# joejep/FOCNeRF

Measured on AMD Instinct MI355X. Metric: train_samples_per_sec, higher is better.
Workload: dtype f16

## Files before the change

focnerf_amd/_lib.py:

```python
import ctypes
import os

import torch

_HERE = os.path.dirname(os.path.abspath(__file__))
LIB_PATH = os.environ.get("FOCNERF_LIB_PATH") or os.path.join(_HERE, "libfocnerf_hip.so")

c_u8p = ctypes.c_void_p
c_vp = ctypes.c_void_p
u32 = ctypes.c_uint32
u64 = ctypes.c_uint64
f32 = ctypes.c_float
i32 = ctypes.c_int

FOC_F32 = 0
FOC_F16 = 1



class FocOccTrainNode(ctypes.Structure):
    _fields_ = [
        ("struct_bytes", u32),
        ("n_rays", u32), ("max_steps", u32), ("cascade", u32), ("grid_size", u32), ("cap", u32), ("pad_align", u32),
        ("bound", f32), ("dt_gamma", f32), ("min_near", f32),
# ... 59 lines not shown
    "foc_occ_train_backward_pad31": (i32, [ctypes.POINTER(FocOccTrainNode), f32, c_vp]),
    "foc_occ_train_forward_obj": (i32, [ctypes.POINTER(FocOccTrainNode), ctypes.POINTER(FocOccTrainObject), c_vp]),
    "foc_occ_train_backward_obj": (i32, [ctypes.POINTER(FocOccTrainNode), ctypes.POINTER(FocOccTrainObject), c_vp]),
    "foc_occ_tail_forward_sumsq": (i32, [c_vp, c_vp, u32, c_vp, c_vp, u32, u32, f32, f32, c_vp, f32, c_vp, c_vp, c_vp, c_vp, c_vp, c_vp, c_vp, c_vp]),
    "foc_occ_tail_backward_sumsq": (i32, [c_vp, c_vp, c_vp, c_vp, u32, c_vp, c_vp, c_vp, c_vp, c_vp, u32, u32, f32, f32, c_vp, f32, c_vp, c_vp, c_vp, c_vp]),
    "foc_occ_tail_forward": (i32, [c_vp, c_vp, u32, c_vp, c_vp, u32, u32, f32, f32, c_vp, f32, c_vp, c_vp, c_vp, c_vp, c_vp, c_vp, c_vp]),
    "foc_occ_tail_backward": (i32, [c_vp, c_vp, c_vp, c_vp, u32, c_vp, c_vp, c_vp, c_vp, c_vp, u32, u32, f32, f32, c_vp, f32, c_vp, c_vp, c_vp]),
    "foc_march_rays_train_scratch_bytes": (u64, [u32, u32]),
    "foc_composite_rays_train_forward": (i32, [c_vp, c_vp, c_vp, c_vp, u32, u32, f32, c_vp, c_vp, c_vp, c_vp]),
    "foc_composite_rays_train_backward": (i32, [c_vp, c_vp, c_vp, c_vp, c_vp, c_vp, c_vp, c_vp, u32, u32, f32,
                                                c_vp, c_vp, c_vp]),
    "foc_march_rays": (i32, [u32, u32, c_vp, c_vp, c_vp, c_vp, f32, f32, u32, u32, u32, c_vp, c_vp, c_vp,
                             c_vp, c_vp, c_vp, c_vp, c_vp]),
    "foc_composite_rays": (i32, [u32, u32, f32, c_vp, c_vp, c_vp, c_vp, c_vp, c_vp, c_vp, c_vp, c_vp]),
    "foc_compact_alive": (i32, [c_vp, u32, c_vp, c_vp, c_vp, c_vp]),
    "foc_march_rays_two_phase": (i32, [u32, u32, c_vp, c_vp, c_vp, c_vp, f32, f32, u32, u32, u32, c_vp, c_vp, c_vp, c_vp, c_vp, c_vp, c_vp, c_vp, i32, c_vp]),
    "foc_composite_compact": (i32, [u32, u32, f32, c_vp, c_vp, c_vp, c_vp, c_vp, c_vp, c_vp, c_vp, c_vp, c_vp, c_vp, c_vp, u32, u32, i32, c_vp]),
    "foc_march_rays_two_phase_fills": (i32, [u32, i32]),
    "foc_march_rays_two_phase_sample_major": (i32, [u32, u32, i32]),
    "foc_occ_render_step_scratch_bytes": (u64, [u32]),
    "foc_occ_render_step": (i32, [u32, u32, c_vp, c_vp, c_vp, c_vp, c_vp, c_vp, f32, f32, u32, u32, u32, c_vp, c_vp, c_vp, c_vp, c_vp, c_vp, c_vp, c_vp,
                                  c_vp, c_vp, c_vp, u32, f32, u32, c_vp, u32, c_vp, u32, u32, c_vp, f32, c_vp, c_vp, c_vp, c_vp, u32, c_vp, u32, u32, c_vp]),
    "foc_occ_render_step_pad31": (i32, [u32, u32, c_vp, c_vp, c_vp, c_vp, c_vp, c_vp, f32, f32, u32, u32, u32, c_vp, c_vp, c_vp, c_vp, c_vp, c_vp, c_vp, c_vp,
                                        c_vp, c_vp, c_vp, u32, f32, u32, c_vp, u32, c_vp, u32, u32, c_vp, f32, c_vp, c_vp, c_vp, c_vp, u32, c_vp, u32, u32, f32,
                                        c_vp]),
    "foc_occ_render_step_pad": (i32, [u32, u32, c_vp, c_vp, c_vp, c_vp, c_vp, c_vp, f32, f32, u32, u32, u32, c_vp, c_vp, c_vp, c_vp, c_vp, c_vp, c_vp, c_vp,
                                      c_vp, c_vp, c_vp, u32, f32, u32, c_vp, u32, c_vp, u32, u32, c_vp, f32, c_vp, c_vp, c_vp, c_vp, u32, c_vp, u32, u32, f32,
                                      c_vp]),
    "foc_grid_encode_forward": (i32, [c_vp, c_vp, c_vp, c_vp, u32, u32, u32, u32, f32, u32, c_vp, u32, i32, u32,
                                      i32, c_vp, c_vp]),
    "foc_grid_encode_forward_bl": (i32, [c_vp, c_vp, c_vp, c_vp, u32, u32, u32, u32, f32, u32, c_vp, u32, i32, u32,
                                         i32, c_vp, c_vp]),
    "foc_grid_encode_backward": (i32, [c_vp, c_vp, c_vp, c_vp, c_vp, u32, u32, u32, u32, f32, u32, c_vp, c_vp,
                                       u32, i32, u32, i32, i32, c_vp, c_vp]),
    "foc_grid_encode_backward_workspace_bytes": (u64, [u32, u32, u32, u32, i32]),
    "foc_grid_planes_to_rows": (i32, [c_vp, c_vp, u32, u32, u32, c_vp]),
    "foc_grid_rows_to_planes": (i32, [c_vp, c_vp, u32, u32, u32, c_vp]),
    "foc_grid_encode_backward_binned": (i32, [c_vp, c_vp, c_vp, c_vp, c_vp, u32, u32, u32, u32, f32, u32, c_vp, c_vp,
                                              u32, i32, u32, i32, i32, c_vp, c_vp, u64, c_vp]),
    "foc_grid_encode_forward_counted": (i32, [c_vp, c_vp, c_vp, c_vp, u32, u32, u32, u32, f32, u32, u32, i32, u32, i32, c_vp, c_vp, u64, c_vp]),
    "foc_grid_encode_backward_count": (i32, [c_vp, c_vp, u32, u32, u32, u32, f32, u32, u32, i32, u32, i32, c_vp, c_vp, u64, c_vp]),
    "foc_grid_encode_backward_binned_counted": (i32, [c_vp, c_vp, c_vp, c_vp, c_vp, u32, u32, u32, u32, f32, u32, c_vp, c_vp,
                                                      u32, i32, u32, i32, i32, c_vp, c_vp, u64, c_vp]),
    "foc_grad_total_variation": (i32, [c_vp, c_vp, c_vp, c_vp, f32, u32, u32, u32, u32, f32, u32, u32, i32, i32, c_vp]),
    "foc_freq_encode_forward": (i32, [c_vp, u32, u32, u32, u32, c_vp, c_vp]),
    "foc_freq_encode_backward": (i32, [c_vp, c_vp, u32, u32, u32, u32, c_vp, c_vp]),
    "foc_ffmlp_forward": (i32, [c_vp, c_vp, u32, u32, u32, u32, u32, u32, u32, c_vp, c_vp, c_vp]),
    "foc_ffmlp_inference": (i32, [c_vp, c_vp, u32, u32, u32, u32, u32, u32, u32, c_vp, c_vp, c_vp]),
    "foc_ffmlp_backward": (i32, [c_vp, c_vp, c_vp, c_vp, u32, u32, u32, u32, u32, u32, u32, i32,
                                 c_vp, c_vp, c_vp, c_vp, u64, c_vp]),
    "foc_ffmlp_backward_workspace_bytes": (u64, [u32, u32, u32]),
    "foc_ffmlp_forward_planar": (i32, [c_vp, c_vp, u32, u32, u32, u32, u32, u32, u32, c_vp, c_vp]),
    "foc_ffmlp_backward_planar": (i32, [c_vp, c_vp, c_vp, u32, u32, u32, u32, u32, u32, u32, i32, c_vp, c_vp, c_vp, u64, c_vp]),
    "foc_allocate_splitk": (i32, [u64]),
    "foc_free_splitk": (i32, []),
    "foc_combine_select": (i32, [c_vp, c_vp, c_vp, c_vp, u64, c_vp]),
    "foc_combine_pack_keys": (i32, [c_vp, u32, c_vp, u64, c_vp]),
    "foc_combine_unpack": (i32, [c_vp, u32, c_vp, c_vp, c_vp, u64, c_vp]),
    "foc_combine_select_composite": (i32, [c_vp, u32, c_vp, c_vp, u32, u32, c_vp, u32, c_vp, c_vp, c_vp, c_vp]),
    "foc_combine_select4": (i32, [c_vp, c_vp, u64, c_vp]),
    "foc_combine_select_composite_attr": (i32, [c_vp, u32, c_vp, c_vp, u32, c_vp, c_vp, u32, u32, c_vp, u32, c_vp, c_vp, c_vp, c_vp, c_vp, c_vp, c_vp, c_vp]),
    "foc_combine_select4_ids": (i32, [c_vp, u32, c_vp, c_vp, u64, c_vp]),
    "foc_mo_select": (i32, [c_vp, c_vp, c_vp, c_vp, u64, u32, u32, c_vp]),
    "foc_fixed_field_pack": (i32, [c_vp, c_vp, c_vp, c_vp, c_vp, c_vp, f32, u32, u32, f32, f32, c_vp, c_vp, c_vp, c_vp, u32, c_vp]),
    "foc_fixed_cull_scratch_bytes": (u64, [u32, u32]),
    "foc_fixed_cull": (i32, [c_vp, c_vp, c_vp, c_vp, c_vp, u32, u32, f32, c_vp, u32, u32, c_vp, c_vp, c_vp, c_vp, u64, c_vp]),
    "foc_fixed_cull_emit": (i32, [c_vp, c_vp, c_vp, c_vp, c_vp, u32, u32, f32, c_vp, c_vp, u32, c_vp, c_vp, c_vp]),
    "foc_fixed_field_pack_culled": (i32, [c_vp, c_vp, c_vp, c_vp, u32, c_vp, c_vp, u32, u32, f32, f32, c_vp, c_vp]),
    "foc_composite_fixed_steps":(i32, [c_vp, c_vp, c_vp, c_vp, u32, u32, f32, c_vp, c_vp, c_vp]),
    "foc_fixed_sample": (i32, [c_vp, c_vp, c_vp, c_vp, c_vp, c_vp, u32, u32, f32, c_vp, c_vp, c_vp, u32, c_vp]),
    "foc_fixed_tail_forward": (i32, [c_vp, c_vp, c_vp, c_vp, c_vp, c_vp, f32, u32, u32, f32, f32, c_vp, c_vp, c_vp, c_vp, c_vp, c_vp, u32, c_vp, c_vp]),
    "foc_fixed_tail_backward": (i32, [c_vp, c_vp, c_vp, c_vp, c_vp, c_vp, c_vp, c_vp, c_vp, c_vp, c_vp, f32, u32, u32, f32, f32, c_vp, c_vp, u32, c_vp, c_vp]),
    "foc_fixed_head_forward": (i32, [c_vp, c_vp, c_vp, c_vp, c_vp, u32, u32, f32, c_vp, c_vp, c_vp, c_vp, c_vp, c_vp, c_vp, u32, c_vp]),
    "foc_fixed_head_backward": (i32, [c_vp, c_vp, c_vp, c_vp, c_vp, c_vp, c_vp, c_vp, c_vp, c_vp, u32, u32, f32, c_vp, u32, c_vp]),
    "foc_color_head_forward": (i32, [c_vp, c_vp, u32, c_vp, u32, u32, u32, u32, c_vp, u32, c_vp, c_vp]),
    "foc_field_forward_train": (i32, [c_vp, c_vp, u32, c_vp, u32, c_vp, u32, u32, u32, u32, c_vp, c_vp, u32, c_vp, c_vp]),
    "foc_color_head_backward": (i32, [c_vp, c_vp, c_vp, u32, c_vp, c_vp, u32, u32, u32, u32, c_vp, c_vp, c_vp, u64, u32, c_vp, c_vp, c_vp]),
    "foc_color_head_forward_pad": (i32, [c_vp, c_vp, u32, c_vp, u32, u32, u32, u32, c_vp, u32, c_vp, f32, c_vp]),
    "foc_color_head_backward_pad": (i32, [c_vp, c_vp, c_vp, u32, c_vp, c_vp, u32, u32, u32, u32, c_vp, c_vp, c_vp, u64, u32, c_vp, c_vp, f32, c_vp]),
    "foc_field_forward_train_pad": (i32, [c_vp, c_vp, u32, c_vp, u32, c_vp, u32, u32, u32, u32, c_vp, c_vp, u32, c_vp, f32, c_vp]),
    "foc_color_head_forward_pad31": (i32, [c_vp, c_vp, u32, c_vp, u32, u32, u32, u32, c_vp, u32, c_vp, f32, c_vp]),
    "foc_color_head_backward_pad31": (i32, [c_vp, c_vp, c_vp, u32, c_vp, c_vp, u32, u32, u32, u32, c_vp, c_vp, c_vp, u64, u32, c_vp, c_vp, f32, c_vp]),
    "foc_field_forward_train_pad31": (i32, [c_vp, c_vp, u32, c_vp, u32, c_vp, u32, u32, u32, u32, c_vp, c_vp, u32, c_vp, f32, c_vp]),
    "foc_fixed_composite_forward": (i32, [c_vp, c_vp, c_vp, f32, u32, u32, f32, c_vp, c_vp]),
    "foc_fixed_composite_backward": (i32, [c_vp, c_vp, c_vp, c_vp, f32, u32, u32, f32, c_vp, c_vp, c_vp]),
    "foc_sample_head_forward": (i32, [c_vp, c_vp, u64, c_vp, c_vp, c_vp, u32, c_vp]),
    "foc_sample_head_backward": (i32, [c_vp, c_vp, c_vp, u64, c_vp, u32, c_vp]),
    "foc_sh_encode": (i32, [c_vp, u64, c_vp, c_vp]),
    "foc_rgb_head_forward": (i32, [c_vp, u64, c_vp, c_vp]),
    "foc_rgb_head_backward": (i32, [c_vp, c_vp, u64, c_vp, c_vp]),
    "foc_fixed_render_inference": (i32, [c_vp, c_vp, c_vp, c_vp, c_vp, c_vp, f32, u32, u32, f32, f32, c_vp, c_vp, c_vp, c_vp, u32, c_vp, c_vp]),
    "foc_nerf_field_inference": (i32, [c_vp, i32, c_vp, u32, u32, u32, c_vp, u32, c_vp, u32, u32, u32, u32, c_vp, c_vp, c_vp, c_vp]),
    "foc_nerf_field_inference_pad": (i32, [c_vp, i32, c_vp, u32, u32, u32, c_vp, u32, c_vp, u32, u32, u32, u32, c_vp, c_vp, c_vp, f32, c_vp]),
    "foc_nerf_field_inference_pad31": (i32, [c_vp, i32, c_vp, u32, u32, u32, c_vp, u32, c_vp, u32, u32, u32, u32, c_vp, c_vp, c_vp, f32, c_vp]),
    "foc_mark_untrained_grid": (i32, [c_vp, u32, f32, f32, f32, f32, f32, u32, u32, c_vp, c_vp, c_vp]),
    "foc_grid_cells_xyz": (i32, [u32, u32, f32, c_vp, c_vp, c_vp]),
    "foc_grid_update_sample_workspace_bytes": (u64, [u32, u32]),
    "foc_grid_update_sample": (i32, [c_vp, u32, u32, f32, u32, c_vp, c_vp, c_vp, c_vp, c_vp, c_vp, u64, c_vp]),
    "foc_grid_update_apply_workspace_bytes": (u64, [u32, u32]),
    "foc_grid_update_apply": (i32, [c_vp, u32, u32, c_vp, c_vp, u32, f32, f32, f32, c_vp, c_vp, c_vp, u64, c_vp]),
    "foc_background_forward": (i32, [c_vp, c_vp, c_vp, f32, u32, c_vp, c_vp, f32, u32, c_vp, c_vp, c_vp]),
    "foc_background_backward_workspace_bytes": (u64, [u32]),
    "foc_background_backward": (i32, [c_vp, c_vp, c_vp, c_vp, f32, u32, c_vp, c_vp, f32, u32, c_vp, c_vp, c_vp, c_vp, u64, c_vp]),
}


def _load():
    if not os.path.exists(LIB_PATH):
        raise ImportError(
            f"focnerf_amd: {LIB_PATH} is missing. Build it with `python -c 'import __graft_entry__ as g; g.build()'` "
            f"or `make -C focnerf_amd/csrc`. There is no CPU or PyTorch fallback for these ops.")
    try:
        lib = ctypes.CDLL(LIB_PATH)
    except OSError as e:
        raise ImportError(f"focnerf_amd: failed to load {LIB_PATH}: {e}") from e
    for name, (res, args) in SIGNATURES.items():
        fn = getattr(lib, name)
        fn.restype = res
        fn.argtypes = args
    return lib


class _Stream(ctypes.c_void_p):
    device_index = None


_multi_device = None


def _on_tensor_device(fn):
    def call(*args):
        global _multi_device
        if _multi_device is None:
            _multi_device = torch.cuda.device_count() > 1
        if _multi_device and args:
            idx = getattr(args[-1], "device_index", None)
            if idx is not None and idx != torch.cuda.current_device():
                with torch.cuda.device(idx):
                    return fn(*args)
        return fn(*args)
    call.__name__ = getattr(fn, "__name__", "foc_call")
    return call


class _Lib:

    def __init__(self, cdll):
        self._cdll = cdll
        for name, (_, args) in SIGNATURES.items():
            fn = getattr(cdll, name)
            setattr(self, name, _on_tensor_device(fn) if args and args[-1] is c_vp and not name.endswith("_bytes") else fn)


lib = _Lib(_load())


def check(rc, what=""):
    if rc != 0:
        msg = lib.foc_last_error().decode("utf-8", "replace")
        raise RuntimeError(f"focnerf_amd {what}: {msg} (code {rc})")


def ptr(t):
    if t is None:
        return None
    return ctypes.c_void_p(t.data_ptr())


_raw_stream = getattr(torch._C, "_cuda_getCurrentRawStream", None) if os.environ.get("FOC_RAW_STREAM", "1") != "0" else None


def raw_stream(index):
    if _raw_stream is not None:
        return _raw_stream(index)
    return torch.cuda.current_stream(index).cuda_stream


def stream_of(t=None):
    dev = t.device if t is not None else None
    index = dev.index if dev is not None and dev.index is not None else torch.cuda.current_device()
    s = _Stream(raw_stream(index))
    s.device_index = index
    return s


def require_cuda(*tensors):
    for t in tensors:
        if t is not None and not t.is_cuda:
            raise RuntimeError("focnerf_amd: expected a CUDA(HIP) tensor; these ops have no CPU implementation")


def dtype_code(t):
    if t.dtype == torch.float32:
        return FOC_F32
    if t.dtype == torch.float16:
        return FOC_F16
    raise RuntimeError(f"focnerf_amd: unsupported dtype {t.dtype} (float32 or float16 expected)")


def get_option(name):
    v = ctypes.c_int(0)
    check(lib.foc_get_option(name.encode(), ctypes.cast(ctypes.byref(v), ctypes.c_void_p)), "get_option")
    return v.value


def set_option(name, value):
    check(lib.foc_set_option(name.encode(), int(value)), "set_option")


class option:

    def __init__(self, name, value):
        self.name, self.value = name, int(value)

    def __enter__(self):
        self.old = get_option(self.name)
        set_option(self.name, self.value)
        return self

    def __exit__(self, *exc):
        set_option(self.name, self.old)
        return False
```

focnerf_amd/csrc/combine.hip:

```cpp
#include "common.h"
#include <string.h>

static thread_local char g_err[512] = "";

void foc_set_error(const char *fmt, ...) {
    va_list ap;
    va_start(ap, fmt);
    vsnprintf(g_err, sizeof(g_err), fmt, ap);
    va_end(ap);
}

__global__ void __launch_bounds__(256) k_combine_select(const float *__restrict__ dens, const float *__restrict__ rgb,
                                                        float *__restrict__ max_dens, float *__restrict__ best_rgb, uint64_t n) {
    for (uint64_t i = (uint64_t)blockIdx.x * 256 + threadIdx.x; i < n; i += (uint64_t)gridDim.x * 256) {
        const float d = dens[i], m = max_dens[i];
        if (d > m) { best_rgb[i * 3] = rgb[i * 3]; best_rgb[i * 3 + 1] = rgb[i * 3 + 1]; best_rgb[i * 3 + 2] = rgb[i * 3 + 2]; }
        max_dens[i] = (d != d || m != m) ? __builtin_nanf("") : (d > m ? d : m);
    }
}

__global__ void __launch_bounds__(256) k_combine_pack(const float *__restrict__ dens, uint32_t rank, uint64_t *__restrict__ keys, uint64_t n) {
    for (uint64_t i = (uint64_t)blockIdx.x * 256 + threadIdx.x; i < n; i += (uint64_t)gridDim.x * 256) {
        float d = dens[i];
        d = d > 0.0f ? d : 0.0f;
// ... 162 lines not shown
        if (lane < n_obj) {
            at->obj_weights[(uint64_t)n * n_obj + lane] = my_w;
            at->obj_depth[(uint64_t)n * n_obj + lane] = my_d;
        }
        if (lane == 0) at->instance[n] = inst;
    }
    if (lane == 0) {
        for (uint32_t q = 0; q < n_bg; q++) {
            const float rest = (1 - ws) * (q == 0 ? bg0 : bg1);
            const float o[4] = {r + rest, g + rest, b + rest, a + rest};
#pragma unroll
            for (int k = 0; k < 4; k++) image4[((uint64_t)q * N + n) * 4 + k] = fminf(1.0f, fmaxf(0.0f, o[k]));
        }
        depth[n] = d;
    }
}

__global__ void __launch_bounds__(256) k_combine_select_composite(CombineFields fields, uint32_t K, const float *__restrict__ nears,
                                                                  const float *__restrict__ fars, uint32_t N, uint32_t T, float bg0, float bg1,
                                                                  uint32_t n_bg, float *__restrict__ image4, float *__restrict__ depth,
                                                                  float4 *__restrict__ merged4) {
    combine_select_composite_body<0>(fields, nullptr, K, nears, fars, N, T, bg0, bg1, n_bg, image4, depth, merged4);
}

template <int NOBJ>
__global__ void __launch_bounds__(256) k_combine_select_composite_attr(CombineFields fields, CombineAttr at, uint32_t K,
                                                                       const float *__restrict__ nears, const float *__restrict__ fars, uint32_t N,
                                                                       uint32_t T, float bg0, float bg1, uint32_t n_bg, float *__restrict__ image4,
                                                                       float *__restrict__ depth, float4 *__restrict__ merged4) {
    combine_select_composite_body<NOBJ>(fields, &at, K, nears, fars, N, T, bg0, bg1, n_bg, image4, depth, merged4);
}

__global__ void __launch_bounds__(256) k_combine_select4(const float4 *__restrict__ f4, float4 *__restrict__ acc4, uint64_t n) {
    for (uint64_t i = (uint64_t)blockIdx.x * 256 + threadIdx.x; i < n; i += (uint64_t)gridDim.x * 256) {
        const float4 f = f4[i];
        float4 best = acc4[i];
        const float m = best.x;
        if (f.x > m) { best.y = f.y; best.z = f.z; best.w = f.w; }
        best.x = (f.x != f.x || m != m) ? __builtin_nanf("") : (f.x > m ? f.x : m);
        acc4[i] = best;
    }
}

__global__ void __launch_bounds__(256) k_combine_select4_ids(const float4 *__restrict__ f4, uint8_t id, float4 *__restrict__ acc4,
                                                             uint8_t *__restrict__ acc_ids, uint64_t n) {
    for (uint64_t i = (uint64_t)blockIdx.x * 256 + threadIdx.x; i < n; i += (uint64_t)gridDim.x * 256) {
        const float4 f = f4[i];
        float4 best = acc4[i];
        const float m = best.x;
        if (f.x > m) { best.y = f.y; best.z = f.z; best.w = f.w; acc_ids[i] = id; }
        best.x = (f.x != f.x || m != m) ? __builtin_nanf("") : (f.x > m ? f.x : m);
        acc4[i] = best;
    }
}

template <typename T>
__global__ void __launch_bounds__(256) k_mo_select(const T *__restrict__ sig_new, const T *__restrict__ feat_new, T *__restrict__ sig_best,
                                                   T *__restrict__ feat_best, uint64_t n, uint32_t width) {
    const uint64_t s0 = ((uint64_t)blockIdx.x * 4u + (threadIdx.x >> 6)) * 64u;
    if (s0 >= n) return;
    const uint32_t lane = threadIdx.x & 63u;
    bool take = false;
    if (s0 + lane < n) {
        const T a_raw = sig_new[s0 + lane];
        const float a = (float)a_raw, b = (float)sig_best[s0 + lane];
        take = (a != a) || (b == b && a >= b);
        if (take) sig_best[s0 + lane] = a_raw;
    }
    const uint64_t rows = __ballot(take);
    const uint32_t live = (uint32_t)(n - s0 < 64u ? n - s0 : 64u);
    const uint64_t base = s0 * width;
    for (uint32_t e = lane; e < live * width; e += 64u)
        if ((rows >> (e / width)) & 1ull) feat_best[base + e] = feat_new[base + e];
}

#include <stdlib.h>
#include <string.h>
#include <atomic>
#include <mutex>
struct FocOptionRow { const char *name; std::atomic<int> value; };
static FocOptionRow foc_option_table[FOC_OPT_COUNT] = {
    {"FOC_MLP_BWD_FUSED", 1}, {"FOC_FIELD_FWD_FUSED", 1}, {"FOC_GB_MERGE_MAX_RES", 480}, {"FOC_GB_FACTORED", 1}, {"FOC_GB_TAIL_SPLIT", 16}, {"FOC_GRID_FUSE_SMALL", 1},
    {"FOC_GRID_PAIRS", 1}, {"FOC_GRID_FAST", 1}, {"FOC_MARCH_SERIAL", -1}, {"FOC_MARCH_RAYS_ROW_MAX", 131072}, {"FOC_OCC_MARCH_FORM", -1},
    {"FOC_OCC_SAMPLE_MAJOR", 1}, {"FOC_OCC_FIELD_PIECE", 1 << 23}, {"FOC_DETERMINISTIC", 0},
};
static int foc_option_parse(int which, const char *text) {
    if (which == FOC_OPT_OCC_MARCH_FORM) {
        if (text[0] == 't') return 0;
        if (text[0] == 'r') return 1;
        if (text[0] == 'l') return 2;
        if (text[0] == 's') return 3;
    }
    return atoi(text);
}
static void foc_options_init() {
    static std::once_flag once;
    std::call_once(once, [] {
        for (int i = 0; i < FOC_OPT_COUNT; i++) {
            const char *e = getenv(foc_option_table[i].name);
            if (e && e[0]) foc_option_table[i].value.store(foc_option_parse(i, e), std::memory_order_relaxed);
        }
    });
}
int foc_opt(FocOpt which) { foc_options_init(); return foc_option_table[which].value.load(std::memory_order_relaxed); }

extern "C" {

int foc_set_option(const char *name, int value) {
    foc_options_init();
    for (int i = 0; i < FOC_OPT_COUNT; i++)
        if (name && strcmp(name, foc_option_table[i].name) == 0) { foc_option_table[i].value.store(value, std::memory_order_relaxed); return FOC_OK; }
    foc_set_error("set_option: unknown option '%s'", name ? name : "(null)");
    return FOC_E_INVALID;
}

int foc_get_option(const char *name, int *value) {
    foc_options_init();
    for (int i = 0; i < FOC_OPT_COUNT; i++)
        if (name && value && strcmp(name, foc_option_table[i].name) == 0) { *value = foc_option_table[i].value.load(std::memory_order_relaxed); return FOC_OK; }
    foc_set_error("get_option: unknown option '%s'", name ? name : "(null)");
    return FOC_E_INVALID;
}

int foc_guard_pick_device(int stream_is_null, int stream_device, int pointer_device, int current_device) {
    return foc_guard_pick(stream_is_null != 0, stream_device, pointer_device, current_device);
}


int foc_combine_select_composite(const float *const *fields4, uint32_t K, const float *nears, const float *fars, uint32_t N, uint32_t T,
                                 const float *bgs, uint32_t n_bg, float *image4, float *depth, float *merged4, void *stream) {
    FocDeviceGuard foc_guard_(stream, nears);
    FOC_REQUIRE(K >= 1 && K <= FOC_COMBINE_MAX_OBJECTS, FOC_E_INVALID, "combine_select_composite: 1 <= K <= %d objects per call (got %u)",
                FOC_COMBINE_MAX_OBJECTS, K);
    FOC_REQUIRE(n_bg >= 1 && n_bg <= 2 && bgs, FOC_E_INVALID, "combine_select_composite: one or two backgrounds");
    FOC_REQUIRE(T >= 2, FOC_E_INVALID, "combine_select_composite: T must be >= 2");
    if (N == 0) return FOC_OK;
    FOC_REQUIRE(fields4 && nears && fars && image4 && depth, FOC_E_INVALID, "combine_select_composite: null pointer");
    CombineFields f;
    for (uint32_t k = 0; k < FOC_COMBINE_MAX_OBJECTS; k++) {
        f.p[k] = reinterpret_cast<const float4 *>(k < K ? fields4[k] : fields4[0]);
        FOC_REQUIRE(f.p[k] && ((uintptr_t)f.p[k] & 15) == 0, FOC_E_INVALID, "combine_select_composite: field %u is null or not 16-byte aligned", k);
    }
    FOC_REQUIRE(((uintptr_t)merged4 & 15) == 0, FOC_E_INVALID, "combine_select_composite: merged4 must be 16-byte aligned");
    hipLaunchKernelGGL(k_combine_select_composite, dim3(foc_div_up(N, 4)), dim3(256), 0, (hipStream_t)stream, f, K, nears, fars, N, T, bgs[0],
                       n_bg > 1 ? bgs[1] : 0.0f, n_bg, image4, depth, reinterpret_cast<float4 *>(merged4));
    FOC_CHECK_LAUNCH("combine_select_composite");
    return FOC_OK;
}

int foc_combine_select4(const float *field4, float *acc4, uint64_t n, void *stream) {
    FocDeviceGuard foc_guard_(stream, field4);
    FOC_REQUIRE(n == 0 || (field4 && acc4), FOC_E_INVALID, "combine_select4: null pointer");
    FOC_REQUIRE((((uintptr_t)field4 | (uintptr_t)acc4) & 15) == 0, FOC_E_INVALID, "combine_select4: fields must be 16-byte aligned");
    if (n == 0) return FOC_OK;
    hipLaunchKernelGGL(k_combine_select4, dim3(foc_grid_1d(n, 256)), dim3(256), 0, (hipStream_t)stream, reinterpret_cast<const float4 *>(field4),
                       reinterpret_cast<float4 *>(acc4), n);
    FOC_CHECK_LAUNCH("combine_select4");
    return FOC_OK;
}

int foc_combine_select_composite_attr(const float *const *fields4, uint32_t K, const uint8_t *const *id_planes, const uint32_t *ids,
                                      uint32_t n_obj, const float *nears, const float *fars, uint32_t N, uint32_t T, const float *bgs,
                                      uint32_t n_bg, float *image4, float *depth, float *merged4, float *obj_weights, float *obj_depth,
                                      int32_t *instance, uint8_t *winner, void *stream) {
    FocDeviceGuard foc_guard_(stream, nears);
    FOC_REQUIRE(K >= 1 && K <= FOC_COMBINE_MAX_OBJECTS, FOC_E_INVALID, "combine_select_composite_attr: 1 <= K <= %d fields per call (got %u)",
                FOC_COMBINE_MAX_OBJECTS, K);
// ... 114 lines not shown
```

focnerf_amd/csrc/common.h:

```cpp
#pragma once
#include <hip/hip_runtime.h>
#include <hip/hip_fp16.h>
#include <stdint.h>
#include <stdio.h>
#include <stdarg.h>
#include "../../include/focnerf.h"

#define FOC_WAVE 64

void foc_set_error(const char *fmt, ...);

enum FocOpt {
    FOC_OPT_MLP_BWD_FUSED,
    FOC_OPT_FIELD_FWD_FUSED,
    FOC_OPT_GB_MERGE_MAX_RES,
    FOC_OPT_GB_FACTORED,
    FOC_OPT_GB_TAIL_SPLIT,
    FOC_OPT_GRID_FUSE_SMALL,
    FOC_OPT_GRID_PAIRS,
    FOC_OPT_GRID_FAST,
    FOC_OPT_MARCH_SERIAL,
    FOC_OPT_MARCH_RAYS_ROW_MAX,
    FOC_OPT_OCC_MARCH_FORM,
    FOC_OPT_OCC_SAMPLE_MAJOR,
    FOC_OPT_OCC_FIELD_PIECE,
    FOC_OPT_DETERMINISTIC,
    FOC_OPT_COUNT
};
int foc_opt(FocOpt which);

#define FOC_REQUIRE(cond, code, ...)                    \
    do {                                                \
        if (!(cond)) {                                  \
            foc_set_error(__VA_ARGS__);                 \
            return (code);                              \
        }                                               \
    } while (0)

#define FOC_CHECK_LAUNCH(name)                                                     \
    do {                                                                           \
        hipError_t e_ = hipGetLastError();                                         \
        if (e_ != hipSuccess) {                                                    \
            foc_set_error("%s: launch failed: %s", name, hipGetErrorString(e_));   \
            return FOC_E_LAUNCH;                                                   \
        }                                                                          \
    } while (0)

static inline int foc_guard_pick(bool stream_is_null, int stream_device, int pointer_device, int current_device) {
    if (!stream_is_null && stream_device >= 0) return stream_device;
    if (pointer_device >= 0) return pointer_device;
    return current_device;
}
struct FocDeviceGuard {
    int prev = -1;
    explicit FocDeviceGuard(void *stream, const void *first_pointer = nullptr) {
        static int n_devices = -1;
        if (n_devices < 0 && hipGetDeviceCount(&n_devices) != hipSuccess) { (void)hipGetLastError(); n_devices = 0; }
        if (n_devices == 1) return;
        int cur = 0;
        if (hipGetDevice(&cur) != hipSuccess) return;
        int sdev = -1, pdev = -1;
        if (stream != nullptr) {
            if (hipStreamGetDevice(static_cast<hipStream_t>(stream), &sdev) != hipSuccess) { (void)hipGetLastError(); sdev = -1; }
        } else if (first_pointer != nullptr) {
            hipPointerAttribute_t attr;
            if (hipPointerGetAttributes(&attr, first_pointer) == hipSuccess && attr.type == hipMemoryTypeDevice) pdev = attr.device;
            else (void)hipGetLastError();
        }
        const int want = foc_guard_pick(stream == nullptr, sdev, pdev, cur);
        if (want != cur && hipSetDevice(want) == hipSuccess) prev = cur;
    }
    ~FocDeviceGuard() { if (prev >= 0) (void)hipSetDevice(prev); }
    FocDeviceGuard(const FocDeviceGuard &) = delete;
    FocDeviceGuard &operator=(const FocDeviceGuard &) = delete;
};

static inline uint32_t foc_div_up(uint64_t a, uint64_t b) { return (uint32_t)((a + b - 1) / b); }

static inline uint32_t foc_grid_1d(uint64_t n, uint32_t block, uint32_t max_blocks = 256 * 8) {
    uint64_t g = (n + block - 1) / block;
    if (g < 1) g = 1;
    if (g > max_blocks) g = max_blocks;
    return (uint32_t)g;
}

__device__ __forceinline__ _Float16 foc_f2h(float v) { asm volatile("" : "+v"(v)); return (_Float16)v; }

__global__ static void __launch_bounds__(256) k_foc_zero(uint32_t *__restrict__ p, uint64_t n_words) {
    for (uint64_t i = (uint64_t)blockIdx.x * 256 + threadIdx.x; i < n_words; i += (uint64_t)gridDim.x * 256) p[i] = 0u;
}
static inline hipError_t foc_zero_async(void *p, size_t bytes, hipStream_t st) {
    const uint64_t n = bytes / 4;
    if (n == 0) return hipSuccess;
    uint64_t blocks = (n + 255) / 256;
    if (blocks > 4096) blocks = 4096;
    hipLaunchKernelGGL(k_foc_zero, dim3((uint32_t)blocks), dim3(256), 0, st, reinterpret_cast<uint32_t *>(p), n);
    return hipGetLastError();
}

__device__ __forceinline__ void foc_lds_barrier() { asm volatile("s_waitcnt lgkmcnt(0)\n\ts_barrier" ::: "memory"); }

__device__ __forceinline__ float wave_sum(float v) {
#pragma unroll
    for (int o = 32; o > 0; o >>= 1) v += __shfl_xor(v, o, 64);
    return v;
}
__device__ __forceinline__ int wave_sum_i(int v) {
#pragma unroll
    for (int o = 32; o > 0; o >>= 1) v += __shfl_xor(v, o, 64);
    return v;
}
__device__ __forceinline__ float wave_incl_prod(float v, int lane) {
#pragma unroll
    for (int o = 1; o < 64; o <<= 1) {
        float u = __shfl_up(v, o, 64);
        if (lane >= o) v *= u;
    }
    return v;
}
__device__ __forceinline__ float wave_incl_sum(float v, int lane) {
#pragma unroll
    for (int o = 1; o < 64; o <<= 1) {
        float u = __shfl_up(v, o, 64);
        if (lane >= o) v += u;
    }
    return v;
}
__device__ __forceinline__ int wave_incl_sum_i(int v, int lane) {
#pragma unroll
    for (int o = 1; o < 64; o <<= 1) {
        int u = __shfl_up(v, o, 64);
        if (lane >= o) v += u;
    }
    return v;
}
```

focnerf_amd/csrc/field_fwd.hip:

```cpp
#include "mlp_common.h"

typedef uint32_t ff_u2 __attribute__((ext_vector_type(2)));

__device__ __forceinline__ uint32_t ff_pack(float a, float b) {
    typedef _Float16 h2 __attribute__((ext_vector_type(2)));
    const h2 p = {(_Float16)a, (_Float16)b};
    return __builtin_bit_cast(uint32_t, p);
}

#ifndef FF_MIN_WAVES
#define FF_MIN_WAVES 2
#endif
template <int NLS, int NLC, bool RELU>
__global__ void __launch_bounds__(MLP_BLOCK, FF_MIN_WAVES) k_field_fwd_train(const _Float16 *__restrict__ planes, const _Float16 *__restrict__ w_sigma,
                                                               const _Float16 *__restrict__ w_color, _Float16 *__restrict__ h_out,
                                                               _Float16 *__restrict__ c_out, uint32_t B, MlpHead hd) {
    constexpr int HIDDEN = 64, MT = 2, KC = 4, KS0 = 2;
    constexpr int FS = MT * KS0 + (NLS - 1) * MT * KC + KC;
    constexpr int FC = MT * KS0 + (NLC - 1) * MT * KC + KC;
    extern __shared__ __attribute__((aligned(16))) _Float16 lds[];
    _Float16 *ldsS = lds, *ldsC = lds + FS * 512;
    const float *obj_bias = reinterpret_cast<const float *>(ldsC + FC * 512);
    stage_weights_fwd<HIDDEN>(w_sigma, ldsS, 32, NLS);
    stage_weights_fwd<HIDDEN>(w_color, ldsC, 32, NLC, true, head_ld0(hd));
    if (head_bias(hd)) stage_head_bias(w_color, hd, const_cast<float *>(obj_bias), HIDDEN);
    __syncthreads();

    const uint32_t lane = threadIdx.x & 63, wave = threadIdx.x >> 6;
    const int c = lane & 31, h = lane >> 5;
    const uint32_t n_tiles = (B + 31) / 32;
    const uint32_t tstride = gridDim.x * MLP_WAVES;
    uint32_t tile = blockIdx.x * MLP_WAVES + wave;
    h8 x_nxt[KS0], sh_nxt;
    auto fetch = [&](uint32_t t) {
#ifdef FF_TIMING_NO_LOAD
        const uint64_t r = (uint64_t)c + 0 * t;
#else
        const uint64_t r = min((uint64_t)min(t, n_tiles - 1u) * 32 + c, (uint64_t)B - 1);
#endif
#pragma unroll
        for (int kc = 0; kc < KS0; kc++) x_nxt[kc] = ld_planar8(planes, B, r, kc, h);
        sh_nxt = ld_head8(planes, hd, r, 0, h);
    };
    fetch(tile);
    for (; tile < n_tiles; tile += tstride) {
#ifndef FF_TIMING_HOIST
        asm volatile("" ::: "memory");
#endif
        const uint64_t row_raw = (uint64_t)tile * 32 + c;
        h8 x_cur[KS0];
#pragma unroll
        for (int kc = 0; kc < KS0; kc++) x_cur[kc] = x_nxt[kc];
        const h8 sh = sh_nxt;
        fetch(tile + tstride);
        f16v acc[MT];
#pragma unroll
        for (int mt = 0; mt < MT; mt++)
#pragma unroll
            for (int e = 0; e < 16; e++) acc[mt][e] = 0.0f;
#pragma unroll
        for (int kc = 0; kc < KS0; kc++)
#pragma unroll
            for (int mt = 0; mt < MT; mt++) acc[mt] = mfma16(ld_frag(ldsS, mt * KS0 + kc, lane), x_cur[kc], acc[mt]);
        f16v o;
        for (uint32_t l = 1; l <= (uint32_t)NLS; l++) {
            h8 bf[KC];
#pragma unroll
            for (int kc = 0; kc < KC; kc++) bf[kc] = acc_to_frag<RELU>(acc[kc >> 1], kc & 1);
            if (l < (uint32_t)NLS) {
                const uint32_t fbase = MT * KS0 + (l - 1) * MT * KC;
#pragma unroll
                for (int mt = 0; mt < MT; mt++)
#pragma unroll
                    for (int e = 0; e < 16; e++) acc[mt][e] = 0.0f;
#pragma unroll
                for (int kc = 0; kc < KC; kc++)
#pragma unroll
                    for (int mt = 0; mt < MT; mt++) acc[mt] = mfma16(ld_frag(ldsS, fbase + mt * KC + kc, lane), bf[kc], acc[mt]);
            } else {
#pragma unroll
                for (int e = 0; e < 16; e++) o[e] = 0.0f;
#pragma unroll
                for (int kc = 0; kc < KC; kc++) o = mfma16(ld_frag(ldsS, FS - KC + kc, lane), bf[kc], o);
            }
        }
        uint32_t P0 = ff_pack(o[0], o[1]), P1 = ff_pack(o[2], o[3]), P2 = ff_pack(o[4], o[5]), P3 = ff_pack(o[6], o[7]);
#ifdef FF_TIMING_NO_STORE
        if (row_raw == 0xFFFFFFFFFFull) {
#else
        if (row_raw < B) {
#endif
            *reinterpret_cast<ff_u2 *>(h_out + row_raw * 16 + 4 * h) = ff_u2{P0, P1};
            *reinterpret_cast<ff_u2 *>(h_out + row_raw * 16 + 8 + 4 * h) = ff_u2{P2, P3};
        }
        const uint32_t nxt = h == 0 ? P2 : 0u;
        const ff_u2 s02 = __builtin_amdgcn_permlane32_swap(P0, P2, false, false);
        const ff_u2 s13 = __builtin_amdgcn_permlane32_swap(P1, P3, false, false);
        const h8 hk = head_shift(u32x4{s02.x, s13.x, s02.y, s13.y}, nxt);
#pragma unroll
        for (int mt = 0; mt < MT; mt++) {
            if (head_bias(hd)) acc[mt] = ld_obj_bias(obj_bias, mt, h);
            else {
#pragma unroll
                for (int e = 0; e < 16; e++) acc[mt][e] = 0.0f;
            }
        }
#pragma unroll
        for (int kc = 0; kc < KS0; kc++)
#pragma unroll
            for (int mt = 0; mt < MT; mt++) acc[mt] = mfma16(ld_frag(ldsC, mt * KS0 + kc, lane), kc == 0 ? sh : hk, acc[mt]);
        for (uint32_t l = 1; l <= (uint32_t)NLC; l++) {
            h8 bf[KC];
#pragma unroll
            for (int kc = 0; kc < KC; kc++) bf[kc] = acc_to_frag<RELU>(acc[kc >> 1], kc & 1);
            if (l < (uint32_t)NLC) {
                const uint32_t fbase = MT * KS0 + (l - 1) * MT * KC;
#pragma unroll
                for (int mt = 0; mt < MT; mt++)
#pragma unroll
                    for (int e = 0; e < 16; e++) acc[mt][e] = 0.0f;
#pragma unroll
                for (int kc = 0; kc < KC; kc++)
#pragma unroll
                    for (int mt = 0; mt < MT; mt++) acc[mt] = mfma16(ld_frag(ldsC, fbase + mt * KC + kc, lane), bf[kc], acc[mt]);
            } else {
#pragma unroll
                for (int e = 0; e < 16; e++) o[e] = 0.0f;
#pragma unroll
                for (int kc = 0; kc < KC; kc++) o = mfma16(ld_frag(ldsC, FC - KC + kc, lane), bf[kc], o);
                if (hd.out_width == 4u) {
#ifdef FF_TIMING_NO_STORE
                    if (h == 0 && row_raw == 0xFFFFFFFFFFull) *reinterpret_cast<ff_u2 *>(c_out + row_raw * 4) = ff_u2{ff_pack(o[0], o[1]), ff_pack(o[2], o[3])};
#else
                    if (h == 0 && row_raw < B) *reinterpret_cast<ff_u2 *>(c_out + row_raw * 4) = ff_u2{ff_pack(o[0], o[1]), ff_pack(o[2], o[3])};
#endif
                } else store_tile<false>(c_out, 16, row_raw, B, 0, 16, o, h);
            }
        }
    }
}

static uint32_t ff_num_cus() {
    int dev = 0, n = 0;
    if (hipGetDevice(&dev) != hipSuccess || hipDeviceGetAttribute(&n, hipDeviceAttributeMultiprocessorCount, dev) != hipSuccess || n <= 0) n = 256;
    return (uint32_t)n;
}

template <int NLS, int NLC, bool RELU>
static int ff_launch(const void *planes, const void *w_sigma, const void *w_color, void *h, void *c, uint32_t B, const MlpHead &hd, hipStream_t st) {
    auto kern = k_field_fwd_train<NLS, NLC, RELU>;
    const size_t lds = (size_t)((4 + (NLS - 1) * 8 + 4) + (4 + (NLC - 1) * 8 + 4)) * 1024 + 256;
    if (lds > 64 * 1024) (void)hipFuncSetAttribute(reinterpret_cast<const void *>(kern), hipFuncAttributeMaxDynamicSharedMemorySize, (int)lds);
    static int resident = 0;
    if (!resident) {
        int n = 0;
        if (hipOccupancyMaxActiveBlocksPerMultiprocessor(&n, kern, MLP_BLOCK, lds) != hipSuccess || n < 1) n = 2;
        resident = n > 8 ? 8 : n;
    }
    uint32_t grid = foc_div_up(foc_div_up(B, 32), MLP_WAVES);
    const uint32_t cap = ff_num_cus() * (uint32_t)resident;
    if (grid > cap) grid = cap;
    hipLaunchKernelGGL(kern, dim3(grid), dim3(MLP_BLOCK), lds, st, (const _Float16 *)planes, (const _Float16 *)w_sigma, (const _Float16 *)w_color,
                       (_Float16 *)h, (_Float16 *)c, B, hd);
    FOC_CHECK_LAUNCH("field_forward_train");
    return FOC_OK;
}

template <int NLS, int NLC>
static int ff_launch_act(const void *planes, const void *w_sigma, const void *w_color, void *h, void *c, uint32_t B, int relu, const MlpHead &hd, hipStream_t st) {
    return relu ? ff_launch<NLS, NLC, true>(planes, w_sigma, w_color, h, c, B, hd, st) : ff_launch<NLS, NLC, false>(planes, w_sigma, w_color, h, c, B, hd, st);
}

static int field_forward_train(const void *planes, const void *sigma_weights, uint32_t sigma_layers, const void *ray_sh, uint32_t samples_per_ray,
                               const void *color_weights, uint32_t color_layers, uint32_t hidden_dim, uint32_t activation, uint32_t B, void *h, void *c,
                               uint32_t out_width, const void *obj_feat, float input_pad, bool pad31, void *stream) {
    FocDeviceGuard foc_guard_(stream, planes);
    if (B == 0) return FOC_OK;
    FOC_REQUIRE(planes && sigma_weights && ray_sh && color_weights && h && c, FOC_E_INVALID, "field_forward_train: null pointer");
    FOC_REQUIRE(hidden_dim == 64 && samples_per_ray >= 1, FOC_E_INVALID, "field_forward_train: hidden_dim must be 64 (got %u), samples_per_ray >= 1", hidden_dim);
    FOC_REQUIRE(activation == FOC_ACT_RELU || activation == FOC_ACT_NONE, FOC_E_INVALID, "field_forward_train: hidden activation must be relu(0) or none(6)");
    FOC_REQUIRE(out_width == 16 || out_width == 4, FOC_E_INVALID, "field_forward_train: out_width must be 16 or 4 (got %u)", out_width);
    const int prc = head_pad_check("field_forward_train", pad31, obj_feat, input_pad);
    if (prc) return prc;
    const MlpHead hd{(const _Float16 *)ray_sh, nullptr, samples_per_ray, out_width, (const _Float16 *)obj_feat, input_pad};
    const int relu = activation == FOC_ACT_RELU;
    hipStream_t st = (hipStream_t)stream;
    switch (sigma_layers * 10 + color_layers) {
        case 12: return ff_launch_act<1, 2>(planes, sigma_weights, color_weights, h, c, B, relu, hd, st);
        case 13: return ff_launch_act<1, 3>(planes, sigma_weights, color_weights, h, c, B, relu, hd, st);
        case 22: return ff_launch_act<2, 2>(planes, sigma_weights, color_weights, h, c, B, relu, hd, st);
        case 23: return ff_launch_act<2, 3>(planes, sigma_weights, color_weights, h, c, B, relu, hd, st);
        case 33: return ff_launch_act<3, 3>(planes, sigma_weights, color_weights, h, c, B, relu, hd, st);
        default: foc_set_error("field_forward_train: layer counts (%u, %u) are not built (1/2, 1/3, 2/2, 2/3, 3/3)", sigma_layers, color_layers); return FOC_E_INVALID;
    }
}

extern "C" {

int foc_field_forward_train(const void *planes, const void *sigma_weights, uint32_t sigma_layers, const void *ray_sh, uint32_t samples_per_ray,
                            const void *color_weights, uint32_t color_layers, uint32_t hidden_dim, uint32_t activation, uint32_t B, void *h, void *c,
                            uint32_t out_width, const void *obj_feat, void *stream) {
    return field_forward_train(planes, sigma_weights, sigma_layers, ray_sh, samples_per_ray, color_weights, color_layers, hidden_dim, activation, B, h, c,
                               out_width, obj_feat, 0.0f, false, stream);
}

int foc_field_forward_train_pad(const void *planes, const void *sigma_weights, uint32_t sigma_layers, const void *ray_sh, uint32_t samples_per_ray,
                                const void *color_weights, uint32_t color_layers, uint32_t hidden_dim, uint32_t activation, uint32_t B, void *h, void *c,
                                uint32_t out_width, const void *obj_feat, float input_pad, void *stream) {
    return field_forward_train(planes, sigma_weights, sigma_layers, ray_sh, samples_per_ray, color_weights, color_layers, hidden_dim, activation, B, h, c,
                               out_width, obj_feat, input_pad, false, stream);
}

int foc_field_forward_train_pad31(const void *planes, const void *sigma_weights, uint32_t sigma_layers, const void *ray_sh, uint32_t samples_per_ray,
                                  const void *color_weights, uint32_t color_layers, uint32_t hidden_dim, uint32_t activation, uint32_t B, void *h, void *c,
                                  uint32_t out_width, const void *obj_feat, float input_pad, void *stream) {
    return field_forward_train(planes, sigma_weights, sigma_layers, ray_sh, samples_per_ray, color_weights, color_layers, hidden_dim, activation, B, h, c,
                               out_width, obj_feat, input_pad, true, stream);
}

}
```

focnerf_amd/csrc/fixedstep.hip:

```cpp
#include "common.h"
#include "fs_common.h"
#include <float.h>

typedef _Float16 h8 __attribute__((ext_vector_type(8)));

template <bool NOISE>
__device__ __forceinline__ float fs_zu(const FsGeom &g, uint32_t i, uint32_t T, float u) {
    const float lin = (i < T / 2) ? (g.step * (float)i) : fmaf(-g.step, (float)(T - 1 - i), 1.0f);
    float z = g.near + g.span * lin;
    if (NOISE) z = z + (u - 0.5f) * g.sample_dist;
    return z;
}

__device__ __forceinline__ void fs_sh16(float x, float y, float z, float (&o)[16]) {
    const float xy = x * y, xz = x * z, yz = y * z, x2 = x * x, y2 = y * y, z2 = z * z;
    o[0] = 0.28209479177387814f;
    o[1] = -0.48860251190291987f * y;
    o[2] = 0.48860251190291987f * z;
    o[3] = -0.48860251190291987f * x;
    o[4] = 1.0925484305920792f * xy;
    o[5] = -1.0925484305920792f * yz;
    o[6] = 0.94617469575755997f * z2 - 0.31539156525251999f;
    o[7] = -1.0925484305920792f * xz;
    o[8] = 0.54627421529603959f * x2 - 0.54627421529603959f * y2;
    o[9] = 0.59004358992664352f * y * (-3.0f * x2 + y2);
    o[10] = 2.8906114426405538f * xy * z;
    o[11] = 0.45704579946446572f * y * (1.0f - 5.0f * z2);
    o[12] = 0.3731763325901154f * z * (5.0f * z2 - 3.0f);
    o[13] = 0.45704579946446572f * x * (1.0f - 5.0f * z2);
    o[14] = 1.4453057213202769f * z * (x2 - y2);
    o[15] = 0.59004358992664352f * x * (-x2 + 3.0f * y2);
}

__global__ void __launch_bounds__(256) k_fs_sample(const float *__restrict__ rays_o, const float *__restrict__ rays_d, const float *__restrict__ nears,
                                                   const float *__restrict__ fars, const float *__restrict__ aabb, const float *__restrict__ noise,
                                                   uint32_t N, uint32_t T, float bound, float *__restrict__ xyzs, float *__restrict__ enc_in,
                                                   _Float16 *__restrict__ ray_sh, uint32_t ray_block) {
    const uint64_t total = ray_block ? (uint64_t)((N + FS_RAY_BLOCK - 1) / FS_RAY_BLOCK) * FS_RAY_BLOCK * T : (uint64_t)N * T;
    const FsBox box = fs_box(aabb);
    const float two_b = 2 * bound;
    for (uint64_t s = (uint64_t)blockIdx.x * 256 + threadIdx.x; s < total; s += (uint64_t)gridDim.x * 256) {
        uint32_t n, i;
        bool own = true;
        if (ray_block) {
            const uint32_t blk = (uint32_t)(s / ((uint64_t)FS_RAY_BLOCK * T)), in = (uint32_t)(s - (uint64_t)blk * FS_RAY_BLOCK * T);
            i = in / FS_RAY_BLOCK;
            n = blk * FS_RAY_BLOCK + in % FS_RAY_BLOCK;
            own = n < N;
            n = own ? n : N - 1;
        } else {
            n = (uint32_t)(s / T); i = (uint32_t)(s - (uint64_t)n * T);
        }
        const FsGeom g = fs_geom(nears, fars, n, T);
        const float z = fs_z(g, i, T, noise, (uint64_t)n * T + i);
        float x, y, w;
        fs_point(rays_o[n * 3], rays_o[n * 3 + 1], rays_o[n * 3 + 2], rays_d[n * 3], rays_d[n * 3 + 1], rays_d[n * 3 + 2], z, box, x, y, w);
        if (xyzs) { xyzs[s * 3] = x; xyzs[s * 3 + 1] = y; xyzs[s * 3 + 2] = w; }
        if (enc_in) { enc_in[s * 3] = fs_norm(x, bound, two_b); enc_in[s * 3 + 1] = fs_norm(y, bound, two_b); enc_in[s * 3 + 2] = fs_norm(w, bound, two_b); }
        if (ray_sh && i == 0 && own) {
            float sh[16];
            fs_sh16(rays_d[n * 3], rays_d[n * 3 + 1], rays_d[n * 3 + 2], sh);
            h8 lo, hi;
#pragma unroll
            for (int k = 0; k < 8; k++) { lo[k] = foc_f2h(sh[k]); hi[k] = foc_f2h(sh[8 + k]); }
            h8 *dst = reinterpret_cast<h8 *>(ray_sh + (uint64_t)n * 16);
            dst[0] = lo; dst[1] = hi;
        }
    }
}

__global__ void __launch_bounds__(256) k_fs_head_fwd(const _Float16 *__restrict__ h, const float *__restrict__ rays_d, const float *__restrict__ nears,
                                                     const float *__restrict__ fars, const float *__restrict__ noise, uint32_t N, uint32_t T,
                                                     float density_scale, float *__restrict__ sigma_out, float *__restrict__ trans_out,
                                                     float *__restrict__ weights_out, float *__restrict__ weights_sum, float *__restrict__ depth,
                                                     _Float16 *__restrict__ cin, const _Float16 *__restrict__ obj, uint32_t cin_ld) {
    const uint32_t lane = threadIdx.x & 63;
    const uint32_t n = blockIdx.x * 4 + (threadIdx.x >> 6);
    if (n >= N) return;
    const FsGeom g = fs_geom(nears, fars, n, T);
    h8 shlo, shhi;
    h8 ob1 = {0, 0, 0, 0, 0, 0, 0, 0}, ob2 = {0, 0, 0, 0, 0, 0, 0, 0};
    _Float16 ob0 = (_Float16)0;
    if (cin) {
        float sh[16];
        fs_sh16(rays_d[n * 3], rays_d[n * 3 + 1], rays_d[n * 3 + 2], sh);
#pragma unroll
        for (int k = 0; k < 8; k++) { shlo[k] = foc_f2h(sh[k]); shhi[k] = foc_f2h(sh[8 + k]); }
        if (obj) {
            ob0 = obj[0];
#pragma unroll
            for (int k = 0; k < 8; k++) ob1[k] = obj[1 + k];
#pragma unroll
            for (int k = 0; k < 7; k++) ob2[k] = obj[9 + k];
        }
    }
    float Tc = 1.0f, ws = 0, dp = 0;
    for (uint32_t base = 0; base < T; base += 64) {
        const uint32_t i = base + lane;
        const bool valid = i < T;
        const uint64_t s = (uint64_t)n * T + (valid ? i : T - 1);
        h8 r0, r1;
        if (cin) { r0 = *reinterpret_cast<const h8 *>(h + s * 16); r1 = *reinterpret_cast<const h8 *>(h + s * 16 + 8); }
        else r0[0] = h[s * 16];
        const float sigma = expf((float)r0[0]);
        const float z = fs_z(g, valid ? i : T - 1, T, noise, s);
        float delta = g.sample_dist;
        if (i + 1 < T) delta = fs_z(g, i + 1, T, noise, s + 1) - z;
        const float alpha = valid ? 1 - expf((-delta * density_scale) * sigma) : 0.0f;
        const float om = valid ? (1 - alpha + 1e-15f) : 1.0f;
        const float P = wave_incl_prod(om, (int)lane);
        float Pex = __shfl_up(P, 1, 64);
        if (lane == 0) Pex = 1.0f;
        const float Tb = Tc * Pex;
        const float w = alpha * Tb;
        if (valid) {
            sigma_out[s] = sigma; trans_out[s] = Tb; weights_out[s] = w;
            float oz = (z - g.near) / g.span;
            oz = oz < 0.0f ? 0.0f : (oz > 1.0f ? 1.0f : oz);
            ws += w; dp += w * oz;
            if (cin) {
                h8 c2, c3;
#pragma unroll
                for (int k = 0; k < 7; k++) { c2[k] = r0[k + 1]; c3[k] = r1[k + 1]; }
                c2[7] = r1[0]; c3[7] = ob0;
                h8 *dst = reinterpret_cast<h8 *>(cin + s * cin_ld);
                dst[0] = shlo; dst[1] = shhi; dst[2] = c2; dst[3] = c3;
                if (cin_ld == 48) { dst[4] = ob1; dst[5] = ob2; }
            }
        }
        Tc *= __shfl(P, 63, 64);
    }
    ws = wave_sum(ws); dp = wave_sum(dp);
    if (lane == 0) { weights_sum[n] = ws; depth[n] = dp; }
}

__device__ __forceinline__ float wave_suffix_incl_sum(float v, int lane) {
#pragma unroll
    for (int o = 1; o < 64; o <<= 1) {
        const float u = __shfl_down(v, o, 64);
        if (lane + o < 64) v += u;
    }
    return v;
}

// ... 23 lines not shown
        float oz = (z - g.near) / g.span;
        oz = oz < 0.0f ? 0.0f : (oz > 1.0f ? 1.0f : oz);
        float gi = (grad_w ? grad_w[s] : 0.0f) + gws;
        if (gdp != 0.0f) gi += gdp * oz;
        const float gw_i = valid ? gi * (alpha * Tb) : 0.0f;
        const float incl = wave_suffix_incl_sum(gw_i, (int)lane);
        const float S_i = S_carry + (incl - gw_i);
        const float dalpha = gi * Tb - S_i / om;
        const float dsigma = dalpha * (delta * density_scale) * ex;
        const _Float16 h0 = h[s * 16];
        const float dh0 = dsigma * expf(fminf(fmaxf((float)h0, -15.0f), 15.0f));
        if (valid) {
            h8 o0, o1;
            if (grad_cin) {
                const h8 c2 = *reinterpret_cast<const h8 *>(grad_cin + s * cin_ld + 16), c3 = *reinterpret_cast<const h8 *>(grad_cin + s * cin_ld + 24);
#pragma unroll
                for (int k = 0; k < 7; k++) { o0[k + 1] = c2[k]; o1[k + 1] = c3[k]; }
                o1[0] = c2[7];
            } else {
#pragma unroll
                for (int k = 0; k < 8; k++) { o0[k] = (_Float16)0; o1[k] = (_Float16)0; }
            }
            o0[0] = foc_f2h(dh0);
            h8 *dst = reinterpret_cast<h8 *>(grad_h + s * 16);
            dst[0] = o0; dst[1] = o1;
        }
        S_carry += __shfl(incl, 0, 64);
    }
}

__device__ __forceinline__ float fs_sigmoid_h(float x) {
    return (float)(_Float16)(1.0f / (1.0f + expf(-x)));
}

__global__ void __launch_bounds__(256) k_fs_composite_fwd(const _Float16 *__restrict__ c, const float *__restrict__ weights, const float *__restrict__ bg_ray,
                                                          float bg_scalar, uint32_t N, uint32_t T, float thresh, float *__restrict__ image) {
    const uint32_t lane = threadIdx.x & 63;
    const uint32_t n = blockIdx.x * 4 + (threadIdx.x >> 6);
    if (n >= N) return;
    float r = 0, g = 0, b = 0, ws = 0;
    for (uint32_t i = lane; i < T; i += 64) {
        const uint64_t s = (uint64_t)n * T + i;
        const float w = weights[s];
        ws += w;
        if (w > thresh) {
            const uint2 raw = *reinterpret_cast<const uint2 *>(c + s * 16);
            const _Float16 *cc = reinterpret_cast<const _Float16 *>(&raw);
            r += w * fs_sigmoid_h((float)cc[0]); g += w * fs_sigmoid_h((float)cc[1]); b += w * fs_sigmoid_h((float)cc[2]);
        }
    }
    r = wave_sum(r); g = wave_sum(g); b = wave_sum(b); ws = wave_sum(ws);
    if (lane == 0) {
        const float b0 = bg_ray ? bg_ray[n * 3] : bg_scalar, b1 = bg_ray ? bg_ray[n * 3 + 1] : bg_scalar, b2 = bg_ray ? bg_ray[n * 3 + 2] : bg_scalar;
        image[n * 3] = r + (1 - ws) * b0; image[n * 3 + 1] = g + (1 - ws) * b1; image[n * 3 + 2] = b + (1 - ws) * b2;
    }
}

__global__ void __launch_bounds__(256) k_fs_composite_bwd(const float *__restrict__ grad_image, const _Float16 *__restrict__ c, const float *__restrict__ weights,
                                                          const float *__restrict__ bg_ray, float bg_scalar, uint32_t N, uint32_t T, float thresh,
                                                          _Float16 *__restrict__ grad_c, float *__restrict__ grad_w) {
    const uint64_t total = (uint64_t)N * T;
    for (uint64_t s = (uint64_t)blockIdx.x * 256 + threadIdx.x; s < total; s += (uint64_t)gridDim.x * 256) {
        const uint32_t n = (uint32_t)(s / T);
        const float g0 = grad_image[n * 3], g1 = grad_image[n * 3 + 1], g2 = grad_image[n * 3 + 2];
        const float b0 = bg_ray ? bg_ray[n * 3] : bg_scalar, b1 = bg_ray ? bg_ray[n * 3 + 1] : bg_scalar, b2 = bg_ray ? bg_ray[n * 3 + 2] : bg_scalar;
        const float w = weights[s];
        float gw = -(g0 * b0 + g1 * b1 + g2 * b2);
        h8 o0, o1;
#pragma unroll
        for (int k = 0; k < 8; k++) { o0[k] = (_Float16)0; o1[k] = (_Float16)0; }
        if (w > thresh) {
            const uint2 raw = *reinterpret_cast<const uint2 *>(c + s * 16);
            const _Float16 *cc = reinterpret_cast<const _Float16 *>(&raw);
            const float y0 = fs_sigmoid_h((float)cc[0]), y1 = fs_sigmoid_h((float)cc[1]), y2 = fs_sigmoid_h((float)cc[2]);
            gw += g0 * y0 + g1 * y1 + g2 * y2;
            o0[0] = foc_f2h(g0 * w * y0 * (1 - y0)); o0[1] = foc_f2h(g1 * w * y1 * (1 - y1)); o0[2] = foc_f2h(g2 * w * y2 * (1 - y2));
        }
        grad_w[s] = gw;
        h8 *dst = reinterpret_cast<h8 *>(grad_c + s * 16);
        dst[0] = o0; dst[1] = o1;
    }
}

template <bool NOISE>
__global__ void __launch_bounds__(256) k_fs_tail_fwd(const _Float16 *__restrict__ h, const _Float16 *__restrict__ c, const float *__restrict__ nears,
                                                     const float *__restrict__ fars, const float *__restrict__ noise, const float *__restrict__ bg_ray,
                                                     float bg_scalar, uint32_t N, uint32_t T, float density_scale, float thresh,
                                                     float *__restrict__ sigma_out, float *__restrict__ trans_out, float *__restrict__ weights_out,
                                                     float *__restrict__ weights_sum, float *__restrict__ depth, float *__restrict__ image, uint32_t c_ld,
                                                     float *__restrict__ ray_sumsq) {
    const uint32_t lane = threadIdx.x & 63;
    const uint32_t n = blockIdx.x * 4 + (threadIdx.x >> 6);
    if (n >= N) return;
    const FsGeom g = fs_geom(nears, fars, n, T);
    float Tc = 1.0f, ws = 0, dp = 0, r = 0, gg = 0, b = 0, sq = 0;
    for (uint32_t base = 0; base < T; base += 64) {
        const uint32_t i = base + lane;
        const bool valid = i < T;
        const uint32_t ic = valid ? i : T - 1;
        const uint64_t s = (uint64_t)n * T + ic;
        const _Float16 h0 = h[s * 16];
        const uint2 raw = *reinterpret_cast<const uint2 *>(c + s * c_ld);
        float u0 = 0.0f, u1 = 0.0f;
        if (NOISE) { u0 = noise[s]; u1 = noise[(uint64_t)n * T + min(ic + 1u, T - 1u)]; }
        const float sigma = expf((float)h0);
        const float z = fs_zu<NOISE>(g, ic, T, u0);
        float delta = g.sample_dist;
        if (i + 1 < T) delta = fs_zu<NOISE>(g, i + 1, T, u1) - z;
        const float alpha = valid ? 1 - expf((-delta * density_scale) * sigma) : 0.0f;
        const float om = valid ? (1 - alpha + 1e-15f) : 1.0f;
        const float P = wave_incl_prod(om, (int)lane);
        float Pex = __shfl_up(P, 1, 64);
        if (lane == 0) Pex = 1.0f;
        const float Tb = Tc * Pex;
        const float w = alpha * Tb;
        if (valid) {
            sigma_out[s] = sigma; trans_out[s] = Tb; weights_out[s] = w;
            float oz = (z - g.near) / g.span;
            oz = oz < 0.0f ? 0.0f : (oz > 1.0f ? 1.0f : oz);
            ws += w; dp += w * oz; sq = fmaf(sigma, sigma, sq);
            if (w > thresh) {
                const _Float16 *cc = reinterpret_cast<const _Float16 *>(&raw);
                r += w * fs_sigmoid_h((float)cc[0]); gg += w * fs_sigmoid_h((float)cc[1]); b += w * fs_sigmoid_h((float)cc[2]);
            }
        }
        Tc *= __shfl(P, 63, 64);
    }
    ws = wave_sum(ws); dp = wave_sum(dp); r = wave_sum(r); gg = wave_sum(gg); b = wave_sum(b);
    if (ray_sumsq) {
        sq = wave_sum(sq);
        if (lane == 0) ray_sumsq[n] = sq;
    }
    if (lane == 0) {
        const float b0 = bg_ray ? bg_ray[n * 3] : bg_scalar, b1 = bg_ray ? bg_ray[n * 3 + 1] : bg_scalar, b2 = bg_ray ? bg_ray[n * 3 + 2] : bg_scalar;
        image[n * 3] = r + (1 - ws) * b0; image[n * 3 + 1] = gg + (1 - ws) * b1; image[n * 3 + 2] = b + (1 - ws) * b2;
        weights_sum[n] = ws; depth[n] = dp;
    }
}

__device__ __forceinline__ float fs_opaque(float v) { asm volatile("" : "+v"(v)); return v; }

template <bool NOISE>
__global__ void __launch_bounds__(256) k_fs_tail_bwd(const float *__restrict__ grad_image, const float *__restrict__ grad_ws, const float *__restrict__ grad_depth,
                                                     const _Float16 *__restrict__ c, const float *__restrict__ sigma_in, const float *__restrict__ trans_in,
                                                     const float *__restrict__ weights, const float *__restrict__ nears, const float *__restrict__ fars,
                                                     const float *__restrict__ noise, const float *__restrict__ bg_ray, float bg_scalar, uint32_t N, uint32_t T,
                                                     float density_scale, float thresh, _Float16 *__restrict__ grad_c, _Float16 *__restrict__ grad_h0, uint32_t c_ld,
                                                     const float *__restrict__ grad_sumsq) {
    const uint32_t lane = threadIdx.x & 63;
    const uint32_t n = blockIdx.x * 4 + (threadIdx.x >> 6);
    if (n >= N) return;
    const FsGeom g = fs_geom(nears, fars, n, T);
    const float gws = grad_ws ? grad_ws[n] : 0.0f, gdp = grad_depth ? grad_depth[n] : 0.0f;
    const float gsq2 = grad_sumsq ? 2.0f * grad_sumsq[n] : 0.0f;
    const float g0 = grad_image[n * 3], g1 = grad_image[n * 3 + 1], g2 = grad_image[n * 3 + 2];
    const float b0 = bg_ray ? bg_ray[n * 3] : bg_scalar, b1 = bg_ray ? bg_ray[n * 3 + 1] : bg_scalar, b2 = bg_ray ? bg_ray[n * 3 + 2] : bg_scalar;
    const float e_lo = expf(fs_opaque(-15.0f)), e_hi = expf(fs_opaque(15.0f));
    float S_carry = 0.0f;
    const uint32_t n_chunks = (T + 63) / 64;
    for (uint32_t cidx = n_chunks; cidx-- > 0;) {
        const uint32_t i = cidx * 64 + lane;
        const bool valid = i < T;
        const uint32_t ic = valid ? i : T - 1;
        const uint64_t s = (uint64_t)n * T + ic;
        const float sigma = sigma_in[s], Tb = trans_in[s], w = weights[s];
        const uint2 raw = *reinterpret_cast<const uint2 *>(c + s * c_ld);
        float u0 = 0.0f, u1 = 0.0f;
        if (NOISE) { u0 = noise[s]; u1 = noise[(uint64_t)n * T + min(ic + 1u, T - 1u)]; }
        float gw = -(g0 * b0 + g1 * b1 + g2 * b2);
        h8 o0, o1;
#pragma unroll
        for (int k = 0; k < 8; k++) { o0[k] = (_Float16)0; o1[k] = (_Float16)0; }
        if (w > thresh) {
            const _Float16 *cc = reinterpret_cast<const _Float16 *>(&raw);
            const float y0 = fs_sigmoid_h((float)cc[0]), y1 = fs_sigmoid_h((float)cc[1]), y2 = fs_sigmoid_h((float)cc[2]);
            gw += g0 * y0 + g1 * y1 + g2 * y2;
            o0[0] = foc_f2h(g0 * w * y0 * (1 - y0)); o0[1] = foc_f2h(g1 * w * y1 * (1 - y1)); o0[2] = foc_f2h(g2 * w * y2 * (1 - y2));
        }
        if (valid) {
            if (c_ld == 4u) *reinterpret_cast<uint2 *>(grad_c + s * 4) = *reinterpret_cast<const uint2 *>(&o0);
            else { h8 *dst = reinterpret_cast<h8 *>(grad_c + s * 16); dst[0] = o0; dst[1] = o1; }
        }
        const float z = fs_zu<NOISE>(g, ic, T, u0);
        float delta = g.sample_dist;
        if (i + 1 < T) delta = fs_zu<NOISE>(g, i + 1, T, u1) - z;
        const float ex = expf((-delta * density_scale) * sigma);
        const float alpha = 1 - ex;
        const float om = 1 - alpha + 1e-15f;
        float oz = (z - g.near) / g.span;
        oz = oz < 0.0f ? 0.0f : (oz > 1.0f ? 1.0f : oz);
        float gi = gw + gws;
        if (gdp != 0.0f) gi += gdp * oz;
        const float gw_i = valid ? gi * (alpha * Tb) : 0.0f;
        const float incl = wave_suffix_incl_sum(gw_i, (int)lane);
        const float S_i = S_carry + (incl - gw_i);
        const float dalpha = gi * Tb - S_i / om;
        float dsigma = dalpha * (delta * density_scale) * ex;
        if (gsq2 != 0.0f) dsigma = fmaf(gsq2, sigma, dsigma);
        const float dh0 = dsigma * fminf(fmaxf(sigma, e_lo), e_hi);
        if (valid) grad_h0[s] = foc_f2h(dh0);
        S_carry += __shfl(incl, 0, 64);
    }
}


template <bool PACK>
__device__ __forceinline__ void fs_infer_finish(FsRayAcc &a, uint32_t n, uint32_t lane, const float *__restrict__ bg_ray, float bg_scalar,
                                                float *__restrict__ image, float *__restrict__ depth, float *__restrict__ weights_sum) {
    const float ws = wave_sum(a.ws), dp = wave_sum(a.dp), r = wave_sum(a.r), gg = wave_sum(a.g), b = wave_sum(a.b);
    if (lane == 0 && (!PACK || image)) {
        const float b0 = bg_ray ? bg_ray[n * 3] : bg_scalar, b1 = bg_ray ? bg_ray[n * 3 + 1] : bg_scalar, b2 = bg_ray ? bg_ray[n * 3 + 2] : bg_scalar;
        image[n * 3] = r + (1 - ws) * b0; image[n * 3 + 1] = gg + (1 - ws) * b1; image[n * 3 + 2] = b + (1 - ws) * b2;
        depth[n] = dp;
        weights_sum[n] = ws;
    }
}

template <bool PACK>
__global__ void __launch_bounds__(256) k_fs_render_infer(const float *__restrict__ sigma_in, const float *__restrict__ rgb_in, const float *__restrict__ nears,
                                                         const float *__restrict__ fars, const float *__restrict__ noise, const float *__restrict__ bg_ray,
                                                         float bg_scalar, uint32_t N, uint32_t T, float density_scale, float thresh,
                                                         float *__restrict__ image, float *__restrict__ depth, float *__restrict__ weights_sum,
                                                         float *__restrict__ rgb_masked, float4 *__restrict__ field4) {
    const uint32_t lane = threadIdx.x & 63;
    const uint32_t n = blockIdx.x * 4 + (threadIdx.x >> 6);
    if (n >= N) return;
    const FsGeom g = fs_geom(nears, fars, n, T);
    FsRayAcc a = {1.0f, 0, 0, 0, 0, 0};
    for (uint32_t base = 0; base < T; base += 64) {
        const uint32_t i = base + lane;
        const bool valid = i < T;
        const uint64_t s = (uint64_t)n * T + (valid ? i : T - 1);
        const float sigma = sigma_in[s];
        float c0 = 0, c1 = 0, c2 = 0;
        if (valid) { c0 = rgb_in[s * 3]; c1 = rgb_in[s * 3 + 1]; c2 = rgb_in[s * 3 + 2]; }
        fs_infer_tile<PACK>(a, g, n, i, lane, T, sigma, c0, c1, c2, noise, density_scale, thresh, rgb_masked, field4, nullptr);
    }
    fs_infer_finish<PACK>(a, n, lane, bg_ray, bg_scalar, image, depth, weights_sum);
}

#define FS_BLK_RAYS 16u
template <bool PACK>
__global__ void __launch_bounds__(1024) k_fs_render_infer_blk(const float *__restrict__ sigma_in, const float *__restrict__ rgb_in, const float *__restrict__ nears,
                                                              const float *__restrict__ fars, const float *__restrict__ noise, const float *__restrict__ bg_ray,
                                                              float bg_scalar, uint32_t N, uint32_t T, float density_scale, float thresh,
                                                              float *__restrict__ image, float *__restrict__ depth, float *__restrict__ weights_sum,
                                                              float *__restrict__ rgb_masked, float4 *__restrict__ field4, float *__restrict__ sigma_rm) {
    __shared__ float tile_s[64][FS_BLK_RAYS + 1];
    __shared__ float tile_c[64][FS_BLK_RAYS * 3 + 1];
    const uint32_t tid = threadIdx.x, lane = tid & 63;
    const uint32_t wv = __builtin_amdgcn_readfirstlane(tid >> 6);
    const uint32_t n0 = blockIdx.x * FS_BLK_RAYS;
    const uint64_t row0 = fs_block_row(n0, 0, T);
    const bool is_s = tid < 256;
    const uint32_t li = is_s ? tid : tid - 256;
    const uint32_t l_step = is_s ? li >> 2 : li / 12, l_part = is_s ? (li & 3) : li % 12;
    const float *src = is_s ? sigma_in + row0 + l_part * 4 : rgb_in + row0 * 3 + l_part * 4;
    const uint32_t src_ld = is_s ? FS_RAY_BLOCK : FS_RAY_BLOCK * 3;
    float *dst = is_s ? &tile_s[l_step][l_part * 4] : &tile_c[l_step][l_part * 4];
    float4 nx = make_float4(0, 0, 0, 0);
    if (l_step < T) nx = *reinterpret_cast<const float4 *>(src + (uint64_t)l_step * src_ld);
    const uint32_t n = n0 + wv;
    const bool own = n < N;
    const FsGeom g = fs_geom(nears, fars, own ? n : N - 1, T);
    FsRayAcc a = {1.0f, 0, 0, 0, 0, 0};
    for (uint32_t base = 0; base < T; base += 64) {
        dst[0] = nx.x; dst[1] = nx.y; dst[2] = nx.z; dst[3] = nx.w;
        __syncthreads();
        if (base + 64 + l_step < T) nx = *reinterpret_cast<const float4 *>(src + (uint64_t)(base + 64 + l_step) * src_ld);
        if (own)
            fs_infer_tile<PACK>(a, g, n, base + lane, lane, T, tile_s[lane][wv], tile_c[lane][wv * 3], tile_c[lane][wv * 3 + 1], tile_c[lane][wv * 3 + 2],
                                noise, density_scale, thresh, rgb_masked, field4, sigma_rm);
        __syncthreads();
    }
    if (own) fs_infer_finish<PACK>(a, n, lane, bg_ray, bg_scalar, image, depth, weights_sum);
}

struct VtState { uint32_t count, first_enc, bad, pad; };

__device__ __forceinline__ bool vt_turn(const float *__restrict__ d, uint32_t i) {
    const float ax = d[(i + 1) * 3] - d[i * 3], ay = d[(i + 1) * 3 + 1] - d[i * 3 + 1], az = d[(i + 1) * 3 + 2] - d[i * 3 + 2];
    const float bx = d[(i + 2) * 3] - d[(i + 1) * 3], by = d[(i + 2) * 3 + 1] - d[(i + 1) * 3 + 1], bz = d[(i + 2) * 3 + 2] - d[(i + 1) * 3 + 2];
    return (bx * ax + by * ay) + bz * az < 0.0f;
}

__global__ void __launch_bounds__(256) k_vt_find(const float *__restrict__ d, uint32_t N, VtState *__restrict__ st) {
    for (uint32_t i = blockIdx.x * 256 + threadIdx.x; i + 2 < N; i += gridDim.x * 256)
        if (vt_turn(d, i)) { atomicAdd(&st->count, 1u); atomicMax(&st->first_enc, N - i); }
}

__global__ void __launch_bounds__(256) k_vt_check(const float *__restrict__ d, uint32_t N, VtState *__restrict__ st) {
    const uint32_t fe = st->first_enc;
    if (fe == 0u) return;
    const uint32_t W = N - fe + 2u;
    for (uint32_t i = blockIdx.x * 256 + threadIdx.x; i + 2 < N; i += gridDim.x * 256) {
        const bool expect = (i + 2u) % W == 0u || (i + 1u) % W == 0u;
        if (vt_turn(d, i) != expect) st->bad = 1u;
    }
}

__global__ void __launch_bounds__(256) k_vt_perm(uint32_t N, uint32_t th, uint32_t tw, const VtState *__restrict__ st, int64_t *__restrict__ perm) {
    const uint32_t fe = st->first_enc, W = fe ? N - fe + 2u : 0u;
    const uint32_t H = W ? N / W : 0u;
    const bool grid = W >= 16u && N % W == 0u && H >= 8u && st->count == 2u * (H - 1u) && st->bad == 0u;
    for (uint32_t p = blockIdx.x * 256 + threadIdx.x; p < N; p += gridDim.x * 256) {
        uint32_t src = p;
        if (grid) {
            const uint64_t wt = (uint64_t)W * th;
            const uint32_t ty = (uint32_t)(p / wt), rem = (uint32_t)(p - ty * wt);
            const uint32_t rows_here = min(th, H - ty * th);
            const uint32_t tx = min(rem / (rows_here * tw), (W - 1u) / tw), r2 = rem - tx * rows_here * tw;
            const uint32_t cols_here = min(tw, W - tx * tw);
            src = (ty * th + r2 / cols_here) * W + tx * tw + r2 % cols_here;
        }
        perm[p] = (int64_t)src;
    }
}

extern "C" {

int foc_fixed_sample(const float *rays_o, const float *rays_d, const float *nears, const float *fars, const float *aabb, const float *noise,
                     uint32_t N, uint32_t T, float bound, float *xyzs, float *enc_in, void *ray_sh, uint32_t ray_block, void *stream) {
    FocDeviceGuard foc_guard_(stream, rays_o);
    if (N == 0) return FOC_OK;
    FOC_REQUIRE(rays_o && rays_d && nears && fars && aabb && (xyzs || enc_in), FOC_E_INVALID, "fixed_sample: null pointer");
    FOC_REQUIRE(T >= 2, FOC_E_INVALID, "fixed_sample: T must be >= 2");
    FOC_REQUIRE(ray_block == 0 || ray_block == FS_RAY_BLOCK, FOC_E_INVALID, "fixed_sample: ray_block must be 0 (ray-major) or %u (got %u)", FS_RAY_BLOCK, ray_block);
    const uint64_t rows = ray_block ? (uint64_t)foc_div_up(N, FS_RAY_BLOCK) * FS_RAY_BLOCK * T : (uint64_t)N * T;
    hipLaunchKernelGGL(k_fs_sample, dim3(foc_grid_1d(rows, 256, 256 * 16)), dim3(256), 0, (hipStream_t)stream, rays_o, rays_d, nears, fars, aabb,
                       noise, N, T, bound, xyzs, enc_in, (_Float16 *)ray_sh, ray_block);
    FOC_CHECK_LAUNCH("fixed_sample");
    return FOC_OK;
}

int foc_fixed_head_forward(const void *h, const float *rays_d, const float *nears, const float *fars, const float *noise, uint32_t N, uint32_t T,
                           float density_scale, float *sigma, float *trans, float *weights, float *weights_sum, float *depth, void *cin,
                           const void *obj_feat, uint32_t cin_width, void *stream) {
    FocDeviceGuard foc_guard_(stream, h);
    if (N == 0) return FOC_OK;
    FOC_REQUIRE(h && rays_d && nears && fars && sigma && trans && weights && weights_sum && depth, FOC_E_INVALID, "fixed_head_forward: null pointer");
    FOC_REQUIRE(T >= 2, FOC_E_INVALID, "fixed_head_forward: T must be >= 2");
    FOC_REQUIRE(cin_width == 32 || cin_width == 48, FOC_E_INVALID, "fixed_head_forward: cin_width must be 32 or 48 (got %u)", cin_width);
    FOC_REQUIRE(!obj_feat || cin_width == 48, FOC_E_INVALID, "fixed_head_forward: an object feature needs the 48-wide colour input");
    hipLaunchKernelGGL(k_fs_head_fwd, dim3(foc_div_up(N, 4)), dim3(256), 0, (hipStream_t)stream, (const _Float16 *)h, rays_d, nears, fars, noise, N, T,
                       density_scale, sigma, trans, weights, weights_sum, depth, (_Float16 *)cin, (const _Float16 *)obj_feat, cin_width);
    FOC_CHECK_LAUNCH("fixed_head_forward");
    return FOC_OK;
}

int foc_fixed_head_backward(const void *h, const float *sigma, const float *trans, const float *nears, const float *fars, const float *noise,
                            const float *grad_w, const float *grad_ws, const float *grad_depth, const void *grad_cin, uint32_t N, uint32_t T,
                            float density_scale, void *grad_h, uint32_t cin_width, void *stream) {
    FocDeviceGuard foc_guard_(stream, h);
    if (N == 0) return FOC_OK;
    FOC_REQUIRE(h && sigma && trans && nears && fars && grad_h, FOC_E_INVALID, "fixed_head_backward: null pointer");
    FOC_REQUIRE(T >= 2, FOC_E_INVALID, "fixed_head_backward: T must be >= 2");
    FOC_REQUIRE(cin_width == 32 || cin_width == 48, FOC_E_INVALID, "fixed_head_backward: cin_width must be 32 or 48 (got %u)", cin_width);
    hipLaunchKernelGGL(k_fs_head_bwd, dim3(foc_div_up(N, 4)), dim3(256), 0, (hipStream_t)stream, (const _Float16 *)h, sigma, trans, nears, fars, noise,
                       grad_w, grad_ws, grad_depth, (const _Float16 *)grad_cin, N, T, density_scale, (_Float16 *)grad_h, cin_width);
    FOC_CHECK_LAUNCH("fixed_head_backward");
    return FOC_OK;
}

int foc_fixed_composite_forward(const void *c, const float *weights, const float *bg_ray, float bg_scalar, uint32_t N, uint32_t T, float thresh,
                                float *image, void *stream) {
    FocDeviceGuard foc_guard_(stream, c);
    if (N == 0) return FOC_OK;
    FOC_REQUIRE(c && weights && image, FOC_E_INVALID, "fixed_composite_forward: null pointer");
    hipLaunchKernelGGL(k_fs_composite_fwd, dim3(foc_div_up(N, 4)), dim3(256), 0, (hipStream_t)stream, (const _Float16 *)c, weights, bg_ray, bg_scalar, N, T,
                       thresh, image);
    FOC_CHECK_LAUNCH("fixed_composite_forward");
    return FOC_OK;
}

int foc_fixed_composite_backward(const float *grad_image, const void *c, const float *weights, const float *bg_ray, float bg_scalar, uint32_t N,
                                 uint32_t T, float thresh, void *grad_c, float *grad_w, void *stream) {
    FocDeviceGuard foc_guard_(stream, grad_image);
    if (N == 0) return FOC_OK;
    FOC_REQUIRE(grad_image && c && weights && grad_c && grad_w, FOC_E_INVALID, "fixed_composite_backward: null pointer");
    hipLaunchKernelGGL(k_fs_composite_bwd, dim3(foc_grid_1d((uint64_t)N * T, 256, 256 * 16)), dim3(256), 0, (hipStream_t)stream, grad_image,
                       (const _Float16 *)c, weights, bg_ray, bg_scalar, N, T, thresh, (_Float16 *)grad_c, grad_w);
    FOC_CHECK_LAUNCH("fixed_composite_backward");
    return FOC_OK;
}

int foc_fixed_tail_forward(const void *h, const void *c, const float *nears, const float *fars, const float *noise, const float *bg_ray, float bg_scalar,
                           uint32_t N, uint32_t T, float density_scale, float thresh, float *sigma, float *trans, float *weights, float *weights_sum,
                           float *depth, float *image, uint32_t c_width, float *ray_sumsq, void *stream) {
    FocDeviceGuard foc_guard_(stream, h);
    if (N == 0) return FOC_OK;
    FOC_REQUIRE(c_width == 16 || c_width == 4, FOC_E_INVALID, "fixed_tail_forward: c_width must be 16 or 4 (got %u)", c_width);
    FOC_REQUIRE(h && c && nears && fars && sigma && trans && weights && weights_sum && depth && image, FOC_E_INVALID, "fixed_tail_forward: null pointer");
    FOC_REQUIRE(T >= 2, FOC_E_INVALID, "fixed_tail_forward: T must be >= 2");
    auto kern = noise ? k_fs_tail_fwd<true> : k_fs_tail_fwd<false>;
    hipLaunchKernelGGL(kern, dim3(foc_div_up(N, 4)), dim3(256), 0, (hipStream_t)stream, (const _Float16 *)h, (const _Float16 *)c, nears, fars, noise,
                       bg_ray, bg_scalar, N, T, density_scale, thresh, sigma, trans, weights, weights_sum, depth, image, c_width, ray_sumsq);
    FOC_CHECK_LAUNCH("fixed_tail_forward");
    return FOC_OK;
}

int foc_fixed_tail_backward(const float *grad_image, const float *grad_ws, const float *grad_depth, const void *c, const float *sigma, const float *trans,
                            const float *weights, const float *nears, const float *fars, const float *noise, const float *bg_ray, float bg_scalar,
                            uint32_t N, uint32_t T, float density_scale, float thresh, void *grad_c, void *grad_h0, uint32_t c_width, const float *grad_sumsq,
                            void *stream) {
    FocDeviceGuard foc_guard_(stream, grad_image);
    if (N == 0) return FOC_OK;
    FOC_REQUIRE(c_width == 16 || c_width == 4, FOC_E_INVALID, "fixed_tail_backward: c_width must be 16 or 4 (got %u)", c_width);
    FOC_REQUIRE(grad_image && c && sigma && trans && weights && nears && fars && grad_c && grad_h0, FOC_E_INVALID, "fixed_tail_backward: null pointer");
    FOC_REQUIRE(T >= 2, FOC_E_INVALID, "fixed_tail_backward: T must be >= 2");
    auto kern = noise ? k_fs_tail_bwd<true> : k_fs_tail_bwd<false>;
    hipLaunchKernelGGL(kern, dim3(foc_div_up(N, 4)), dim3(256), 0, (hipStream_t)stream, grad_image, grad_ws, grad_depth, (const _Float16 *)c, sigma,
                       trans, weights, nears, fars, noise, bg_ray, bg_scalar, N, T, density_scale, thresh, (_Float16 *)grad_c, (_Float16 *)grad_h0, c_width,
                       grad_sumsq);
    FOC_CHECK_LAUNCH("fixed_tail_backward");
    return FOC_OK;
}

int foc_fixed_render_inference(const float *sigma, const float *rgb, const float *nears, const float *fars, const float *noise, const float *bg_ray,
                               float bg_scalar, uint32_t N, uint32_t T, float density_scale, float thresh, float *image, float *depth, float *weights_sum,
                               float *rgb_masked, uint32_t ray_block, float *sigma_raymajor, void *stream) {
    FocDeviceGuard foc_guard_(stream, sigma);
    if (N == 0) return FOC_OK;
    FOC_REQUIRE(sigma && rgb && nears && fars && image && depth && weights_sum, FOC_E_INVALID, "fixed_render_inference: null pointer");
    FOC_REQUIRE(T >= 2, FOC_E_INVALID, "fixed_render_inference: T must be >= 2");
    FOC_REQUIRE(ray_block == 0 || ray_block == FS_RAY_BLOCK, FOC_E_INVALID, "fixed_render_inference: ray_block must be 0 or %u (got %u)", FS_RAY_BLOCK, ray_block);
    FOC_REQUIRE(ray_block || !sigma_raymajor, FOC_E_INVALID, "fixed_render_inference: sigma_raymajor is the un-blocked copy of a blocked sigma (ray_block == 0: sigma already is ray-major)");
    if (ray_block) {
        FOC_REQUIRE((((uintptr_t)sigma | (uintptr_t)rgb) & 15) == 0, FOC_E_INVALID, "fixed_render_inference: blocked sigma / rgb must be 16-byte aligned");
        hipLaunchKernelGGL(k_fs_render_infer_blk<false>, dim3(foc_div_up(N, FS_BLK_RAYS)), dim3(1024), 0, (hipStream_t)stream, sigma, rgb, nears, fars, noise, bg_ray, bg_scalar,
                           N, T, density_scale, thresh, image, depth, weights_sum, rgb_masked, (float4 *)nullptr, sigma_raymajor);
        FOC_CHECK_LAUNCH("fixed_render_inference");
        return FOC_OK;
    }
    hipLaunchKernelGGL(k_fs_render_infer<false>, dim3(foc_div_up(N, 4)), dim3(256), 0, (hipStream_t)stream, sigma, rgb, nears, fars, noise, bg_ray, bg_scalar, N, T,
                       density_scale, thresh, image, depth, weights_sum, rgb_masked, (float4 *)nullptr);
    FOC_CHECK_LAUNCH("fixed_render_inference");
    return FOC_OK;
}

int foc_fixed_field_pack(const float *sigma, const float *rgb, const float *nears, const float *fars, const float *noise, const float *bg_ray,
                         float bg_scalar, uint32_t N, uint32_t T, float density_scale, float thresh, float *image, float *depth, float *weights_sum,
                         float *field4, uint32_t ray_block, void *stream) {
    FocDeviceGuard foc_guard_(stream, sigma);
    if (N == 0) return FOC_OK;
    FOC_REQUIRE(sigma && rgb && nears && fars && field4, FOC_E_INVALID, "fixed_field_pack: null pointer");
    FOC_REQUIRE((image && depth && weights_sum) || (!image && !depth && !weights_sum), FOC_E_INVALID,
                "fixed_field_pack: image, depth and weights_sum go together (all or none)");
    FOC_REQUIRE(((uintptr_t)field4 & 15) == 0, FOC_E_INVALID, "fixed_field_pack: field4 must be 16-byte aligned");
    FOC_REQUIRE(T >= 2, FOC_E_INVALID, "fixed_field_pack: T must be >= 2");
    FOC_REQUIRE(ray_block == 0 || ray_block == FS_RAY_BLOCK, FOC_E_INVALID, "fixed_field_pack: ray_block must be 0 or %u (got %u)", FS_RAY_BLOCK, ray_block);
    if (ray_block) {
        FOC_REQUIRE((((uintptr_t)sigma | (uintptr_t)rgb) & 15) == 0, FOC_E_INVALID, "fixed_field_pack: blocked sigma / rgb must be 16-byte aligned");
        hipLaunchKernelGGL(k_fs_render_infer_blk<true>, dim3(foc_div_up(N, FS_BLK_RAYS)), dim3(1024), 0, (hipStream_t)stream, sigma, rgb, nears, fars, noise, bg_ray, bg_scalar,
                           N, T, density_scale, thresh, image, depth, weights_sum, (float *)nullptr, (float4 *)field4, (float *)nullptr);
        FOC_CHECK_LAUNCH("fixed_field_pack");
        return FOC_OK;
    }
    hipLaunchKernelGGL(k_fs_render_infer<true>, dim3(foc_div_up(N, 4)), dim3(256), 0, (hipStream_t)stream, sigma, rgb, nears, fars, noise, bg_ray, bg_scalar, N, T,
                       density_scale, thresh, image, depth, weights_sum, (float *)nullptr, (float4 *)field4);
    FOC_CHECK_LAUNCH("fixed_field_pack");
    return FOC_OK;
}

int foc_view_tile_order(const float *rays_d, uint32_t N, uint32_t tile_h, uint32_t tile_w, int64_t *perm, void *state16, void *stream) {
    FocDeviceGuard foc_guard_(stream, rays_d);
    if (N == 0) return FOC_OK;
    FOC_REQUIRE(rays_d && perm && state16, FOC_E_INVALID, "view_tile_order: null pointer");
    FOC_REQUIRE(tile_h >= 1 && tile_w >= 1 && tile_h * tile_w <= 4096, FOC_E_INVALID, "view_tile_order: tile %u x %u", tile_h, tile_w);
    FOC_REQUIRE(N < (1u << 31), FOC_E_INVALID, "view_tile_order: N too large");
    hipStream_t st = (hipStream_t)stream;
    VtState *state = reinterpret_cast<VtState *>(state16);
    if (foc_zero_async(state, sizeof(VtState), st) != hipSuccess) { foc_set_error("view_tile_order: zero fill failed"); return FOC_E_LAUNCH; }
    if (N >= 3) {
        hipLaunchKernelGGL(k_vt_find, dim3(foc_grid_1d(N, 256)), dim3(256), 0, st, rays_d, N, state);
        hipLaunchKernelGGL(k_vt_check, dim3(foc_grid_1d(N, 256)), dim3(256), 0, st, rays_d, N, state);
    }
    hipLaunchKernelGGL(k_vt_perm, dim3(foc_grid_1d(N, 256)), dim3(256), 0, st, N, tile_h, tile_w, state, perm);
    FOC_CHECK_LAUNCH("view_tile_order");
    return FOC_OK;
}

}
```

focnerf_amd/csrc/fs_common.h:

```cpp
#pragma once
#include "common.h"

struct FsGeom { float near, far, span, sample_dist, step; };

#define FS_RAY_BLOCK 64u
__host__ __device__ __forceinline__ uint64_t fs_block_row(uint32_t n, uint32_t i, uint32_t T) {
    return (uint64_t)(n / FS_RAY_BLOCK) * FS_RAY_BLOCK * T + (uint64_t)i * FS_RAY_BLOCK + n % FS_RAY_BLOCK;
}

__device__ __forceinline__ FsGeom fs_geom(const float *__restrict__ nears, const float *__restrict__ fars, uint32_t n, uint32_t T) {
    FsGeom g;
    g.near = nears[n]; g.far = fars[n];
    g.span = g.far - g.near;
    g.sample_dist = g.span / (float)T;
    g.step = 1.0f / (float)(T - 1);
    return g;
}
__device__ __forceinline__ float fs_z(const FsGeom &g, uint32_t i, uint32_t T, const float *__restrict__ noise, uint64_t s) {
    const float lin = (i < T / 2) ? (g.step * (float)i) : fmaf(-g.step, (float)(T - 1 - i), 1.0f);
    float z = g.near + g.span * lin;
    if (noise) z = z + (noise[s] - 0.5f) * g.sample_dist;
    return z;
}

struct FsBox { float a0, a1, a2, a3, a4, a5; };
__device__ __forceinline__ FsBox fs_box(const float *__restrict__ aabb) { return FsBox{aabb[0], aabb[1], aabb[2], aabb[3], aabb[4], aabb[5]}; }
__device__ __forceinline__ void fs_point(float ox, float oy, float oz, float dx, float dy, float dz, float z, const FsBox &b, float &x, float &y, float &w) {
    x = ox + dx * z; y = oy + dy * z; w = oz + dz * z;
    x = fminf(fmaxf(x, b.a0), b.a3); y = fminf(fmaxf(y, b.a1), b.a4); w = fminf(fmaxf(w, b.a2), b.a5);
}
__device__ __forceinline__ float fs_norm(float x, float bound, float two_b) { return (x + bound) / two_b; }

struct FsRayAcc { float Tc, ws, dp, r, g, b; };

template <bool PACK>
__device__ __forceinline__ void fs_infer_tile(FsRayAcc &a, const FsGeom &g, uint32_t n, uint32_t i, uint32_t lane, uint32_t T, float sigma, float c0, float c1,
                                              float c2, const float *__restrict__ noise, float density_scale, float thresh, float *__restrict__ rgb_masked,
                                              float4 *__restrict__ field4, float *__restrict__ sigma_rm) {
    const bool valid = i < T;
    const uint64_t s = (uint64_t)n * T + (valid ? i : T - 1);
    const float z = fs_z(g, valid ? i : T - 1, T, noise, s);
    float delta = g.sample_dist;
    if (i + 1 < T) delta = fs_z(g, i + 1, T, noise, s + 1) - z;
    const float alpha = valid ? 1 - expf((-delta * density_scale) * sigma) : 0.0f;
    const float om = valid ? (1 - alpha + 1e-15f) : 1.0f;
    const float P = wave_incl_prod(om, (int)lane);
    float Pex = __shfl_up(P, 1, 64);
    if (lane == 0) Pex = 1.0f;
    const float w = alpha * (a.Tc * Pex);
    if (valid) {
        float oz = (z - g.near) / g.span;
        oz = oz < 0.0f ? 0.0f : (oz > 1.0f ? 1.0f : oz);
        a.ws += w; a.dp += w * oz;
        const bool on = w > thresh;
        if (on) { a.r += w * c0; a.g += w * c1; a.b += w * c2; }
        if (rgb_masked) { rgb_masked[s * 3] = on ? c0 : 0.0f; rgb_masked[s * 3 + 1] = on ? c1 : 0.0f; rgb_masked[s * 3 + 2] = on ? c2 : 0.0f; }
        if (PACK) field4[s] = make_float4(sigma, on ? c0 : 0.0f, on ? c1 : 0.0f, on ? c2 : 0.0f);
        if (sigma_rm) sigma_rm[s] = sigma;
    }
    a.Tc *= __shfl(P, 63, 64);
}
```

focnerf_amd/csrc/raymarching.hip:

```cpp
#include "common.h"
#include "occ_cell.h"
#include <float.h>

#define RM_SQRT3 1.7320508075688772f
#define RM_RPI   0.3183098861837907f

__device__ __forceinline__ float rm_sign(float x) { return copysignf(1.0f, x); }

__device__ __forceinline__ uint32_t rm_morton3D_invert(uint32_t x) {
    x = x & 0x49249249u;
    x = (x | (x >> 2)) & 0xc30c30c3u;
    x = (x | (x >> 4)) & 0x0f00f00fu;
    x = (x | (x >> 8)) & 0xff0000ffu;
    x = (x | (x >> 16)) & 0x0000ffffu;
    return x;
}

__device__ __forceinline__ void rm_near_far(float ox, float oy, float oz, float dx, float dy, float dz, float a0, float a1, float a2, float a3, float a4, float a5,
                                            float min_near, float &near_out, float &far_out) {
    const float rdx = 1 / dx, rdy = 1 / dy, rdz = 1 / dz;
    float near = (a0 - ox) * rdx, far = (a3 - ox) * rdx, t;
    if (near > far) { t = near; near = far; far = t; }
    float near_y = (a1 - oy) * rdy, far_y = (a4 - oy) * rdy;
    if (near_y > far_y) { t = near_y; near_y = far_y; far_y = t; }
    bool miss = (near > far_y || near_y > far);
    if (!miss) {
        if (near_y > near) near = near_y;
        if (far_y < far) far = far_y;
        float near_z = (a2 - oz) * rdz, far_z = (a5 - oz) * rdz;
        if (near_z > far_z) { t = near_z; near_z = far_z; far_z = t; }
        miss = (near > far_z || near_z > far);
        if (!miss) {
            if (near_z > near) near = near_z;
            if (far_z < far) far = far_z;
            if (near < min_near) near = min_near;
        }
    }
    near_out = miss ? FLT_MAX : near;
    far_out = miss ? FLT_MAX : far;
}

__global__ void __launch_bounds__(256) k_near_far_from_aabb(const float *__restrict__ rays_o, const float *__restrict__ rays_d,
                                     const float *__restrict__ aabb, uint32_t N, float min_near,
                                     float *__restrict__ nears, float *__restrict__ fars) {
    const float a0 = aabb[0], a1 = aabb[1], a2 = aabb[2], a3 = aabb[3], a4 = aabb[4], a5 = aabb[5];
    for (uint32_t n = blockIdx.x * blockDim.x + threadIdx.x; n < N; n += gridDim.x * blockDim.x) {
        float near, far;
        rm_near_far(rays_o[n * 3], rays_o[n * 3 + 1], rays_o[n * 3 + 2], rays_d[n * 3], rays_d[n * 3 + 1], rays_d[n * 3 + 2], a0, a1, a2, a3, a4, a5, min_near, near, far);
        nears[n] = near;
        fars[n] = far;
    }
}

__global__ void __launch_bounds__(256) k_sph_from_ray(const float *__restrict__ rays_o, const float *__restrict__ rays_d, float radius,
                               uint32_t N, float *__restrict__ coords) {
    for (uint32_t n = blockIdx.x * blockDim.x + threadIdx.x; n < N; n += gridDim.x * blockDim.x) {
        const float ox = rays_o[n * 3], oy = rays_o[n * 3 + 1], oz = rays_o[n * 3 + 2];
        const float dx = rays_d[n * 3], dy = rays_d[n * 3 + 1], dz = rays_d[n * 3 + 2];
        const float A = fmaf(dz, dz, fmaf(dy, dy, dx * dx));
        const float B = fmaf(oz, dz, fmaf(oy, dy, ox * dx));
        const float C = fmaf(-radius, radius, fmaf(oz, oz, fmaf(oy, oy, ox * ox)));
        const float t = (-B + sqrtf(fmaf(B, B, -(A * C)))) / A;
        const float x = fmaf(t, dx, ox), y = fmaf(t, dy, oy), z = fmaf(t, dz, oz);
        const float theta = atan2f(sqrtf(fmaf(z, z, x * x)), y);
        const float phi = atan2f(z, x);
        coords[n * 2] = fmaf(2 * theta, RM_RPI, -1.0f);
        coords[n * 2 + 1] = phi * RM_RPI;
    }
}

__global__ void __launch_bounds__(256) k_morton3D(const int32_t *__restrict__ coords, uint32_t N, int32_t *__restrict__ indices) {
    for (uint32_t n = blockIdx.x * blockDim.x + threadIdx.x; n < N; n += gridDim.x * blockDim.x)
        indices[n] = (int32_t)rm_morton3D((uint32_t)coords[n * 3], (uint32_t)coords[n * 3 + 1], (uint32_t)coords[n * 3 + 2]);
}
__global__ void __launch_bounds__(256) k_morton3D_invert(const int32_t *__restrict__ indices, uint32_t N, int32_t *__restrict__ coords) {
    for (uint32_t n = blockIdx.x * blockDim.x + threadIdx.x; n < N; n += gridDim.x * blockDim.x) {
        const int32_t ind = indices[n];
        coords[n * 3] = (int32_t)rm_morton3D_invert((uint32_t)(ind >> 0));
        coords[n * 3 + 1] = (int32_t)rm_morton3D_invert((uint32_t)(ind >> 1));
        coords[n * 3 + 2] = (int32_t)rm_morton3D_invert((uint32_t)(ind >> 2));
    }
}

__global__ void __launch_bounds__(256) k_packbits_x4(const float4 *__restrict__ grid4, uint32_t N4, float thresh,
                              uint32_t *__restrict__ bitfield4) {
    for (uint32_t n = blockIdx.x * blockDim.x + threadIdx.x; n < N4; n += gridDim.x * blockDim.x) {
        uint32_t bits = 0;
#pragma unroll
        for (int q = 0; q < 8; q++) {
            const float4 v = grid4[(uint64_t)n * 8 + q];
            bits |= (v.x > thresh ? 1u : 0u) << (q * 4 + 0);
            bits |= (v.y > thresh ? 1u : 0u) << (q * 4 + 1);
            bits |= (v.z > thresh ? 1u : 0u) << (q * 4 + 2);
            bits |= (v.w > thresh ? 1u : 0u) << (q * 4 + 3);
        }
        bitfield4[n] = bits;
    }
}
__global__ void __launch_bounds__(256) k_packbits_tail(const float *__restrict__ grid, uint32_t n0, uint32_t N, float thresh,
                                uint8_t *__restrict__ bitfield) {
    for (uint32_t n = n0 + blockIdx.x * blockDim.x + threadIdx.x; n < N; n += gridDim.x * blockDim.x) {
        uint32_t bits = 0;
#pragma unroll
        for (int i = 0; i < 8; i++) bits |= (grid[(uint64_t)n * 8 + i] > thresh ? 1u : 0u) << i;
        bitfield[n] = (uint8_t)bits;
    }
}

struct RmCell { float x, y, z, dt, mip_bound; int nx, ny, nz; };

struct RmParams {
    float bound, dt_gamma, dt_min, dt_max, rH, H3, Hf, Cf, Hm1;
    uint32_t H;
    float norm_inv;
    int rederive;
    int gamma_pow2;
};
__device__ __forceinline__ float rm_out(const RmParams &p, float x) { return p.norm_inv != 0.0f ? (x + p.bound) * p.norm_inv : x; }

__device__ __forceinline__ bool rm_cell(const uint8_t *__restrict__ grid, const RmParams &p, float ox, float oy, float oz,
                                        float dx, float dy, float dz, float t, RmCell &c) {
    c.x = rm_clamp(fmaf(t, dx, ox), -p.bound, p.bound);
// ... 1193 lines not shown
```

focnerf_amd/field.py:

```python
import os
from dataclasses import dataclass
from typing import Optional

import torch
from torch.autograd import Function
from torch.amp import custom_bwd, custom_fwd

from .backend import _gridencoder, _ffmlp
from .ffmlp import FFMLP, PackedMLP, single_pass_backward
from .gridencoder import GridEncoder, GridSpec


def fused_mlp(model, name):
    get = getattr(model, "fused_mlp", None)
    return get(name) if get is not None else getattr(model, name, None)


@dataclass(frozen=True)
class MlpShape:
    input_dim: int
    hidden_dim: int
    num_layers: int
    activation: int
    output_activation: int
# ... 105 lines not shown
            _half_scope = {}
        return self

    def __exit__(self, *exc):
        global _half_scope
        _half_scope = self._outer
        return False


def _half_of(param):
    if param.dtype == torch.half:
        return param.contiguous()
    if _half_scope is None:
        return param.detach().to(torch.half).contiguous()
    hit = _half_scope.get(id(param))
    if hit is not None and hit[0] is param and hit[1].device == param.device:
        if hit[2] is not None and _raw_stream_of(param.device) != hit[3]:
            torch.cuda.current_stream(param.device).wait_event(hit[2])
        return hit[1]
    h = param.detach().to(torch.half).contiguous()
    ev = st = None
    if h.is_cuda:
        st = _raw_stream_of(h.device)
        ev = torch.cuda.Event()
        ev.record(torch.cuda.current_stream(h.device))
    _half_scope[id(param)] = (param, h, ev, st)
    return h


def scope_cached(key, owner, make):
    if _half_scope is None:
        return make()
    hit = _half_scope.get(key)
    if hit is not None and hit[0] is owner:
        if hit[2] is not None and _raw_stream_of(hit[1].device) != hit[3]:
            torch.cuda.current_stream(hit[1].device).wait_event(hit[2])
        return hit[1]
    v = make()
    ev = st = None
    if v.is_cuda:
        st = _raw_stream_of(v.device)
        ev = torch.cuda.Event()
        ev.record(torch.cuda.current_stream(v.device))
    _half_scope[key] = (owner, v, ev, st)
    return v


def _check_colour_branch(colour, B):
    cweights, shape, ray_sh, T, c_width, obj_feat = colour[:6]
    T = int(T)
    if not (ray_sh.dtype == torch.half and ray_sh.dim() == 2 and ray_sh.shape[1] == 16 and ray_sh.is_contiguous() and T > 0
            and B == ray_sh.shape[0] * T):
        raise RuntimeError(f"hashgrid_mlp colour branch: ray_sh must be a contiguous half [B / T, 16] tensor with B = {B}, T = {T}; got "
                           f"{tuple(ray_sh.shape)} {ray_sh.dtype}{'' if ray_sh.is_contiguous() else ' (strided)'}")
    if c_width not in (4, 16):
        raise RuntimeError(f"hashgrid_mlp colour branch: c_width must be 4 or 16, got {c_width}")
    if shape.input_dim not in (32, 48) or (obj_feat is not None) != (shape.input_dim == 48) or (obj_feat is not None and obj_feat.numel() != 16):
        raise RuntimeError(f"hashgrid_mlp colour branch: a {shape.input_dim}-wide colour input takes "
                           f"{'a 16-element object feature' if shape.input_dim == 48 else 'no object feature'}, got "
                           f"{'none' if obj_feat is None else f'{obj_feat.numel()} elements'}")
    if cweights.numel() != 64 * (shape.input_dim + 64 * (shape.num_layers - 1) + 16):
        raise RuntimeError(f"hashgrid_mlp colour branch: the colour weights hold {cweights.numel()} elements, a {shape.input_dim}-wide "
                           f"{shape.num_layers}-layer network has {64 * (shape.input_dim + 64 * (shape.num_layers - 1) + 16)}")


class _hashgrid_mlp(Function):
    @staticmethod
    @custom_fwd(device_type="cuda")
    def forward(ctx, x, embeddings, weights, offsets, grid, sigma, training, colour=None):
        x = x.contiguous().float()
        B = x.shape[0]
        if colour is not None:
            _check_colour_branch(colour, B)
        S, H, (gridtype, align_corners, interp) = grid.log2_scale, grid.base_resolution, grid.tail()
        L = offsets.shape[0] - 1
        emb = _half_of(embeddings)
        w = _half_of(weights)
        enc = torch.empty(L, B, 2, device=x.device, dtype=torch.half)
        ticket = _gridencoder.grid_encode_forward_counted(x, emb, offsets, enc, B, 3, 2, L, S, H, gridtype, align_corners, interp,
                                                          standalone=_gridencoder.precount_standalone()) if training else None
        if ticket is None:
            _gridencoder.grid_encode_forward(x, emb, offsets, enc, B, 3, 2, L, S, H, None, gridtype, align_corners, interp)
        h = torch.empty(B, 16, device=x.device, dtype=torch.half)
        c = None
        if colour is not None:
            from ._lib import ptr, stream_of, check
            cweights, cshape, ray_sh, T, c_width, obj_feat = colour[:6]
            pad = float(colour[6]) if len(colour) > 6 else 0.0
            wc = _half_of(cweights)
            obj16 = obj_feat.detach().reshape(-1).half().contiguous() if obj_feat is not None else None
            c = torch.empty(B, c_width, device=x.device, dtype=torch.half)
            args = (ptr(enc), ptr(w), sigma.num_layers, ptr(ray_sh), int(T), ptr(wc), int(cshape.num_layers), 64, int(sigma.activation), B, ptr(h),
                    ptr(c), int(c_width), ptr(obj16))
            fn, extra = pad_twin("foc_field_forward_train", pad, obj16 is not None)
            check(fn(*args, *extra, stream_of(enc)), "field_forward_train")
        else:
            _ffmlp.ffmlp_forward_planar(enc, w, B, sigma.input_dim, 16, sigma.hidden_dim, sigma.num_layers, sigma.activation, sigma.output_activation, h)
        if training:
            ctx.save_for_backward(x, emb, w, offsets, enc)
            ctx.cfg = (grid, sigma, B, L)
            ctx.ticket = ticket
        if c is None:
            return h
        ctx.mark_non_differentiable(c)
        ctx.set_materialize_grads(False)
        return h, c

    @staticmethod
    @custom_bwd(device_type="cuda")
    def backward(ctx, grad_h, _grad_c=None):
        x, emb, w, offsets, enc = ctx.saved_tensors
        grid, sigma, B, L = ctx.cfg
        if grad_h is None:
            return (None,) * 8
        grad_h = grad_h.contiguous().half()
        g_enc = torch.empty_like(enc)
        g_w = torch.empty_like(w)
        _ffmlp.ffmlp_backward_planar(grad_h, enc, w, B, sigma.input_dim, 16, sigma.hidden_dim, sigma.num_layers, sigma.activation,
                                     sigma.output_activation, True, g_enc, g_w)
        g_emb = torch.zeros_like(emb)
        _gridencoder.grid_encode_backward(g_enc, x, emb, offsets, g_emb, B, 3, 2, L, grid.log2_scale, grid.base_resolution, None, None, *grid.tail(),
                                          grad_bl=False, precount=ctx.ticket)
        return None, g_emb, g_w, None, None, None, None, None


@torch.no_grad()
def field_infer(model, xn, dirs, dir_div=1, dir_block=0, obj_feat=None):
    from ._lib import ptr, stream_of, check
    enc, sn, cn = model.encoder, fused_mlp(model, "sigma_net"), fused_mlp(model, "color_net")
    grid = enc.spec()
    xn = xn.contiguous().float()
    dirs = dirs.contiguous().float()
    M = xn.shape[0]
    L = enc.offsets.shape[0] - 1
    emb, ws, wc = _half_of(enc.embeddings), _half_of(sn.weights), _half_of(cn.weights)
    planes = torch.empty(L, M, 2, device=xn.device, dtype=torch.half)
    _gridencoder.grid_encode_forward(xn, emb, enc.offsets, planes, M, 3, 2, L, grid.log2_scale, grid.base_resolution, None, *grid.tail())
    sigma = torch.empty(M, dtype=torch.float32, device=xn.device)
    rgb = torch.empty(M, 3, dtype=torch.float32, device=xn.device)
    obj16 = None
    if getattr(model, "uses_object_feature", False):
        if obj_feat is None:
            raise RuntimeError("field_infer: an object-conditioned network needs its encoded object feature")
        obj16 = obj_feat.detach().reshape(-1).half().contiguous()
        assert obj16.numel() == 16
    args = (ptr(planes), 1, ptr(dirs), int(dir_div), int(dir_block), dirs.shape[0], ptr(ws), sn.num_layers, ptr(wc), cn.num_layers, 64, sn.activation, M,
            ptr(sigma), ptr(rgb), ptr(obj16))
    fn, extra = pad_twin("foc_nerf_field_inference", float(getattr(model, "colour_input_pad", 0.0)), obj16 is not None)
    check(fn(*args, *extra, stream_of(xn)), "nerf_field_inference")
    return sigma, rgb


def hashgrid_mlp(encoder, mlp, x, bound=1, colour=None):
    prefix = list(x.shape[:-1])
    xn = (x if bound is None else (x + bound) / (2 * bound)).view(-1, 3)
    h = _hashgrid_mlp.apply(xn, encoder.embeddings, mlp.weights, encoder.offsets, encoder.spec(), MlpShape.of(mlp), mlp.training and torch.is_grad_enabled(),
                            colour)
    if colour is not None:
        h, c = h
        return h.view(prefix + [16]), c
    return h.view(prefix + [16])
```

focnerf_amd/fixedstep.py:

```python
import torch
from torch.autograd import Function

from . import raymarching
from ._lib import lib, ptr, stream_of, check
from .gridencoder import grid_encode


RAY_BLOCK = 64


def ray_block_default():
    import os
    return RAY_BLOCK if os.environ.get("FOC_RAY_BLOCK", str(RAY_BLOCK)) != "0" else 0


def blocked_rows(N, T, ray_block):
    return N * T if not ray_block else -(-N // ray_block) * ray_block * T


def fixed_sample(rays_o, rays_d, nears, fars, aabb, noise, T, bound, want_xyzs=False, want_ray_sh=False, ray_block=0):
    N = rays_o.shape[0]
    dev = rays_o.device
    rows = blocked_rows(N, T, ray_block)
    enc_in = torch.empty(rows, 3, dtype=torch.float32, device=dev)
    xyzs = torch.empty(rows, 3, dtype=torch.float32, device=dev) if want_xyzs else None
    ray_sh = torch.empty(N, 16, dtype=torch.float16, device=dev) if want_ray_sh else None
    check(lib.foc_fixed_sample(ptr(rays_o), ptr(rays_d), ptr(nears), ptr(fars), ptr(aabb), ptr(noise), N, T, float(bound), ptr(xyzs), ptr(enc_in),
                               ptr(ray_sh), int(ray_block), stream_of(rays_o)), "fixed_sample")
    if want_ray_sh:
        return enc_in, xyzs, ray_sh
    return enc_in, xyzs


def ray_sh_rows(rays_d):
    rays_d = rays_d.contiguous().float()
    N, dev = rays_d.shape[0], rays_d.device
    zeros, ones = torch.zeros(N, device=dev), torch.ones(N, device=dev)
    aabb = torch.tensor([-1., -1., -1., 1., 1., 1.], device=dev)
    return fixed_sample(torch.zeros_like(rays_d), rays_d, zeros, ones, aabb, None, 2, 1.0, want_ray_sh=True)[2]


class _density_head(Function):

    @staticmethod
    def forward(ctx, h, rays_d, nears, fars, noise, N, T, density_scale, obj_feat=None):
        h = h.contiguous()
        assert h.dtype == torch.float16 and h.shape == (N * T, 16)
        dev = h.device
        M = N * T
        sigma = torch.empty(M, dtype=torch.float32, device=dev)
        trans = torch.empty(M, dtype=torch.float32, device=dev)
        weights = torch.empty(M, dtype=torch.float32, device=dev)
        ws = torch.empty(N, dtype=torch.float32, device=dev)
        depth = torch.empty(N, dtype=torch.float32, device=dev)
        width = 32 if obj_feat is None else 48
        if obj_feat is not None:
            obj_feat = obj_feat.detach().reshape(-1).half().contiguous()
            assert obj_feat.numel() == 16
        cin = torch.empty(M, width, dtype=torch.float16, device=dev)
        check(lib.foc_fixed_head_forward(ptr(h), ptr(rays_d), ptr(nears), ptr(fars), ptr(noise), N, T, float(density_scale), ptr(sigma), ptr(trans),
                                         ptr(weights), ptr(ws), ptr(depth), ptr(cin), ptr(obj_feat), width, stream_of(h)), "fixed_head_forward")
        ctx.save_for_backward(h, sigma, trans, nears, fars, noise if noise is not None else torch.empty(0, device=dev))
        ctx.has_noise = noise is not None
        ctx.dims = (N, T, float(density_scale))
        ctx.width = width
        ctx.mark_non_differentiable(sigma)
        ctx.set_materialize_grads(False)
        return weights, ws, depth, sigma, cin

    @staticmethod
    def backward(ctx, g_weights, g_ws, g_depth, g_sigma, g_cin):
        h, sigma, trans, nears, fars, noise = ctx.saved_tensors
        N, T, ds = ctx.dims
        noise = noise if ctx.has_noise else None
        g_weights = g_weights.contiguous().float() if g_weights is not None else None
        g_ws = g_ws.contiguous().float() if g_ws is not None else None
        g_depth = g_depth.contiguous().float() if g_depth is not None else None
        g_cin = g_cin.contiguous().half() if g_cin is not None else None
        grad_h = torch.empty_like(h)
        check(lib.foc_fixed_head_backward(ptr(h), ptr(sigma), ptr(trans), ptr(nears), ptr(fars), ptr(noise), ptr(g_weights), ptr(g_ws), ptr(g_depth),
                                          ptr(g_cin), N, T, ds, ptr(grad_h), ctx.width, stream_of(h)), "fixed_head_backward")
        g_obj = None
        if ctx.width == 48 and ctx.needs_input_grad[8] and g_cin is not None:
            g_obj = g_cin[:, 31:47].float().sum(0)
        return grad_h, None, None, None, None, None, None, None, g_obj


class _fixed_composite(Function):

    @staticmethod
    def forward(ctx, c, weights, bg_ray, bg_scalar, N, T, thresh, weights_sum=None):
        c = c.contiguous()
        weights = weights.contiguous()
        assert c.dtype == torch.float16 and c.shape == (N * T, 16) and weights.dtype == torch.float32
        image = torch.empty(N, 3, dtype=torch.float32, device=c.device)
        check(lib.foc_fixed_composite_forward(ptr(c), ptr(weights), ptr(bg_ray), float(bg_scalar), N, T, float(thresh), ptr(image), stream_of(c)),
              "fixed_composite_forward")
        ctx.bg_grad = bg_ray is not None and ctx.needs_input_grad[2]
        if ctx.bg_grad and weights_sum is None:
            raise RuntimeError("_fixed_composite: a background that needs a gradient needs weights_sum")
        empty = torch.empty(0, device=c.device)
        ctx.save_for_backward(c, weights, bg_ray if bg_ray is not None else empty, weights_sum.detach() if ctx.bg_grad else empty)
        ctx.has_bg = bg_ray is not None
        ctx.dims = (N, T, float(thresh), float(bg_scalar))
        return image

    @staticmethod
    def backward(ctx, g_image):
        c, weights, bg_ray, weights_sum = ctx.saved_tensors
        N, T, thresh, bg_scalar = ctx.dims
        bg_ray = bg_ray if ctx.has_bg else None
        g_image = g_image.contiguous().float()
        grad_c = torch.empty_like(c)
        grad_w = torch.empty_like(weights)
        check(lib.foc_fixed_composite_backward(ptr(g_image), ptr(c), ptr(weights), ptr(bg_ray), bg_scalar, N, T, thresh, ptr(grad_c), ptr(grad_w),
                                               stream_of(c)), "fixed_composite_backward")
        g_bg = g_image * (1 - weights_sum).unsqueeze(-1) if ctx.bg_grad else None
        return grad_c, grad_w, g_bg, None, None, None, None, None


_C_WIDTH = 4


class _render_tail(Function):

    @staticmethod
    def forward(ctx, h, cweights, ray_sh, nears, fars, noise, bg_ray, bg_scalar, N, T, density_scale, thresh, num_layers, activation, obj_feat=None,
                want_sumsq=False, c_pre=None, w16_pre=None, input_pad=0.0):
        from .field import _half_of, pad_twin
        h = h.contiguous()
        assert h.dtype == torch.float16 and h.shape == (N * T, 16)
        assert ray_sh.dtype == torch.float16 and ray_sh.shape == (N, 16) and ray_sh.is_contiguous()
        dev, M = h.device, N * T
        st = stream_of(h)
        w16 = w16_pre if w16_pre is not None else _half_of(cweights)
        obj16 = None
        if obj_feat is not None:
            obj16 = obj_feat.detach().reshape(-1).half().contiguous()
            assert obj16.numel() == 16 and w16.numel() == 64 * (48 + 64 * (int(num_layers) - 1) + 16)
        if c_pre is not None:
            assert c_pre.dtype == torch.float16 and c_pre.shape == (M, _C_WIDTH) and c_pre.is_contiguous()
            c = c_pre
        else:
            c = torch.empty(M, _C_WIDTH, dtype=torch.float16, device=dev)
            args = (ptr(h), ptr(ray_sh), T, ptr(w16), M, 64, int(num_layers), int(activation), ptr(c), _C_WIDTH, ptr(obj16))
            fn, extra = pad_twin("foc_color_head_forward", input_pad, obj16 is not None)
            check(fn(*args, *extra, st), "color_head_forward")
        sigma = torch.empty(M, dtype=torch.float32, device=dev)
        trans = torch.empty(M, dtype=torch.float32, device=dev)
        weights = torch.empty(M, dtype=torch.float32, device=dev)
        ws = torch.empty(N, dtype=torch.float32, device=dev)
        depth = torch.empty(N, dtype=torch.float32, device=dev)
        image = torch.empty(N, 3, dtype=torch.float32, device=dev)
        sumsq = torch.empty(N, dtype=torch.float32, device=dev) if want_sumsq else None
        check(lib.foc_fixed_tail_forward(ptr(h), ptr(c), ptr(nears), ptr(fars), ptr(noise), ptr(bg_ray), float(bg_scalar), N, T, float(density_scale),
                                         float(thresh), ptr(sigma), ptr(trans), ptr(weights), ptr(ws), ptr(depth), ptr(image), _C_WIDTH, ptr(sumsq), st),
              "fixed_tail_forward")
        empty = torch.empty(0, device=dev)
        ctx.bg_grad = bg_ray is not None and ctx.needs_input_grad[6]
        ctx.save_for_backward(h, w16, sigma, trans, weights, c, ray_sh, nears, fars, noise if noise is not None else empty,
                              bg_ray if bg_ray is not None else empty, obj16 if obj16 is not None else empty, ws if ctx.bg_grad else empty)
        ctx.flags = (noise is not None, bg_ray is not None, obj16 is not None, obj_feat.dtype if obj_feat is not None else None,
                     tuple(obj_feat.shape) if obj_feat is not None else None)
        ctx.dims = (N, T, float(density_scale), float(thresh), float(bg_scalar), int(num_layers), int(activation), float(input_pad))
        ctx.mark_non_differentiable(sigma, weights, c)
        ctx.set_materialize_grads(False)
        if want_sumsq:
            return image, ws, depth, sigma, weights, c, sumsq
        return image, ws, depth, sigma, weights, c

    @staticmethod
    def backward(ctx, g_image, g_ws, g_depth, _g_sigma, _g_weights, _g_c, g_sumsq=None):
        from .backend import _scratch
        from .field import pad_twin
        h, w16, sigma, trans, weights, c, ray_sh, nears, fars, noise, bg_ray, obj16, ws = ctx.saved_tensors
        has_noise, has_bg, has_obj, obj_dtype, obj_shape = ctx.flags
        obj16 = obj16 if has_obj else None
        N, T, ds, thresh, bg_scalar, num_layers, activation, input_pad = ctx.dims
        noise = noise if has_noise else None
        bg_ray = bg_ray if has_bg else None
        dev, M = h.device, N * T
        st = stream_of(h)
        g_image = g_image.contiguous().float() if g_image is not None else torch.zeros(N, 3, dtype=torch.float32, device=dev)
        g_ws = g_ws.contiguous().float() if g_ws is not None else None
        g_depth = g_depth.contiguous().float() if g_depth is not None else None
        g_sumsq = g_sumsq.contiguous().float() if g_sumsq is not None else None
        grad_c = torch.empty_like(c)
        grad_h0 = torch.empty(M, dtype=torch.float16, device=dev)
        check(lib.foc_fixed_tail_backward(ptr(g_image), ptr(g_ws), ptr(g_depth), ptr(c), ptr(sigma), ptr(trans), ptr(weights), ptr(nears), ptr(fars),
                                          ptr(noise), ptr(bg_ray), bg_scalar, N, T, ds, thresh, ptr(grad_c), ptr(grad_h0), _C_WIDTH, ptr(g_sumsq), st),
              "fixed_tail_backward")
        grad_h = torch.empty_like(h)
        g_w = torch.empty_like(w16)
        wsb = _scratch.get("ffmlp_ws", lib.foc_ffmlp_backward_workspace_bytes(48 if has_obj else 32, 64, num_layers), dev)
        g_obj32 = torch.empty(16, dtype=torch.float32, device=dev) if has_obj and ctx.needs_input_grad[14] else None
        args = (ptr(grad_c), ptr(h), ptr(ray_sh), T, ptr(grad_h0), ptr(w16), M, 64, num_layers, activation, ptr(grad_h), ptr(g_w), ptr(wsb),
                wsb.numel(), _C_WIDTH, ptr(obj16), ptr(g_obj32))
        fn, extra = pad_twin("foc_color_head_backward", input_pad, has_obj)
        check(fn(*args, *extra, st), "color_head_backward")
        g_obj = g_obj32.to(obj_dtype).view(obj_shape) if g_obj32 is not None else None
        g_bg = g_image * (1 - ws).unsqueeze(-1) if ctx.bg_grad else None
        return (grad_h, g_w, None, None, None, None, g_bg) + (None,) * 7 + (g_obj, None, None, None, None)


class _masked_norm(Function):

    @staticmethod
    def forward(ctx, sumsq, outside):
        crit = torch.sqrt((sumsq * outside).sum())
        ctx.save_for_backward(crit, outside)
        return crit

    @staticmethod
    def backward(ctx, g):
        crit, outside = ctx.saved_tensors
        coef = torch.where(crit > 0, g / (2 * crit), torch.zeros_like(crit))
        return outside * coef, None


def _background(bg_color, N, dev):
    if bg_color is None:
        return None, 1.0
    if torch.is_tensor(bg_color):
        if bg_color.numel() > 1:
            return bg_color.to(dev, torch.float32).expand(N, 3).contiguous(), 0.0
        return None, float(bg_color)
    return None, float(bg_color)


def render_fixed_steps(model, rays_o, rays_d, yolo_details=None, num_steps=512, bg_color=None, perturb=False, weight_thresh=1e-10,
                       return_fields=None, _out=None, **kwargs):
    import time
    if return_fields is None:
        return_fields = not model.training
    t_start = time.time()
    prefix = rays_o.shape[:-1]
    rays_o = rays_o.contiguous().view(-1, 3).float()
    rays_d = rays_d.contiguous().view(-1, 3).float()
    N, T = rays_o.shape[0], int(num_steps)
    dev = rays_o.device
    aabb = model.aabb_train if model.training else model.aabb_infer
    nears, fars = raymarching.near_far_from_aabb(rays_o, rays_d, aabb, model.min_near)
    noise = torch.rand(N * T, dtype=torch.float32, device=dev) if perturb else None
    from .field import field_plan, field_infer
    plan = field_plan(model)
    if getattr(model, "bg_radius", 0) > 0:
        bg_color = model._background_colour(rays_o, rays_d, bg_color)
    want_tail = plan.tail and model.training and torch.is_grad_enabled()
    fused_infer = not torch.is_grad_enabled() and plan.infer
    rb = ray_block_default() if fused_infer else 0
    enc_in, _, ray_sh = fixed_sample(rays_o, rays_d, nears, fars, aabb, noise, T, model.bound, want_ray_sh=True) if want_tail else \
        fixed_sample(rays_o, rays_d, nears, fars, aabb, noise, T, model.bound, ray_block=rb) + (None,)

    if fused_infer:
        obj_feat = model.encode_object_feature(yolo_details, dev) if plan.uses_object_feature else None
        sigma, rgb = field_infer(model, enc_in, rays_d, dir_div=T, dir_block=rb, obj_feat=obj_feat)
        bg_ray, bg_scalar = _background(bg_color, N, dev)
        direct = (_out is not None and _out[0].dtype == torch.float32 and _out[1].dtype == torch.float32 and _out[0].is_contiguous()
                  and _out[1].is_contiguous() and _out[0].numel() == N and _out[1].numel() == 3 * N and _out[0].device == dev)
        depth, image = (_out[0].view(N), _out[1].view(N, 3)) if direct else (torch.empty(N, dtype=torch.float32, device=dev),
                                                                              torch.empty(N, 3, dtype=torch.float32, device=dev))
        weights_sum = torch.empty(N, dtype=torch.float32, device=dev)
        rgb_masked = densities = None
        if return_fields:
            if direct and len(_out) == 4 and all(t.dtype == torch.float32 and t.is_contiguous() and t.device == dev for t in _out[2:]) \
                    and _out[2].numel() == N * T and _out[3].numel() == 3 * N * T and rb:
                densities, rgb_masked = _out[2].view(N * T), _out[3].view(N * T, 3)
            else:
                rgb_masked = torch.empty(N * T, 3, dtype=torch.float32, device=dev)
                densities = torch.empty(N * T, dtype=torch.float32, device=dev) if rb else None
        check(lib.foc_fixed_render_inference(ptr(sigma), ptr(rgb), ptr(nears), ptr(fars), ptr(noise), ptr(bg_ray), float(bg_scalar), N, T,
                                             float(model.density_scale), float(weight_thresh), ptr(image), ptr(depth), ptr(weights_sum), ptr(rgb_masked),
                                             rb, ptr(densities), stream_of(sigma)), "fixed_render_inference")
        t_mid = time.time()
        results = {'depth': depth.view(*prefix), 'image': image.view(*prefix, 3), 'weights_sum': weights_sum, 'criterion_outside_mask': None,
                   'timing': [t_mid - t_start, time.time() - t_mid]}
        if return_fields:
            results['densities'] = (densities if rb else sigma).view(N, T, 1)
            results['rgbs'] = rgb_masked.view(N, T, 3)
        return results

    enc = model.encoder
    from .field import hashgrid_mlp, fused_mlp
    c_pre = obj_feat = None
    cweights = fused_mlp(model, "color_net").weights if want_tail else None
    with torch.autocast("cuda", dtype=torch.float16):
        if plan.uses_object_feature:
            obj_feat = model.encode_object_feature(yolo_details, dev)
        if plan.field:
            colour = wc16 = None
            if want_tail and plan.train_forward:
                from .field import _half_of
                wc16 = _half_of(cweights)
                colour = (wc16, plan.colour, ray_sh, T, _C_WIDTH, obj_feat, plan.colour_input_pad)
            h = hashgrid_mlp(enc, fused_mlp(model, "sigma_net"), enc_in, None, colour)
            if colour is not None:
                h, c_pre = h
        else:
            feats = grid_encode(enc_in, enc.embeddings, enc.offsets, enc.per_level_scale, enc.base_resolution, False, enc.gridtype_id,
                                enc.align_corners, enc.interp_id)
            h = fused_mlp(model, "sigma_net")(feats)
        if h.shape[1] != 16:
            raise RuntimeError("render_fixed_steps expects a 16-wide sigma head (1 + geo_feat_dim = 16)")
        fused_tail = want_tail
        want_crit = model.training and yolo_details is not None and yolo_details[0] is not None
        criterion_outside_mask = None
        if fused_tail:
            cn = fused_mlp(model, "color_net")
            bg_ray, bg_scalar = _background(bg_color, N, dev)
            outs = _render_tail.apply(h, cweights, ray_sh, nears, fars, noise, bg_ray, bg_scalar, N, T, model.density_scale, weight_thresh,
                                      cn.num_layers, cn.activation, obj_feat, want_crit and yolo_details[0].numel() == N, c_pre,
                                      wc16 if c_pre is not None else None, plan.colour_input_pad)
            image, weights_sum, depth, sigma, weights, c = outs[:6]
            if len(outs) == 7:
                criterion_outside_mask = _masked_norm.apply(outs[6], (~yolo_details[0].reshape(N)).to(torch.float32))
        else:
            weights, weights_sum, depth, sigma, cin = _density_head.apply(h, rays_d, nears, fars, noise, N, T, model.density_scale, obj_feat)
            if plan.colour_input_pad != 0:
                cin = torch.cat([cin[:, :-1], cin.new_full((cin.shape[0], 1), plan.colour_input_pad)], dim=1)
        if want_crit and criterion_outside_mask is None:
            from .activation import trunc_exp
            criterion_outside_mask = torch.norm(trunc_exp(h[:, 0]).view(N, T)[~yolo_details[0].squeeze(0)] - 0)
        if not fused_tail:
            c = fused_mlp(model, "color_net").forward_padded(cin)
    t_mid = time.time()

    if not fused_tail:
        bg_ray, bg_scalar = _background(bg_color, N, dev)
        image = _fixed_composite.apply(c, weights, bg_ray, bg_scalar, N, T, weight_thresh, weights_sum)

    results = {'depth': depth.view(*prefix), 'image': image.view(*prefix, 3), 'weights_sum': weights_sum,
               'criterion_outside_mask': criterion_outside_mask, 'timing': [t_mid - t_start, time.time() - t_mid]}
    if return_fields:
        from .head import rgb_head
        c16 = c.detach()
        if c16.shape[1] != 16:
            c16 = torch.nn.functional.pad(c16, (0, 16 - c16.shape[1]))
        rgb = rgb_head(c16) * (weights > weight_thresh).unsqueeze(-1)
        results['densities'] = sigma.view(N, T, 1)
        results['rgbs'] = rgb.view(N, T, 3)
    return results


@torch.no_grad()
def render_field4(model, rays_o, rays_d, num_steps=512, weight_thresh=1e-10, yolo_details=None, out=None, occupancy=None):
    from .field import field_plan, field_infer
    rays_o = rays_o.contiguous().view(-1, 3).float()
    rays_d = rays_d.contiguous().view(-1, 3).float()
    N, T = rays_o.shape[0], int(num_steps)
    dev = rays_o.device
    if out is None:
        out = torch.empty(N, T, 4, dtype=torch.float32, device=dev)
    assert out.shape == (N, T, 4) and out.dtype == torch.float32 and out.is_contiguous()
    plan = field_plan(model)
    if occupancy is not None:
        from .fixedcull import render_field4_culled
        return render_field4_culled(model, plan, rays_o, rays_d, T, weight_thresh, yolo_details, out, occupancy)
    if plan.infer and model.bg_radius <= 0:
        aabb = model.aabb_train if model.training else model.aabb_infer
        nears, fars = raymarching.near_far_from_aabb(rays_o, rays_d, aabb, model.min_near)
        rb = ray_block_default()
        enc_in, _ = fixed_sample(rays_o, rays_d, nears, fars, aabb, None, T, model.bound, ray_block=rb)
        obj_feat = model.encode_object_feature(yolo_details, dev) if plan.uses_object_feature else None
        sigma, rgb = field_infer(model, enc_in, rays_d, dir_div=T, dir_block=rb, obj_feat=obj_feat)
        check(lib.foc_fixed_field_pack(ptr(sigma), ptr(rgb), ptr(nears), ptr(fars), None, None, 1.0, N, T, float(model.density_scale),
                                       float(weight_thresh), None, None, None, ptr(out), rb, stream_of(sigma)), "fixed_field_pack")
        return out
    from .combine import pack_field4
    with torch.autocast("cuda", dtype=torch.float16):
        res = model.run(rays_o[None], rays_d[None], yolo_details, num_steps=T, upsample_steps=0, perturb=False, weight_thresh=weight_thresh,
                        return_fields=True)
    out.copy_(pack_field4(res['densities'], res['rgbs']))
    return out
```

include/focnerf.h:

```cpp
#ifndef FOCNERF_H
#define FOCNERF_H

#include <stdint.h>

#ifdef __cplusplus
extern "C" {
#endif

#define FOC_OK            0
#define FOC_E_INVALID     1
#define FOC_E_DTYPE       2
#define FOC_E_LAUNCH      3

#define FOC_F32 0
#define FOC_F16 1

#define FOC_ABI_VERSION 2
int         foc_abi_version(void);
const char *foc_last_error(void);
int foc_set_option(const char *name, int value);
int foc_get_option(const char *name, int *value);
int foc_guard_pick_device(int stream_is_null, int stream_device, int pointer_device, int current_device);
const char *foc_arch(void);

// ... 139 lines not shown
                             const int32_t *offsets, float weight,
                             uint32_t B, uint32_t D, uint32_t C, uint32_t L, float S, uint32_t H,
                             uint32_t gridtype, int align_corners, int dtype, void *stream);


int foc_freq_encode_forward(const float *inputs, uint32_t B, uint32_t D, uint32_t deg, uint32_t C,
                            float *outputs, void *stream);
int foc_freq_encode_backward(const float *grad, const float *outputs, uint32_t B, uint32_t D,
                             uint32_t deg, uint32_t C, float *grad_inputs, void *stream);


int foc_ffmlp_forward(const void *inputs, const void *weights, uint32_t B, uint32_t input_dim,
                      uint32_t output_dim, uint32_t hidden_dim, uint32_t num_layers,
                      uint32_t activation, uint32_t output_activation,
                      void *forward_buffer, void *outputs, void *stream);

int foc_ffmlp_inference(const void *inputs, const void *weights, uint32_t B, uint32_t input_dim,
                        uint32_t output_dim, uint32_t hidden_dim, uint32_t num_layers,
                        uint32_t activation, uint32_t output_activation,
                        void *inference_buffer, void *outputs, void *stream);

int foc_ffmlp_backward(const void *grad, const void *inputs, const void *weights,
                       const void *forward_buffer, uint32_t B, uint32_t input_dim,
                       uint32_t output_dim, uint32_t hidden_dim, uint32_t num_layers,
                       uint32_t activation, uint32_t output_activation, int calc_grad_inputs,
                       void *backward_buffer, void *grad_inputs, void *grad_weights,
                       void *workspace, uint64_t workspace_bytes, void *stream);
uint64_t foc_ffmlp_backward_workspace_bytes(uint32_t input_dim, uint32_t hidden_dim, uint32_t num_layers);

int foc_ffmlp_forward_planar(const void *inputs_planar, const void *weights, uint32_t B, uint32_t input_dim,
                             uint32_t output_dim, uint32_t hidden_dim, uint32_t num_layers,
                             uint32_t activation, uint32_t output_activation, void *outputs, void *stream);
int foc_ffmlp_backward_planar(const void *grad, const void *inputs_planar, const void *weights, uint32_t B,
                              uint32_t input_dim, uint32_t output_dim, uint32_t hidden_dim, uint32_t num_layers,
                              uint32_t activation, uint32_t output_activation, int calc_grad_inputs,
                              void *grad_inputs_planar, void *grad_weights, void *workspace, uint64_t workspace_bytes, void *stream);

int foc_nerf_field_inference(const void *enc, int enc_planar, const float *dirs, uint32_t dir_div,
                             uint32_t dir_block, uint32_t n_dirs, const void *sigma_weights, uint32_t sigma_layers, const void *color_weights,
                             uint32_t color_layers, uint32_t hidden_dim, uint32_t activation, uint32_t B,
                             float *sigma, float *rgb, const void *obj_feat, void *stream);
int foc_nerf_field_inference_pad(const void *enc, int enc_planar, const float *dirs, uint32_t dir_div,
                                 uint32_t dir_block, uint32_t n_dirs, const void *sigma_weights, uint32_t sigma_layers, const void *color_weights,
                                 uint32_t color_layers, uint32_t hidden_dim, uint32_t activation, uint32_t B,
                                 float *sigma, float *rgb, const void *obj_feat, float input_pad, void *stream);
int foc_nerf_field_inference_pad31(const void *enc, int enc_planar, const float *dirs, uint32_t dir_div,
                                   uint32_t dir_block, uint32_t n_dirs, const void *sigma_weights, uint32_t sigma_layers, const void *color_weights,
                                   uint32_t color_layers, uint32_t hidden_dim, uint32_t activation, uint32_t B,
                                   float *sigma, float *rgb, const void *obj_feat, float input_pad, void *stream);

int foc_color_head_forward(const void *h, const void *ray_sh, uint32_t samples_per_ray, const void *weights,
                           uint32_t B, uint32_t hidden_dim, uint32_t num_layers, uint32_t activation,
                           void *outputs, uint32_t out_width, const void *obj_feat, void *stream);
int foc_color_head_backward(const void *grad, const void *h, const void *ray_sh, uint32_t samples_per_ray,
                            const void *grad_h0, const void *weights, uint32_t B, uint32_t hidden_dim,
                            uint32_t num_layers, uint32_t activation, void *grad_h, void *grad_weights,
                            void *workspace, uint64_t workspace_bytes, uint32_t out_width, const void *obj_feat, float *grad_obj, void *stream);
int foc_color_head_forward_pad(const void *h, const void *ray_sh, uint32_t samples_per_ray, const void *weights,
                               uint32_t B, uint32_t hidden_dim, uint32_t num_layers, uint32_t activation,
                               void *outputs, uint32_t out_width, const void *obj_feat, float input_pad, void *stream);
int foc_color_head_backward_pad(const void *grad, const void *h, const void *ray_sh, uint32_t samples_per_ray,
                                const void *grad_h0, const void *weights, uint32_t B, uint32_t hidden_dim,
                                uint32_t num_layers, uint32_t activation, void *grad_h, void *grad_weights,
                                void *workspace, uint64_t workspace_bytes, uint32_t out_width, const void *obj_feat, float *grad_obj,
                                float input_pad, void *stream);
int foc_color_head_forward_pad31(const void *h, const void *ray_sh, uint32_t samples_per_ray, const void *weights,
                                 uint32_t B, uint32_t hidden_dim, uint32_t num_layers, uint32_t activation,
                                 void *outputs, uint32_t out_width, const void *obj_feat, float input_pad, void *stream);
int foc_color_head_backward_pad31(const void *grad, const void *h, const void *ray_sh, uint32_t samples_per_ray,
                                  const void *grad_h0, const void *weights, uint32_t B, uint32_t hidden_dim,
                                  uint32_t num_layers, uint32_t activation, void *grad_h, void *grad_weights,
                                  void *workspace, uint64_t workspace_bytes, uint32_t out_width, const void *obj_feat, float *grad_obj,
                                  float input_pad, void *stream);

int foc_field_forward_train(const void *planes, const void *sigma_weights, uint32_t sigma_layers, const void *ray_sh, uint32_t samples_per_ray,
                            const void *color_weights, uint32_t color_layers, uint32_t hidden_dim, uint32_t activation, uint32_t B,
                            void *h, void *c, uint32_t out_width, const void *obj_feat, void *stream);
int foc_field_forward_train_pad(const void *planes, const void *sigma_weights, uint32_t sigma_layers, const void *ray_sh, uint32_t samples_per_ray,
                                const void *color_weights, uint32_t color_layers, uint32_t hidden_dim, uint32_t activation, uint32_t B,
                                void *h, void *c, uint32_t out_width, const void *obj_feat, float input_pad, void *stream);
int foc_field_forward_train_pad31(const void *planes, const void *sigma_weights, uint32_t sigma_layers, const void *ray_sh, uint32_t samples_per_ray,
                                  const void *color_weights, uint32_t color_layers, uint32_t hidden_dim, uint32_t activation, uint32_t B,
                                  void *h, void *c, uint32_t out_width, const void *obj_feat, float input_pad, void *stream);

int foc_allocate_splitk(uint64_t size);
int foc_free_splitk(void);


int foc_combine_select(const float *dens, const float *rgb, float *max_dens, float *best_rgb,
                       uint64_t n, void *stream);

int foc_combine_pack_keys(const float *dens, uint32_t rank, uint64_t *keys, uint64_t n, void *stream);
int foc_combine_unpack(const uint64_t *keys, uint32_t rank, const float *rgb,
                       float *max_dens, float *masked_rgb, uint64_t n, void *stream);

int foc_composite_fixed_steps(const float *sigmas, const float *rgbs, const float *nears,
                              const float *fars, uint32_t N, uint32_t T, float bg,
                              float *image4, float *depth, void *stream);

#define FOC_COMBINE_MAX_OBJECTS 16

int foc_combine_select_composite(const float *const *fields4, uint32_t K, const float *nears, const float *fars,
                                 uint32_t N, uint32_t T, const float *bgs, uint32_t n_bg, float *image4, float *depth,
                                 float *merged4, void *stream);

int foc_combine_select4(const float *field4, float *acc4, uint64_t n, void *stream);

int foc_combine_select_composite_attr(const float *const *fields4, uint32_t K, const uint8_t *const *id_planes,
                                      const uint32_t *ids, uint32_t n_obj, const float *nears, const float *fars,
                                      uint32_t N, uint32_t T, const float *bgs, uint32_t n_bg, float *image4, float *depth,
                                      float *merged4, float *obj_weights, float *obj_depth, int32_t *instance,
                                      uint8_t *winner, void *stream);

int foc_combine_select4_ids(const float *field4, uint32_t id, float *acc4, uint8_t *acc_ids, uint64_t n, void *stream);

int foc_mo_select(const void *sigma_new, const void *feat_new, void *sigma_best, void *feat_best, uint64_t n,
                  uint32_t feat_width, uint32_t elem_bytes, void *stream);


int foc_fixed_sample(const float *rays_o, const float *rays_d, const float *nears, const float *fars,
                     const float *aabb, const float *noise, uint32_t N, uint32_t T, float bound,
                     float *xyzs, float *enc_in, void *ray_sh, uint32_t ray_block, void *stream);

int foc_fixed_head_forward(const void *h, const float *rays_d, const float *nears, const float *fars,
                           const float *noise, uint32_t N, uint32_t T, float density_scale,
                           float *sigma, float *trans, float *weights, float *weights_sum, float *depth,
                           void *cin, const void *obj_feat, uint32_t cin_width, void *stream);
int foc_fixed_head_backward(const void *h, const float *sigma, const float *trans, const float *nears,
                            const float *fars, const float *noise, const float *grad_w, const float *grad_ws,
                            const float *grad_depth, const void *grad_cin, uint32_t N, uint32_t T,
                            float density_scale, void *grad_h, uint32_t cin_width, void *stream);

int foc_fixed_tail_forward(const void *h, const void *c, const float *nears, const float *fars, const float *noise,
                           const float *bg_ray, float bg_scalar, uint32_t N, uint32_t T, float density_scale, float thresh,
                           float *sigma, float *trans, float *weights, float *weights_sum, float *depth, float *image,
                           uint32_t c_width, float *ray_sumsq, void *stream);
int foc_fixed_tail_backward(const float *grad_image, const float *grad_ws, const float *grad_depth, const void *c,
                            const float *sigma, const float *trans, const float *weights, const float *nears,
                            const float *fars, const float *noise, const float *bg_ray, float bg_scalar, uint32_t N,
                            uint32_t T, float density_scale, float thresh, void *grad_c, void *grad_h0, uint32_t c_width,
                            const float *grad_sumsq, void *stream);

int foc_occ_tail_forward(const void *h, const void *c, uint32_t c_width, const float *deltas, const int32_t *rays,
                         uint32_t M, uint32_t N, float T_thresh, float density_scale, const float *bg_ray, float bg_scalar,
                         const float *nears, const float *fars, float *weights_sum, float *image_raw, float *image,
                         float *depth, void *stream);
int foc_occ_tail_backward(const float *grad_image, const float *grad_ws, const void *h, const void *c, uint32_t c_width,
                          const float *deltas, const int32_t *rays, const int32_t *counter, const float *weights_sum,
                          const float *image_raw, uint32_t M, uint32_t N, float T_thresh, float density_scale,
                          const float *bg_ray, float bg_scalar, void *grad_c, void *grad_h0, void *stream);
int foc_occ_tail_forward_sumsq(const void *h, const void *c, uint32_t c_width, const float *deltas, const int32_t *rays,
                               uint32_t M, uint32_t N, float T_thresh, float density_scale, const float *bg_ray, float bg_scalar,
                               const float *nears, const float *fars, float *weights_sum, float *image_raw, float *image,
                               float *depth, float *ray_sumsq, void *stream);
int foc_occ_tail_backward_sumsq(const float *grad_image, const float *grad_ws, const void *h, const void *c, uint32_t c_width,
                                const float *deltas, const int32_t *rays, const int32_t *counter, const float *weights_sum,
                                const float *image_raw, uint32_t M, uint32_t N, float T_thresh, float density_scale,
                                const float *bg_ray, float bg_scalar, void *grad_c, void *grad_h0, const float *grad_sumsq, void *stream);

typedef struct FocOccTrainNode {
    uint32_t struct_bytes;
    uint32_t n_rays, max_steps, cascade, grid_size, cap, pad_align;
    float bound, dt_gamma, min_near;
    const float *rays_o, *rays_d, *aabb, *jitter;
    const uint8_t *bitfield;
    float *nears, *fars, *enc_in, *deltas;
    void *sh_rows;
    int32_t *rays, *counter, *march_scratch;
    uint32_t levels, base_resolution, gridtype, interp;
    int32_t align_corners, table_dtype;
    float per_level_scale_log2;
    const void *embeddings;
    const int32_t *offsets, *offsets_host;
    void *planes, *grid_workspace;
    uint64_t grid_workspace_bytes;
    uint32_t sigma_input_dim, sigma_hidden, sigma_layers, sigma_activation, sigma_output_activation;
    uint32_t color_hidden, color_layers, color_activation, c_width;
    const void *w_sigma, *w_color;
    void *h, *c;
    float T_thresh, density_scale, bg_scalar;
    const float *bg_ray;
    float *weights_sum, *image_raw, *image, *depth;
    int32_t precounted;
    const float *grad_image, *grad_ws;
    void *grad_c, *grad_h0, *grad_h, *grad_planes, *grad_w_color, *grad_w_sigma, *grad_embeddings, *mlp_workspace;
    uint64_t mlp_workspace_bytes;
} FocOccTrainNode;
int foc_occ_train_forward(const FocOccTrainNode *node, void *stream);
int foc_occ_train_backward(const FocOccTrainNode *node, void *stream);
int foc_occ_train_forward_pad31(const FocOccTrainNode *node, float input_pad, void *stream);
int foc_occ_train_backward_pad31(const FocOccTrainNode *node, float input_pad, void *stream);
typedef struct FocOccTrainObject {
    uint32_t struct_bytes;
    float input_pad;
    const void *obj_feat;
    float *ray_sumsq;
    const float *grad_sumsq;
    float *grad_obj;
} FocOccTrainObject;
int foc_occ_train_forward_obj(const FocOccTrainNode *node, const FocOccTrainObject *object, void *stream);
int foc_occ_train_backward_obj(const FocOccTrainNode *node, const FocOccTrainObject *object, void *stream);

int foc_view_tile_order(const float *rays_d, uint32_t N, uint32_t tile_h, uint32_t tile_w, int64_t *perm, void *state16,
                        void *stream);

int foc_fixed_composite_forward(const void *c, const float *weights, const float *bg_ray, float bg_scalar,
                                uint32_t N, uint32_t T, float thresh, float *image, void *stream);
int foc_fixed_composite_backward(const float *grad_image, const void *c, const float *weights,
                                 const float *bg_ray, float bg_scalar, uint32_t N, uint32_t T, float thresh,
                                 void *grad_c, float *grad_w, void *stream);

int foc_fixed_render_inference(const float *sigma, const float *rgb, const float *nears, const float *fars,
                               const float *noise, const float *bg_ray, float bg_scalar, uint32_t N, uint32_t T,
                               float density_scale, float thresh, float *image, float *depth, float *weights_sum,
                               float *rgb_masked, uint32_t ray_block, float *sigma_raymajor, void *stream);

int foc_fixed_field_pack(const float *sigma, const float *rgb, const float *nears, const float *fars,
                         const float *noise, const float *bg_ray, float bg_scalar, uint32_t N, uint32_t T,
                         float density_scale, float thresh, float *image, float *depth, float *weights_sum,
                         float *field4, uint32_t ray_block, void *stream);

uint64_t foc_fixed_cull_scratch_bytes(uint32_t N, uint32_t T);
int foc_fixed_cull(const float *rays_o, const float *rays_d, const float *nears, const float *fars, const float *aabb,
                   uint32_t N, uint32_t T, float bound, const uint8_t *bitfield, uint32_t cascade, uint32_t grid_size,
// ... 45 lines not shown
```

Before: 1.321 billion.

## Add lean fixed-step tail path with fused near/far sampling and compact h0 plane

Fuses the ray-AABB near/far computation into the fixed-step sample kernel, which removes a separate launch. The field forward kernel can now also write a compact plane holding only the h0 (density) channel. New lean tail forward and backward kernels read that plane and recompute per-sample sigma, transmittance and weights instead of storing and reloading them. The aim is to cut memory traffic and kernel launches in training, at the cost of extra recomputation and a new code path gated by an option and a maximum step count.

```diff
diff --git a/focnerf_amd/_lib.py b/focnerf_amd/_lib.py
--- a/focnerf_amd/_lib.py
+++ b/focnerf_amd/_lib.py
@@ -165,6 +165,11 @@
     "foc_color_head_forward_pad31": (i32, [c_vp, c_vp, u32, c_vp, u32, u32, u32, u32, c_vp, u32, c_vp, f32, c_vp]),
     "foc_color_head_backward_pad31": (i32, [c_vp, c_vp, c_vp, u32, c_vp, c_vp, u32, u32, u32, u32, c_vp, c_vp, c_vp, u64, u32, c_vp, c_vp, f32, c_vp]),
     "foc_field_forward_train_pad31": (i32, [c_vp, c_vp, u32, c_vp, u32, c_vp, u32, u32, u32, u32, c_vp, c_vp, u32, c_vp, f32, c_vp]),
+    "foc_field_forward_train_h0": (i32, [c_vp, c_vp, u32, c_vp, u32, c_vp, u32, u32, u32, u32, c_vp, c_vp, u32, c_vp, u32, f32, c_vp, c_vp]),
+    "foc_fixed_sample_nearfar": (i32, [c_vp, c_vp, c_vp, f32, c_vp, u32, u32, f32, c_vp, c_vp, c_vp, c_vp, c_vp, u32, c_vp]),
+    "foc_fixed_tail_lean_max_steps": (u32, []),
+    "foc_fixed_tail_forward_lean": (i32, [c_vp, c_vp, c_vp, c_vp, c_vp, c_vp, f32, u32, u32, f32, f32, c_vp, c_vp, c_vp, u32, c_vp, c_vp]),
+    "foc_fixed_tail_backward_lean": (i32, [c_vp, c_vp, c_vp, c_vp, c_vp, c_vp, c_vp, c_vp, c_vp, f32, u32, u32, f32, f32, c_vp, c_vp, u32, c_vp, c_vp]),
     "foc_fixed_composite_forward": (i32, [c_vp, c_vp, c_vp, f32, u32, u32, f32, c_vp, c_vp]),
     "foc_fixed_composite_backward": (i32, [c_vp, c_vp, c_vp, c_vp, f32, u32, u32, f32, c_vp, c_vp, c_vp]),
     "foc_sample_head_forward": (i32, [c_vp, c_vp, u64, c_vp, c_vp, c_vp, u32, c_vp]),
@@ -226,6 +231,19 @@
     return call
 
 
+def _with_h0_plane(plain, owner, n_plain, pad_mode):
+    def call(*args):
+        if len(args) == n_plain:
+            return plain(*args)
+        if len(args) != n_plain + 1:
+            raise TypeError(f"{call.__name__}: {n_plain} arguments, or {n_plain + 1} with the h0 plane before the stream (got {len(args)})")
+        *head, h0_plane, stream = args
+        if pad_mode == 0:
+            head.append(0.0)
+        return owner.foc_field_forward_train_h0(*head[:-1], pad_mode, head[-1], h0_plane, stream)
+    return call
+
+
 class _Lib:
 
     def __init__(self, cdll):
@@ -233,6 +251,10 @@
         for name, (_, args) in SIGNATURES.items():
             fn = getattr(cdll, name)
             setattr(self, name, _on_tensor_device(fn) if args and args[-1] is c_vp and not name.endswith("_bytes") else fn)
+        for mode, name in enumerate(("foc_field_forward_train", "foc_field_forward_train_pad", "foc_field_forward_train_pad31")):
+            call = _with_h0_plane(getattr(self, name), self, len(SIGNATURES[name][1]), mode)
+            call.__name__ = name
+            setattr(self, name, call)
 
 
 lib = _Lib(_load())
diff --git a/focnerf_amd/csrc/combine.hip b/focnerf_amd/csrc/combine.hip
--- a/focnerf_amd/csrc/combine.hip
+++ b/focnerf_amd/csrc/combine.hip
@@ -268,7 +268,7 @@
 static FocOptionRow foc_option_table[FOC_OPT_COUNT] = {
     {"FOC_MLP_BWD_FUSED", 1}, {"FOC_FIELD_FWD_FUSED", 1}, {"FOC_GB_MERGE_MAX_RES", 480}, {"FOC_GB_FACTORED", 1}, {"FOC_GB_TAIL_SPLIT", 16}, {"FOC_GRID_FUSE_SMALL", 1},
     {"FOC_GRID_PAIRS", 1}, {"FOC_GRID_FAST", 1}, {"FOC_MARCH_SERIAL", -1}, {"FOC_MARCH_RAYS_ROW_MAX", 131072}, {"FOC_OCC_MARCH_FORM", -1},
-    {"FOC_OCC_SAMPLE_MAJOR", 1}, {"FOC_OCC_FIELD_PIECE", 1 << 23}, {"FOC_DETERMINISTIC", 0},
+    {"FOC_OCC_SAMPLE_MAJOR", 1}, {"FOC_OCC_FIELD_PIECE", 1 << 23}, {"FOC_DETERMINISTIC", 0}, {"FOC_TAIL_LEAN", 1},
 };
 static int foc_option_parse(int which, const char *text) {
     if (which == FOC_OPT_OCC_MARCH_FORM) {
diff --git a/focnerf_amd/csrc/common.h b/focnerf_amd/csrc/common.h
--- a/focnerf_amd/csrc/common.h
+++ b/focnerf_amd/csrc/common.h
@@ -4,6 +4,7 @@
 #include <stdint.h>
 #include <stdio.h>
 #include <stdarg.h>
+#include <float.h>
 #include "../../include/focnerf.h"
 
 #define FOC_WAVE 64
@@ -25,6 +26,7 @@
     FOC_OPT_OCC_SAMPLE_MAJOR,
     FOC_OPT_OCC_FIELD_PIECE,
     FOC_OPT_DETERMINISTIC,
+    FOC_OPT_TAIL_LEAN,
     FOC_OPT_COUNT
 };
 int foc_opt(FocOpt which);
@@ -86,6 +88,30 @@
 
 __device__ __forceinline__ _Float16 foc_f2h(float v) { asm volatile("" : "+v"(v)); return (_Float16)v; }
 
+__device__ __forceinline__ void rm_near_far(float ox, float oy, float oz, float dx, float dy, float dz, float a0, float a1, float a2, float a3, float a4, float a5,
+                                            float min_near, float &near_out, float &far_out) {
+    const float rdx = 1 / dx, rdy = 1 / dy, rdz = 1 / dz;
+    float near = (a0 - ox) * rdx, far = (a3 - ox) * rdx, t;
+    if (near > far) { t = near; near = far; far = t; }
+    float near_y = (a1 - oy) * rdy, far_y = (a4 - oy) * rdy;
+    if (near_y > far_y) { t = near_y; near_y = far_y; far_y = t; }
+    bool miss = (near > far_y || near_y > far);
+    if (!miss) {
+        if (near_y > near) near = near_y;
+        if (far_y < far) far = far_y;
+        float near_z = (a2 - oz) * rdz, far_z = (a5 - oz) * rdz;
+        if (near_z > far_z) { t = near_z; near_z = far_z; far_z = t; }
+        miss = (near > far_z || near_z > far);
+        if (!miss) {
+            if (near_z > near) near = near_z;
+            if (far_z < far) far = far_z;
+            if (near < min_near) near = min_near;
+        }
+    }
+    near_out = miss ? FLT_MAX : near;
+    far_out = miss ? FLT_MAX : far;
+}
+
 __global__ static void __launch_bounds__(256) k_foc_zero(uint32_t *__restrict__ p, uint64_t n_words) {
     for (uint64_t i = (uint64_t)blockIdx.x * 256 + threadIdx.x; i < n_words; i += (uint64_t)gridDim.x * 256) p[i] = 0u;
 }
diff --git a/focnerf_amd/csrc/field_fwd.hip b/focnerf_amd/csrc/field_fwd.hip
--- a/focnerf_amd/csrc/field_fwd.hip
+++ b/focnerf_amd/csrc/field_fwd.hip
@@ -14,7 +14,7 @@
 template <int NLS, int NLC, bool RELU>
 __global__ void __launch_bounds__(MLP_BLOCK, FF_MIN_WAVES) k_field_fwd_train(const _Float16 *__restrict__ planes, const _Float16 *__restrict__ w_sigma,
                                                                const _Float16 *__restrict__ w_color, _Float16 *__restrict__ h_out,
-                                                               _Float16 *__restrict__ c_out, uint32_t B, MlpHead hd) {
+                                                               _Float16 *__restrict__ c_out, uint32_t B, MlpHead hd, _Float16 *__restrict__ h0_out) {
     constexpr int HIDDEN = 64, MT = 2, KC = 4, KS0 = 2;
     constexpr int FS = MT * KS0 + (NLS - 1) * MT * KC + KC;
     constexpr int FC = MT * KS0 + (NLC - 1) * MT * KC + KC;
@@ -92,6 +92,7 @@
 #endif
             *reinterpret_cast<ff_u2 *>(h_out + row_raw * 16 + 4 * h) = ff_u2{P0, P1};
             *reinterpret_cast<ff_u2 *>(h_out + row_raw * 16 + 8 + 4 * h) = ff_u2{P2, P3};
+            if (h0_out && h == 0) reinterpret_cast<uint16_t *>(h0_out)[row_raw] = (uint16_t)(P0 & 0xffffu);
         }
         const uint32_t nxt = h == 0 ? P2 : 0u;
         const ff_u2 s02 = __builtin_amdgcn_permlane32_swap(P0, P2, false, false);
@@ -147,7 +148,7 @@
 }
 
 template <int NLS, int NLC, bool RELU>
-static int ff_launch(const void *planes, const void *w_sigma, const void *w_color, void *h, void *c, uint32_t B, const MlpHead &hd, hipStream_t st) {
+static int ff_launch(const void *planes, const void *w_sigma, const void *w_color, void *h, void *c, uint32_t B, const MlpHead &hd, void *h0, hipStream_t st) {
     auto kern = k_field_fwd_train<NLS, NLC, RELU>;
     const size_t lds = (size_t)((4 + (NLS - 1) * 8 + 4) + (4 + (NLC - 1) * 8 + 4)) * 1024 + 256;
     if (lds > 64 * 1024) (void)hipFuncSetAttribute(reinterpret_cast<const void *>(kern), hipFuncAttributeMaxDynamicSharedMemorySize, (int)lds);
@@ -161,19 +162,19 @@
     const uint32_t cap = ff_num_cus() * (uint32_t)resident;
     if (grid > cap) grid = cap;
     hipLaunchKernelGGL(kern, dim3(grid), dim3(MLP_BLOCK), lds, st, (const _Float16 *)planes, (const _Float16 *)w_sigma, (const _Float16 *)w_color,
-                       (_Float16 *)h, (_Float16 *)c, B, hd);
+                       (_Float16 *)h, (_Float16 *)c, B, hd, (_Float16 *)h0);
     FOC_CHECK_LAUNCH("field_forward_train");
     return FOC_OK;
 }
 
 template <int NLS, int NLC>
-static int ff_launch_act(const void *planes, const void *w_sigma, const void *w_color, void *h, void *c, uint32_t B, int relu, const MlpHead &hd, hipStream_t st) {
-    return relu ? ff_launch<NLS, NLC, true>(planes, w_sigma, w_color, h, c, B, hd, st) : ff_launch<NLS, NLC, false>(planes, w_sigma, w_color, h, c, B, hd, st);
+static int ff_launch_act(const void *planes, const void *w_sigma, const void *w_color, void *h, void *c, uint32_t B, int relu, const MlpHead &hd, void *h0, hipStream_t st) {
+    return relu ? ff_launch<NLS, NLC, true>(planes, w_sigma, w_color, h, c, B, hd, h0, st) : ff_launch<NLS, NLC, false>(planes, w_sigma, w_color, h, c, B, hd, h0, st);
 }
 
 static int field_forward_train(const void *planes, const void *sigma_weights, uint32_t sigma_layers, const void *ray_sh, uint32_t samples_per_ray,
                                const void *color_weights, uint32_t color_layers, uint32_t hidden_dim, uint32_t activation, uint32_t B, void *h, void *c,
-                               uint32_t out_width, const void *obj_feat, float input_pad, bool pad31, void *stream) {
+                               uint32_t out_width, const void *obj_feat, float input_pad, bool pad31, void *h0_plane, void *stream) {
     FocDeviceGuard foc_guard_(stream, planes);
     if (B == 0) return FOC_OK;
     FOC_REQUIRE(planes && sigma_weights && ray_sh && color_weights && h && c, FOC_E_INVALID, "field_forward_train: null pointer");
@@ -186,11 +187,11 @@
     const int relu = activation == FOC_ACT_RELU;
     hipStream_t st = (hipStream_t)stream;
     switch (sigma_layers * 10 + color_layers) {
-        case 12: return ff_launch_act<1, 2>(planes, sigma_weights, color_weights, h, c, B, relu, hd, st);
-        case 13: return ff_launch_act<1, 3>(planes, sigma_weights, color_weights, h, c, B, relu, hd, st);
-        case 22: return ff_launch_act<2, 2>(planes, sigma_weights, color_weights, h, c, B, relu, hd, st);
-        case 23: return ff_launch_act<2, 3>(planes, sigma_weights, color_weights, h, c, B, relu, hd, st);
-        case 33: return ff_launch_act<3, 3>(planes, sigma_weights, color_weights, h, c, B, relu, hd, st);
+        case 12: return ff_launch_act<1, 2>(planes, sigma_weights, color_weights, h, c, B, relu, hd, h0_plane, st);
+        case 13: return ff_launch_act<1, 3>(planes, sigma_weights, color_weights, h, c, B, relu, hd, h0_plane, st);
+        case 22: return ff_launch_act<2, 2>(planes, sigma_weights, color_weights, h, c, B, relu, hd, h0_plane, st);
+        case 23: return ff_launch_act<2, 3>(planes, sigma_weights, color_weights, h, c, B, relu, hd, h0_plane, st);
+        case 33: return ff_launch_act<3, 3>(planes, sigma_weights, color_weights, h, c, B, relu, hd, h0_plane, st);
         default: foc_set_error("field_forward_train: layer counts (%u, %u) are not built (1/2, 1/3, 2/2, 2/3, 3/3)", sigma_layers, color_layers); return FOC_E_INVALID;
     }
 }
@@ -201,21 +202,31 @@
                             const void *color_weights, uint32_t color_layers, uint32_t hidden_dim, uint32_t activation, uint32_t B, void *h, void *c,
                             uint32_t out_width, const void *obj_feat, void *stream) {
     return field_forward_train(planes, sigma_weights, sigma_layers, ray_sh, samples_per_ray, color_weights, color_layers, hidden_dim, activation, B, h, c,
-                               out_width, obj_feat, 0.0f, false, stream);
+                               out_width, obj_feat, 0.0f, false, nullptr, stream);
 }
 
 int foc_field_forward_train_pad(const void *planes, const void *sigma_weights, uint32_t sigma_layers, const void *ray_sh, uint32_t samples_per_ray,
                                 const void *color_weights, uint32_t color_layers, uint32_t hidden_dim, uint32_t activation, uint32_t B, void *h, void *c,
                                 uint32_t out_width, const void *obj_feat, float input_pad, void *stream) {
     return field_forward_train(planes, sigma_weights, sigma_layers, ray_sh, samples_per_ray, color_weights, color_layers, hidden_dim, activation, B, h, c,
-                               out_width, obj_feat, input_pad, false, stream);
+                               out_width, obj_feat, input_pad, false, nullptr, stream);
 }
 
 int foc_field_forward_train_pad31(const void *planes, const void *sigma_weights, uint32_t sigma_layers, const void *ray_sh, uint32_t samples_per_ray,
                                   const void *color_weights, uint32_t color_layers, uint32_t hidden_dim, uint32_t activation, uint32_t B, void *h, void *c,
                                   uint32_t out_width, const void *obj_feat, float input_pad, void *stream) {
     return field_forward_train(planes, sigma_weights, sigma_layers, ray_sh, samples_per_ray, color_weights, color_layers, hidden_dim, activation, B, h, c,
-                               out_width, obj_feat, input_pad, true, stream);
-}
-
-}
+                               out_width, obj_feat, input_pad, true, nullptr, stream);
+}
+
+int foc_field_forward_train_h0(const void *planes, const void *sigma_weights, uint32_t sigma_layers, const void *ray_sh, uint32_t samples_per_ray,
+                               const void *color_weights, uint32_t color_layers, uint32_t hidden_dim, uint32_t activation, uint32_t B, void *h, void *c,
+                               uint32_t out_width, const void *obj_feat, uint32_t pad_mode, float input_pad, void *h0_plane, void *stream) {
+    FOC_REQUIRE(pad_mode <= 2, FOC_E_INVALID, "field_forward_train_h0: pad_mode must be 0 (no pad), 1 (column 47) or 2 (column 31), got %u", pad_mode);
+    FOC_REQUIRE(pad_mode != 0 || input_pad == 0.0f, FOC_E_INVALID, "field_forward_train_h0: pad_mode 0 takes input_pad 0");
+    FOC_REQUIRE(B == 0 || h0_plane, FOC_E_INVALID, "field_forward_train_h0: null h0_plane");
+    return field_forward_train(planes, sigma_weights, sigma_layers, ray_sh, samples_per_ray, color_weights, color_layers, hidden_dim, activation, B, h, c,
+                               out_width, obj_feat, input_pad, pad_mode == 2, h0_plane, stream);
+}
+
+}
diff --git a/focnerf_amd/csrc/fixedstep.hip b/focnerf_amd/csrc/fixedstep.hip
--- a/focnerf_amd/csrc/fixedstep.hip
+++ b/focnerf_amd/csrc/fixedstep.hip
@@ -32,10 +32,12 @@
     o[15] = 0.59004358992664352f * x * (-x2 + 3.0f * y2);
 }
 
+template <bool NEARFAR>
 __global__ void __launch_bounds__(256) k_fs_sample(const float *__restrict__ rays_o, const float *__restrict__ rays_d, const float *__restrict__ nears,
                                                    const float *__restrict__ fars, const float *__restrict__ aabb, const float *__restrict__ noise,
                                                    uint32_t N, uint32_t T, float bound, float *__restrict__ xyzs, float *__restrict__ enc_in,
-                                                   _Float16 *__restrict__ ray_sh, uint32_t ray_block) {
+                                                   _Float16 *__restrict__ ray_sh, uint32_t ray_block, float min_near, float *__restrict__ nears_out,
+                                                   float *__restrict__ fars_out) {
     const uint64_t total = ray_block ? (uint64_t)((N + FS_RAY_BLOCK - 1) / FS_RAY_BLOCK) * FS_RAY_BLOCK * T : (uint64_t)N * T;
     const FsBox box = fs_box(aabb);
     const float two_b = 2 * bound;
@@ -51,15 +53,22 @@
         } else {
             n = (uint32_t)(s / T); i = (uint32_t)(s - (uint64_t)n * T);
         }
-        const FsGeom g = fs_geom(nears, fars, n, T);
+        const float ox = rays_o[n * 3], oy = rays_o[n * 3 + 1], oz = rays_o[n * 3 + 2], dx = rays_d[n * 3], dy = rays_d[n * 3 + 1], dz = rays_d[n * 3 + 2];
+        FsGeom g;
+        if (NEARFAR) {
+            float near, far;
+            rm_near_far(ox, oy, oz, dx, dy, dz, box.a0, box.a1, box.a2, box.a3, box.a4, box.a5, min_near, near, far);
+            if (i == 0 && own) { nears_out[n] = near; fars_out[n] = far; }
+            g = fs_geom_of(near, far, T);
+        } else g = fs_geom(nears, fars, n, T);
         const float z = fs_z(g, i, T, noise, (uint64_t)n * T + i);
         float x, y, w;
-        fs_point(rays_o[n * 3], rays_o[n * 3 + 1], rays_o[n * 3 + 2], rays_d[n * 3], rays_d[n * 3 + 1], rays_d[n * 3 + 2], z, box, x, y, w);
+        fs_point(ox, oy, oz, dx, dy, dz, z, box, x, y, w);
         if (xyzs) { xyzs[s * 3] = x; xyzs[s * 3 + 1] = y; xyzs[s * 3 + 2] = w; }
         if (enc_in) { enc_in[s * 3] = fs_norm(x, bound, two_b); enc_in[s * 3 + 1] = fs_norm(y, bound, two_b); enc_in[s * 3 + 2] = fs_norm(w, bound, two_b); }
         if (ray_sh && i == 0 && own) {
             float sh[16];
-            fs_sh16(rays_d[n * 3], rays_d[n * 3 + 1], rays_d[n * 3 + 2], sh);
+            fs_sh16(dx, dy, dz, sh);
             h8 lo, hi;
 #pragma unroll
             for (int k = 0; k < 8; k++) { lo[k] = foc_f2h(sh[k]); hi[k] = foc_f2h(sh[8 + k]); }
@@ -249,7 +258,34 @@
     }
 }
 
+
+struct FsTailSample { float sigma, z, delta, ex, alpha, om; };
 template <bool NOISE>
+__device__ __forceinline__ FsTailSample fs_tail_sample(const FsGeom &g, uint32_t i, uint32_t ic, uint32_t T, bool valid, float h0, float u0, float u1,
+                                                       float density_scale) {
+    FsTailSample p;
+    p.sigma = expf(h0);
+    p.z = fs_zu<NOISE>(g, ic, T, u0);
+    p.delta = g.sample_dist;
+    if (i + 1 < T) p.delta = fs_zu<NOISE>(g, i + 1, T, u1) - p.z;
+    p.ex = expf((-p.delta * density_scale) * p.sigma);
+    p.alpha = valid ? 1 - p.ex : 0.0f;
+    p.om = valid ? (1 - p.alpha + 1e-15f) : 1.0f;
+    return p;
+}
+__device__ __forceinline__ float fs_tail_trans(float om, uint32_t lane, float Tc, float &chunk) {
+    const float P = wave_incl_prod(om, (int)lane);
+    float Pex = __shfl_up(P, 1, 64);
+    if (lane == 0) Pex = 1.0f;
+    chunk = __shfl(P, 63, 64);
+    return Tc * Pex;
+}
+__device__ __forceinline__ float fs_tail_oz(const FsGeom &g, float z) {
+    float oz = (z - g.near) / g.span;
+    return oz < 0.0f ? 0.0f : (oz > 1.0f ? 1.0f : oz);
+}
+
+template <bool NOISE, bool LEAN>
 __global__ void __launch_bounds__(256) k_fs_tail_fwd(const _Float16 *__restrict__ h, const _Float16 *__restrict__ c, const float *__restrict__ nears,
                                                      const float *__restrict__ fars, const float *__restrict__ noise, const float *__restrict__ bg_ray,
                                                      float bg_scalar, uint32_t N, uint32_t T, float density_scale, float thresh,
@@ -266,32 +302,24 @@
         const bool valid = i < T;
         const uint32_t ic = valid ? i : T - 1;
         const uint64_t s = (uint64_t)n * T + ic;
-        const _Float16 h0 = h[s * 16];
+        const _Float16 h0 = LEAN ? h[s] : h[s * 16];
         const uint2 raw = *reinterpret_cast<const uint2 *>(c + s * c_ld);
         float u0 = 0.0f, u1 = 0.0f;
         if (NOISE) { u0 = noise[s]; u1 = noise[(uint64_t)n * T + min(ic + 1u, T - 1u)]; }
-        const float sigma = expf((float)h0);
-        const float z = fs_zu<NOISE>(g, ic, T, u0);
-        float delta = g.sample_dist;
-        if (i + 1 < T) delta = fs_zu<NOISE>(g, i + 1, T, u1) - z;
-        const float alpha = valid ? 1 - expf((-delta * density_scale) * sigma) : 0.0f;
-        const float om = valid ? (1 - alpha + 1e-15f) : 1.0f;
-        const float P = wave_incl_prod(om, (int)lane);
-        float Pex = __shfl_up(P, 1, 64);
-        if (lane == 0) Pex = 1.0f;
-        const float Tb = Tc * Pex;
-        const float w = alpha * Tb;
+        const FsTailSample p = fs_tail_sample<NOISE>(g, i, ic, T, valid, (float)h0, u0, u1, density_scale);
+        float chunk;
+        const float Tb = fs_tail_trans(p.om, lane, Tc, chunk);
+        const float w = p.alpha * Tb;
         if (valid) {
-            sigma_out[s] = sigma; trans_out[s] = Tb; weights_out[s] = w;
-            float oz = (z - g.near) / g.span;
-            oz = oz < 0.0f ? 0.0f : (oz > 1.0f ? 1.0f : oz);
-            ws += w; dp += w * oz; sq = fmaf(sigma, sigma, sq);
+            if (!LEAN) { sigma_out[s] = p.sigma; trans_out[s] = Tb; weights_out[s] = w; }
+            const float oz = fs_tail_oz(g, p.z);
+            ws += w; dp += w * oz; sq = fmaf(p.sigma, p.sigma, sq);
             if (w > thresh) {
                 const _Float16 *cc = reinterpret_cast<const _Float16 *>(&raw);
                 r += w * fs_sigmoid_h((float)cc[0]); gg += w * fs_sigmoid_h((float)cc[1]); b += w * fs_sigmoid_h((float)cc[2]);
             }
         }
-        Tc *= __shfl(P, 63, 64);
+        Tc *= chunk;
     }
     ws = wave_sum(ws); dp = wave_sum(dp); r = wave_sum(r); gg = wave_sum(gg); b = wave_sum(b);
     if (ray_sumsq) {
@@ -356,6 +384,85 @@
         const float om = 1 - alpha + 1e-15f;
         float oz = (z - g.near) / g.span;
         oz = oz < 0.0f ? 0.0f : (oz > 1.0f ? 1.0f : oz);
+        float gi = gw + gws;
+        if (gdp != 0.0f) gi += gdp * oz;
+        const float gw_i = valid ? gi * (alpha * Tb) : 0.0f;
+        const float incl = wave_suffix_incl_sum(gw_i, (int)lane);
+        const float S_i = S_carry + (incl - gw_i);
+        const float dalpha = gi * Tb - S_i / om;
+        float dsigma = dalpha * (delta * density_scale) * ex;
+        if (gsq2 != 0.0f) dsigma = fmaf(gsq2, sigma, dsigma);
+        const float dh0 = dsigma * fminf(fmaxf(sigma, e_lo), e_hi);
+        if (valid) grad_h0[s] = foc_f2h(dh0);
+        S_carry += __shfl(incl, 0, 64);
+    }
+}
+
+#define FS_LEAN_MAX_T 4096u
+template <bool NOISE>
+__global__ void __launch_bounds__(256) k_fs_tail_bwd_lean(const float *__restrict__ grad_image, const float *__restrict__ grad_ws, const float *__restrict__ grad_depth,
+                                                          const _Float16 *__restrict__ c, const _Float16 *__restrict__ h0_in, const float *__restrict__ nears,
+                                                          const float *__restrict__ fars, const float *__restrict__ noise, const float *__restrict__ bg_ray,
+                                                          float bg_scalar, uint32_t N, uint32_t T, float density_scale, float thresh, _Float16 *__restrict__ grad_c,
+                                                          _Float16 *__restrict__ grad_h0, uint32_t c_ld, const float *__restrict__ grad_sumsq) {
+    const uint32_t lane = threadIdx.x & 63;
+    const uint32_t n = blockIdx.x * 4 + (threadIdx.x >> 6);
+    if (n >= N) return;
+    const FsGeom g = fs_geom(nears, fars, n, T);
+    const float gws = grad_ws ? grad_ws[n] : 0.0f, gdp = grad_depth ? grad_depth[n] : 0.0f;
+    const float gsq2 = grad_sumsq ? 2.0f * grad_sumsq[n] : 0.0f;
+    const float g0 = grad_image[n * 3], g1 = grad_image[n * 3 + 1], g2 = grad_image[n * 3 + 2];
+    const float b0 = bg_ray ? bg_ray[n * 3] : bg_scalar, b1 = bg_ray ? bg_ray[n * 3 + 1] : bg_scalar, b2 = bg_ray ? bg_ray[n * 3 + 2] : bg_scalar;
+    const float e_lo = expf(fs_opaque(-15.0f)), e_hi = expf(fs_opaque(15.0f));
+    const uint32_t n_chunks = (T + 63) / 64;
+    float Tc_of = 1.0f;
+    {
+        float Tc = 1.0f;
+        for (uint32_t cidx = 0; cidx + 1 < n_chunks; cidx++) {
+            const uint32_t i = cidx * 64 + lane;
+            const uint64_t s = (uint64_t)n * T + i;
+            const _Float16 h0 = h0_in[s];
+            float u0 = 0.0f, u1 = 0.0f;
+            if (NOISE) { u0 = noise[s]; u1 = noise[(uint64_t)n * T + min(i + 1u, T - 1u)]; }
+            const FsTailSample p = fs_tail_sample<NOISE>(g, i, i, T, true, (float)h0, u0, u1, density_scale);
+            float chunk;
+            (void)fs_tail_trans(p.om, lane, Tc, chunk);
+            Tc *= chunk;
+            if (lane == cidx + 1) Tc_of = Tc;
+        }
+    }
+    float S_carry = 0.0f;
+    for (uint32_t cidx = n_chunks; cidx-- > 0;) {
+        const uint32_t i = cidx * 64 + lane;
+        const bool valid = i < T;
+        const uint32_t ic = valid ? i : T - 1;
+        const uint64_t s = (uint64_t)n * T + ic;
+        const _Float16 h0 = h0_in[s];
+        const uint2 raw = *reinterpret_cast<const uint2 *>(c + s * c_ld);
+        float u0 = 0.0f, u1 = 0.0f;
+        if (NOISE) { u0 = noise[s]; u1 = noise[(uint64_t)n * T + min(ic + 1u, T - 1u)]; }
+        const FsTailSample p = fs_tail_sample<NOISE>(g, i, ic, T, valid, (float)h0, u0, u1, density_scale);
+        float chunk;
+        const float Tb = fs_tail_trans(p.om, lane, __shfl(Tc_of, (int)cidx, 64), chunk);
+        const float sigma = p.sigma, w = p.alpha * Tb;
+        float gw = -(g0 * b0 + g1 * b1 + g2 * b2);
+        h8 o0, o1;
+#pragma unroll
+        for (int k = 0; k < 8; k++) { o0[k] = (_Float16)0; o1[k] = (_Float16)0; }
+        if (w > thresh) {
+            const _Float16 *cc = reinterpret_cast<const _Float16 *>(&raw);
+            const float y0 = fs_sigmoid_h((float)cc[0]), y1 = fs_sigmoid_h((float)cc[1]), y2 = fs_sigmoid_h((float)cc[2]);
+            gw += g0 * y0 + g1 * y1 + g2 * y2;
+            o0[0] = foc_f2h(g0 * w * y0 * (1 - y0)); o0[1] = foc_f2h(g1 * w * y1 * (1 - y1)); o0[2] = foc_f2h(g2 * w * y2 * (1 - y2));
+        }
+        if (valid) {
+            if (c_ld == 4u) *reinterpret_cast<uint2 *>(grad_c + s * 4) = *reinterpret_cast<const uint2 *>(&o0);
+            else { h8 *dst = reinterpret_cast<h8 *>(grad_c + s * 16); dst[0] = o0; dst[1] = o1; }
+        }
+        const float delta = p.delta, ex = p.ex;
+        const float alpha = 1 - ex;
+        const float om = 1 - alpha + 1e-15f;
+        const float oz = fs_tail_oz(g, p.z);
         float gi = gw + gws;
         if (gdp != 0.0f) gi += gdp * oz;
         const float gw_i = valid ? gi * (alpha * Tb) : 0.0f;
@@ -494,9 +601,23 @@
     FOC_REQUIRE(T >= 2, FOC_E_INVALID, "fixed_sample: T must be >= 2");
     FOC_REQUIRE(ray_block == 0 || ray_block == FS_RAY_BLOCK, FOC_E_INVALID, "fixed_sample: ray_block must be 0 (ray-major) or %u (got %u)", FS_RAY_BLOCK, ray_block);
     const uint64_t rows = ray_block ? (uint64_t)foc_div_up(N, FS_RAY_BLOCK) * FS_RAY_BLOCK * T : (uint64_t)N * T;
-    hipLaunchKernelGGL(k_fs_sample, dim3(foc_grid_1d(rows, 256, 256 * 16)), dim3(256), 0, (hipStream_t)stream, rays_o, rays_d, nears, fars, aabb,
-                       noise, N, T, bound, xyzs, enc_in, (_Float16 *)ray_sh, ray_block);
+    hipLaunchKernelGGL(k_fs_sample<false>, dim3(foc_grid_1d(rows, 256, 256 * 16)), dim3(256), 0, (hipStream_t)stream, rays_o, rays_d, nears, fars, aabb,
+                       noise, N, T, bound, xyzs, enc_in, (_Float16 *)ray_sh, ray_block, 0.0f, (float *)nullptr, (float *)nullptr);
     FOC_CHECK_LAUNCH("fixed_sample");
+    return FOC_OK;
+}
+
+int foc_fixed_sample_nearfar(const float *rays_o, const float *rays_d, const float *aabb, float min_near, const float *noise, uint32_t N, uint32_t T,
+                             float bound, float *nears, float *fars, float *xyzs, float *enc_in, void *ray_sh, uint32_t ray_block, void *stream) {
+    FocDeviceGuard foc_guard_(stream, rays_o);
+    if (N == 0) return FOC_OK;
+    FOC_REQUIRE(rays_o && rays_d && nears && fars && aabb && (xyzs || enc_in), FOC_E_INVALID, "fixed_sample_nearfar: null pointer");
+    FOC_REQUIRE(T >= 2, FOC_E_INVALID, "fixed_sample_nearfar: T must be >= 2");
+    FOC_REQUIRE(ray_block == 0 || ray_block == FS_RAY_BLOCK, FOC_E_INVALID, "fixed_sample_nearfar: ray_block must be 0 (ray-major) or %u (got %u)", FS_RAY_BLOCK, ray_block);
+    const uint64_t rows = ray_block ? (uint64_t)foc_div_up(N, FS_RAY_BLOCK) * FS_RAY_BLOCK * T : (uint64_t)N * T;
+    hipLaunchKernelGGL(k_fs_sample<true>, dim3(foc_grid_1d(rows, 256, 256 * 16)), dim3(256), 0, (hipStream_t)stream, rays_o, rays_d, (const float *)nullptr,
+                       (const float *)nullptr, aabb, noise, N, T, bound, xyzs, enc_in, (_Float16 *)ray_sh, ray_block, min_near, nears, fars);
+    FOC_CHECK_LAUNCH("fixed_sample_nearfar");
     return FOC_OK;
 }
 
@@ -559,7 +680,7 @@
     FOC_REQUIRE(c_width == 16 || c_width == 4, FOC_E_INVALID, "fixed_tail_forward: c_width must be 16 or 4 (got %u)", c_width);
     FOC_REQUIRE(h && c && nears && fars && sigma && trans && weights && weights_sum && depth && image, FOC_E_INVALID, "fixed_tail_forward: null pointer");
     FOC_REQUIRE(T >= 2, FOC_E_INVALID, "fixed_tail_forward: T must be >= 2");
-    auto kern = noise ? k_fs_tail_fwd<true> : k_fs_tail_fwd<false>;
+    auto kern = noise ? k_fs_tail_fwd<true, false> : k_fs_tail_fwd<false, false>;
     hipLaunchKernelGGL(kern, dim3(foc_div_up(N, 4)), dim3(256), 0, (hipStream_t)stream, (const _Float16 *)h, (const _Float16 *)c, nears, fars, noise,
                        bg_ray, bg_scalar, N, T, density_scale, thresh, sigma, trans, weights, weights_sum, depth, image, c_width, ray_sumsq);
     FOC_CHECK_LAUNCH("fixed_tail_forward");
@@ -580,6 +701,42 @@
                        trans, weights, nears, fars, noise, bg_ray, bg_scalar, N, T, density_scale, thresh, (_Float16 *)grad_c, (_Float16 *)grad_h0, c_width,
                        grad_sumsq);
     FOC_CHECK_LAUNCH("fixed_tail_backward");
+    return FOC_OK;
+}
+
+uint32_t foc_fixed_tail_lean_max_steps(void) { return FS_LEAN_MAX_T; }
+
+int foc_fixed_tail_forward_lean(const void *h0, const void *c, const float *nears, const float *fars, const float *noise, const float *bg_ray,
+                                float bg_scalar, uint32_t N, uint32_t T, float density_scale, float thresh, float *weights_sum, float *depth, float *image,
+                                uint32_t c_width, float *ray_sumsq, void *stream) {
+    FocDeviceGuard foc_guard_(stream, h0);
+    if (N == 0) return FOC_OK;
+    FOC_REQUIRE(c_width == 16 || c_width == 4, FOC_E_INVALID, "fixed_tail_forward_lean: c_width must be 16 or 4 (got %u)", c_width);
+    FOC_REQUIRE(h0 && c && nears && fars && weights_sum && depth && image, FOC_E_INVALID, "fixed_tail_forward_lean: null pointer");
+    FOC_REQUIRE(T >= 2, FOC_E_INVALID, "fixed_tail_forward_lean: T must be >= 2");
+    auto kern = noise ? k_fs_tail_fwd<true, true> : k_fs_tail_fwd<false, true>;
+    hipLaunchKernelGGL(kern, dim3(foc_div_up(N, 4)), dim3(256), 0, (hipStream_t)stream, (const _Float16 *)h0, (const _Float16 *)c, nears, fars, noise,
+                       bg_ray, bg_scalar, N, T, density_scale, thresh, (float *)nullptr, (float *)nullptr, (float *)nullptr, weights_sum, depth, image, c_width,
+                       ray_sumsq);
+    FOC_CHECK_LAUNCH("fixed_tail_forward_lean");
+    return FOC_OK;
+}
+
+int foc_fixed_tail_backward_lean(const float *grad_image, const float *grad_ws, const float *grad_depth, const void *c, const void *h0, const float *nears,
+                                 const float *fars, const float *noise, const float *bg_ray, float bg_scalar, uint32_t N, uint32_t T, float density_scale,
+                                 float thresh, void *grad_c, void *grad_h0, uint32_t c_width, const float *grad_sumsq, void *stream) {
+    FocDeviceGuard foc_guard_(stream, grad_image);
+    if (N == 0) return FOC_OK;
+    FOC_REQUIRE(c_width == 16 || c_width == 4, FOC_E_INVALID, "fixed_tail_backward_lean: c_width must be 16 or 4 (got %u)", c_width);
+    FOC_REQUIRE(grad_image && c && h0 && nears && fars && grad_c && grad_h0, FOC_E_INVALID, "fixed_tail_backward_lean: null pointer");
+    FOC_REQUIRE(T >= 2, FOC_E_INVALID, "fixed_tail_backward_lean: T must be >= 2");
+    FOC_REQUIRE(T <= FS_LEAN_MAX_T, FOC_E_INVALID, "fixed_tail_backward_lean: T must be <= %u (got %u): longer rays take foc_fixed_tail_forward / _backward",
+                FS_LEAN_MAX_T, T);
+    auto kern = noise ? k_fs_tail_bwd_lean<true> : k_fs_tail_bwd_lean<false>;
+    hipLaunchKernelGGL(kern, dim3(foc_div_up(N, 4)), dim3(256), 0, (hipStream_t)stream, grad_image, grad_ws, grad_depth, (const _Float16 *)c,
+                       (const _Float16 *)h0, nears, fars, noise, bg_ray, bg_scalar, N, T, density_scale, thresh, (_Float16 *)grad_c, (_Float16 *)grad_h0,
+                       c_width, grad_sumsq);
+    FOC_CHECK_LAUNCH("fixed_tail_backward_lean");
     return FOC_OK;
 }
 
diff --git a/focnerf_amd/csrc/fs_common.h b/focnerf_amd/csrc/fs_common.h
--- a/focnerf_amd/csrc/fs_common.h
+++ b/focnerf_amd/csrc/fs_common.h
@@ -8,13 +8,16 @@
     return (uint64_t)(n / FS_RAY_BLOCK) * FS_RAY_BLOCK * T + (uint64_t)i * FS_RAY_BLOCK + n % FS_RAY_BLOCK;
 }
 
-__device__ __forceinline__ FsGeom fs_geom(const float *__restrict__ nears, const float *__restrict__ fars, uint32_t n, uint32_t T) {
+__device__ __forceinline__ FsGeom fs_geom_of(float near, float far, uint32_t T) {
     FsGeom g;
-    g.near = nears[n]; g.far = fars[n];
+    g.near = near; g.far = far;
     g.span = g.far - g.near;
     g.sample_dist = g.span / (float)T;
     g.step = 1.0f / (float)(T - 1);
     return g;
+}
+__device__ __forceinline__ FsGeom fs_geom(const float *__restrict__ nears, const float *__restrict__ fars, uint32_t n, uint32_t T) {
+    return fs_geom_of(nears[n], fars[n], T);
 }
 __device__ __forceinline__ float fs_z(const FsGeom &g, uint32_t i, uint32_t T, const float *__restrict__ noise, uint64_t s) {
     const float lin = (i < T / 2) ? (g.step * (float)i) : fmaf(-g.step, (float)(T - 1 - i), 1.0f);
diff --git a/focnerf_amd/csrc/raymarching.hip b/focnerf_amd/csrc/raymarching.hip
--- a/focnerf_amd/csrc/raymarching.hip
+++ b/focnerf_amd/csrc/raymarching.hip
@@ -14,30 +14,6 @@
     x = (x | (x >> 8)) & 0xff0000ffu;
     x = (x | (x >> 16)) & 0x0000ffffu;
     return x;
-}
-
-__device__ __forceinline__ void rm_near_far(float ox, float oy, float oz, float dx, float dy, float dz, float a0, float a1, float a2, float a3, float a4, float a5,
-                                            float min_near, float &near_out, float &far_out) {
-    const float rdx = 1 / dx, rdy = 1 / dy, rdz = 1 / dz;
-    float near = (a0 - ox) * rdx, far = (a3 - ox) * rdx, t;
-    if (near > far) { t = near; near = far; far = t; }
-    float near_y = (a1 - oy) * rdy, far_y = (a4 - oy) * rdy;
-    if (near_y > far_y) { t = near_y; near_y = far_y; far_y = t; }
-    bool miss = (near > far_y || near_y > far);
-    if (!miss) {
-        if (near_y > near) near = near_y;
-        if (far_y < far) far = far_y;
-        float near_z = (a2 - oz) * rdz, far_z = (a5 - oz) * rdz;
-        if (near_z > far_z) { t = near_z; near_z = far_z; far_z = t; }
-        miss = (near > far_z || near_z > far);
-        if (!miss) {
-            if (near_z > near) near = near_z;
-            if (far_z < far) far = far_z;
-            if (near < min_near) near = min_near;
-        }
-    }
-    near_out = miss ? FLT_MAX : near;
-    far_out = miss ? FLT_MAX : far;
 }
 
 __global__ void __launch_bounds__(256) k_near_far_from_aabb(const float *__restrict__ rays_o, const float *__restrict__ rays_d,
diff --git a/focnerf_amd/field.py b/focnerf_amd/field.py
--- a/focnerf_amd/field.py
+++ b/focnerf_amd/field.py
@@ -211,17 +211,20 @@
         if ticket is None:
             _gridencoder.grid_encode_forward(x, emb, offsets, enc, B, 3, 2, L, S, H, None, gridtype, align_corners, interp)
         h = torch.empty(B, 16, device=x.device, dtype=torch.half)
-        c = None
+        c = h0 = None
         if colour is not None:
             from ._lib import ptr, stream_of, check
             cweights, cshape, ray_sh, T, c_width, obj_feat = colour[:6]
             pad = float(colour[6]) if len(colour) > 6 else 0.0
+            h0 = torch.empty(B, device=x.device, dtype=torch.half) if len(colour) > 7 and colour[7] else None
             wc = _half_of(cweights)
             obj16 = obj_feat.detach().reshape(-1).half().contiguous() if obj_feat is not None else None
             c = torch.empty(B, c_width, device=x.device, dtype=torch.half)
             args = (ptr(enc), ptr(w), sigma.num_layers, ptr(ray_sh), int(T), ptr(wc), int(cshape.num_layers), 64, int(sigma.activation), B, ptr(h),
                     ptr(c), int(c_width), ptr(obj16))
             fn, extra = pad_twin("foc_field_forward_train", pad, obj16 is not None)
+            if h0 is not None:
+                extra = extra + (ptr(h0),)
             check(fn(*args, *extra, stream_of(enc)), "field_forward_train")
         else:
             _ffmlp.ffmlp_forward_planar(enc, w, B, sigma.input_dim, 16, sigma.hidden_dim, sigma.num_layers, sigma.activation, sigma.output_activation, h)
@@ -231,13 +234,16 @@
             ctx.ticket = ticket
         if c is None:
             return h
+        ctx.set_materialize_grads(False)
+        if h0 is not None:
+            ctx.mark_non_differentiable(c, h0)
+            return h, c, h0
         ctx.mark_non_differentiable(c)
-        ctx.set_materialize_grads(False)
         return h, c
 
     @staticmethod
     @custom_bwd(device_type="cuda")
-    def backward(ctx, grad_h, _grad_c=None):
+    def backward(ctx, grad_h, _grad_c=None, _grad_h0=None):
         x, emb, w, offsets, enc = ctx.saved_tensors
         grid, sigma, B, L = ctx.cfg
         if grad_h is None:
@@ -286,6 +292,6 @@
     h = _hashgrid_mlp.apply(xn, encoder.embeddings, mlp.weights, encoder.offsets, encoder.spec(), MlpShape.of(mlp), mlp.training and torch.is_grad_enabled(),
                             colour)
     if colour is not None:
-        h, c = h
-        return h.view(prefix + [16]), c
+        h, *rest = h
+        return (h.view(prefix + [16]), *rest)
     return h.view(prefix + [16])
diff --git a/focnerf_amd/fixedstep.py b/focnerf_amd/fixedstep.py
--- a/focnerf_amd/fixedstep.py
+++ b/focnerf_amd/fixedstep.py
@@ -30,6 +30,29 @@
     if want_ray_sh:
         return enc_in, xyzs, ray_sh
     return enc_in, xyzs
+
+
+def fixed_sample_nearfar(rays_o, rays_d, aabb, min_near, noise, T, bound):
+    N, dev = rays_o.shape[0], rays_o.device
+    aabb = aabb.to(dev, torch.float32).contiguous()
+    nears = torch.empty(N, dtype=torch.float32, device=dev)
+    fars = torch.empty(N, dtype=torch.float32, device=dev)
+    enc_in = torch.empty(N * T, 3, dtype=torch.float32, device=dev)
+    ray_sh = torch.empty(N, 16, dtype=torch.float16, device=dev)
+    check(lib.foc_fixed_sample_nearfar(ptr(rays_o), ptr(rays_d), ptr(aabb), float(min_near), ptr(noise), N, T, float(bound), ptr(nears), ptr(fars), None,
+                                       ptr(enc_in), ptr(ray_sh), 0, stream_of(rays_o)), "fixed_sample_nearfar")
+    return nears, fars, enc_in, ray_sh
+
+
+_lean_max_steps = None
+
+
+def tail_lean(T):
+    global _lean_max_steps
+    from ._lib import get_option
+    if _lean_max_steps is None:
+        _lean_max_steps = int(lib.foc_fixed_tail_lean_max_steps())
+    return get_option("FOC_TAIL_LEAN") != 0 and T <= _lean_max_steps
 
 
 def ray_sh_rows(rays_d):
@@ -126,7 +149,7 @@
 
     @staticmethod
     def forward(ctx, h, cweights, ray_sh, nears, fars, noise, bg_ray, bg_scalar, N, T, density_scale, thresh, num_layers, activation, obj_feat=None,
-                want_sumsq=False, c_pre=None, w16_pre=None, input_pad=0.0):
+                want_sumsq=False, c_pre=None, w16_pre=None, input_pad=0.0, h0_plane=None):
         from .field import _half_of, pad_twin
         h = h.contiguous()
         assert h.dtype == torch.float16 and h.shape == (N * T, 16)
@@ -146,24 +169,36 @@
             args = (ptr(h), ptr(ray_sh), T, ptr(w16), M, 64, int(num_layers), int(activation), ptr(c), _C_WIDTH, ptr(obj16))
             fn, extra = pad_twin("foc_color_head_forward", input_pad, obj16 is not None)
             check(fn(*args, *extra, st), "color_head_forward")
-        sigma = torch.empty(M, dtype=torch.float32, device=dev)
-        trans = torch.empty(M, dtype=torch.float32, device=dev)
-        weights = torch.empty(M, dtype=torch.float32, device=dev)
+        lean = h0_plane is not None
+        if lean:
+            assert c_pre is not None and h0_plane.dtype == torch.float16 and h0_plane.shape == (M,) and h0_plane.is_contiguous()
         ws = torch.empty(N, dtype=torch.float32, device=dev)
         depth = torch.empty(N, dtype=torch.float32, device=dev)
         image = torch.empty(N, 3, dtype=torch.float32, device=dev)
         sumsq = torch.empty(N, dtype=torch.float32, device=dev) if want_sumsq else None
-        check(lib.foc_fixed_tail_forward(ptr(h), ptr(c), ptr(nears), ptr(fars), ptr(noise), ptr(bg_ray), float(bg_scalar), N, T, float(density_scale),
-                                         float(thresh), ptr(sigma), ptr(trans), ptr(weights), ptr(ws), ptr(depth), ptr(image), _C_WIDTH, ptr(sumsq), st),
-              "fixed_tail_forward")
         empty = torch.empty(0, device=dev)
+        if lean:
+            sigma = trans = weights = None
+            check(lib.foc_fixed_tail_forward_lean(ptr(h0_plane), ptr(c), ptr(nears), ptr(fars), ptr(noise), ptr(bg_ray), float(bg_scalar), N, T,
+                                                  float(density_scale), float(thresh), ptr(ws), ptr(depth), ptr(image), _C_WIDTH, ptr(sumsq), st),
+                  "fixed_tail_forward_lean")
+            fields = (h0_plane, empty, empty)
+        else:
+            sigma = torch.empty(M, dtype=torch.float32, device=dev)
+            trans = torch.empty(M, dtype=torch.float32, device=dev)
+            weights = torch.empty(M, dtype=torch.float32, device=dev)
+            check(lib.foc_fixed_tail_forward(ptr(h), ptr(c), ptr(nears), ptr(fars), ptr(noise), ptr(bg_ray), float(bg_scalar), N, T, float(density_scale),
+                                             float(thresh), ptr(sigma), ptr(trans), ptr(weights), ptr(ws), ptr(depth), ptr(image), _C_WIDTH, ptr(sumsq), st),
+                  "fixed_tail_forward")
+            fields = (sigma, trans, weights)
+        ctx.lean = lean
         ctx.bg_grad = bg_ray is not None and ctx.needs_input_grad[6]
-        ctx.save_for_backward(h, w16, sigma, trans, weights, c, ray_sh, nears, fars, noise if noise is not None else empty,
+        ctx.save_for_backward(h, w16, *fields, c, ray_sh, nears, fars, noise if noise is not None else empty,
                               bg_ray if bg_ray is not None else empty, obj16 if obj16 is not None else empty, ws if ctx.bg_grad else empty)
         ctx.flags = (noise is not None, bg_ray is not None, obj16 is not None, obj_feat.dtype if obj_feat is not None else None,
                      tuple(obj_feat.shape) if obj_feat is not None else None)
         ctx.dims = (N, T, float(density_scale), float(thresh), float(bg_scalar), int(num_layers), int(activation), float(input_pad))
-        ctx.mark_non_differentiable(sigma, weights, c)
+        ctx.mark_non_differentiable(*((c,) if lean else (sigma, weights, c)))
         ctx.set_materialize_grads(False)
         if want_sumsq:
             return image, ws, depth, sigma, weights, c, sumsq
@@ -187,9 +222,14 @@
         g_sumsq = g_sumsq.contiguous().float() if g_sumsq is not None else None
         grad_c = torch.empty_like(c)
         grad_h0 = torch.empty(M, dtype=torch.float16, device=dev)
-        check(lib.foc_fixed_tail_backward(ptr(g_image), ptr(g_ws), ptr(g_depth), ptr(c), ptr(sigma), ptr(trans), ptr(weights), ptr(nears), ptr(fars),
-                                          ptr(noise), ptr(bg_ray), bg_scalar, N, T, ds, thresh, ptr(grad_c), ptr(grad_h0), _C_WIDTH, ptr(g_sumsq), st),
-              "fixed_tail_backward")
+        if ctx.lean:
+            check(lib.foc_fixed_tail_backward_lean(ptr(g_image), ptr(g_ws), ptr(g_depth), ptr(c), ptr(sigma), ptr(nears), ptr(fars), ptr(noise),
+                                                   ptr(bg_ray), bg_scalar, N, T, ds, thresh, ptr(grad_c), ptr(grad_h0), _C_WIDTH, ptr(g_sumsq), st),
+                  "fixed_tail_backward_lean")
+        else:
+            check(lib.foc_fixed_tail_backward(ptr(g_image), ptr(g_ws), ptr(g_depth), ptr(c), ptr(sigma), ptr(trans), ptr(weights), ptr(nears), ptr(fars),
+                                              ptr(noise), ptr(bg_ray), bg_scalar, N, T, ds, thresh, ptr(grad_c), ptr(grad_h0), _C_WIDTH, ptr(g_sumsq), st),
+                  "fixed_tail_backward")
         grad_h = torch.empty_like(h)
         g_w = torch.empty_like(w16)
         wsb = _scratch.get("ffmlp_ws", lib.foc_ffmlp_backward_workspace_bytes(48 if has_obj else 32, 64, num_layers), dev)
@@ -200,7 +240,7 @@
         check(fn(*args, *extra, st), "color_head_backward")
         g_obj = g_obj32.to(obj_dtype).view(obj_shape) if g_obj32 is not None else None
         g_bg = g_image * (1 - ws).unsqueeze(-1) if ctx.bg_grad else None
-        return (grad_h, g_w, None, None, None, None, g_bg) + (None,) * 7 + (g_obj, None, None, None, None)
+        return (grad_h, g_w, None, None, None, None, g_bg) + (None,) * 7 + (g_obj, None, None, None, None, None)
 
 
 class _masked_norm(Function):
@@ -240,17 +280,21 @@
     N, T = rays_o.shape[0], int(num_steps)
     dev = rays_o.device
     aabb = model.aabb_train if model.training else model.aabb_infer
-    nears, fars = raymarching.near_far_from_aabb(rays_o, rays_d, aabb, model.min_near)
     noise = torch.rand(N * T, dtype=torch.float32, device=dev) if perturb else None
     from .field import field_plan, field_infer
     plan = field_plan(model)
+    want_tail = plan.tail and model.training and torch.is_grad_enabled()
+    lean = want_tail and tail_lean(T)
+    nears, fars = raymarching.near_far_from_aabb(rays_o, rays_d, aabb, model.min_near) if not lean else (None, None)
     if getattr(model, "bg_radius", 0) > 0:
         bg_color = model._background_colour(rays_o, rays_d, bg_color)
-    want_tail = plan.tail and model.training and torch.is_grad_enabled()
     fused_infer = not torch.is_grad_enabled() and plan.infer
     rb = ray_block_default() if fused_infer else 0
-    enc_in, _, ray_sh = fixed_sample(rays_o, rays_d, nears, fars, aabb, noise, T, model.bound, want_ray_sh=True) if want_tail else \
-        fixed_sample(rays_o, rays_d, nears, fars, aabb, noise, T, model.bound, ray_block=rb) + (None,)
+    if lean:
+        nears, fars, enc_in, ray_sh = fixed_sample_nearfar(rays_o, rays_d, aabb, model.min_near, noise, T, model.bound)
+    else:
+        enc_in, _, ray_sh = fixed_sample(rays_o, rays_d, nears, fars, aabb, noise, T, model.bound, want_ray_sh=True) if want_tail else \
+            fixed_sample(rays_o, rays_d, nears, fars, aabb, noise, T, model.bound, ray_block=rb) + (None,)
 
     if fused_infer:
         obj_feat = model.encode_object_feature(yolo_details, dev) if plan.uses_object_feature else None
@@ -282,7 +326,7 @@
 
     enc = model.encoder
     from .field import hashgrid_mlp, fused_mlp
-    c_pre = obj_feat = None
+    c_pre = h0_plane = obj_feat = None
     cweights = fused_mlp(model, "color_net").weights if want_tail else None
     with torch.autocast("cuda", dtype=torch.float16):
         if plan.uses_object_feature:
@@ -292,10 +336,11 @@
             if want_tail and plan.train_forward:
                 from .field import _half_of
                 wc16 = _half_of(cweights)
-                colour = (wc16, plan.colour, ray_sh, T, _C_WIDTH, obj_feat, plan.colour_input_pad)
+                colour = (wc16, plan.colour, ray_sh, T, _C_WIDTH, obj_feat, plan.colour_input_pad, lean and not return_fields)
             h = hashgrid_mlp(enc, fused_mlp(model, "sigma_net"), enc_in, None, colour)
             if colour is not None:
-                h, c_pre = h
+                h, c_pre, *rest = h
+                h0_plane = rest[0] if rest else None
         else:
             feats = grid_encode(enc_in, enc.embeddings, enc.offsets, enc.per_level_scale, enc.base_resolution, False, enc.gridtype_id,
                                 enc.align_corners, enc.interp_id)
@@ -310,7 +355,7 @@
             bg_ray, bg_scalar = _background(bg_color, N, dev)
             outs = _render_tail.apply(h, cweights, ray_sh, nears, fars, noise, bg_ray, bg_scalar, N, T, model.density_scale, weight_thresh,
                                       cn.num_layers, cn.activation, obj_feat, want_crit and yolo_details[0].numel() == N, c_pre,
-                                      wc16 if c_pre is not None else None, plan.colour_input_pad)
+                                      wc16 if c_pre is not None else None, plan.colour_input_pad, h0_plane)
             image, weights_sum, depth, sigma, weights, c = outs[:6]
             if len(outs) == 7:
                 criterion_outside_mask = _masked_norm.apply(outs[6], (~yolo_details[0].reshape(N)).to(torch.float32))
diff --git a/include/focnerf.h b/include/focnerf.h
--- a/include/focnerf.h
+++ b/include/focnerf.h
@@ -245,6 +245,10 @@
 int foc_field_forward_train_pad31(const void *planes, const void *sigma_weights, uint32_t sigma_layers, const void *ray_sh, uint32_t samples_per_ray,
                                   const void *color_weights, uint32_t color_layers, uint32_t hidden_dim, uint32_t activation, uint32_t B,
                                   void *h, void *c, uint32_t out_width, const void *obj_feat, float input_pad, void *stream);
+int foc_field_forward_train_h0(const void *planes, const void *sigma_weights, uint32_t sigma_layers, const void *ray_sh, uint32_t samples_per_ray,
+                               const void *color_weights, uint32_t color_layers, uint32_t hidden_dim, uint32_t activation, uint32_t B,
+                               void *h, void *c, uint32_t out_width, const void *obj_feat, uint32_t pad_mode, float input_pad,
+                               void *h0_plane, void *stream);
 
 int foc_allocate_splitk(uint64_t size);
 int foc_free_splitk(void);
@@ -284,6 +288,9 @@
 int foc_fixed_sample(const float *rays_o, const float *rays_d, const float *nears, const float *fars,
                      const float *aabb, const float *noise, uint32_t N, uint32_t T, float bound,
                      float *xyzs, float *enc_in, void *ray_sh, uint32_t ray_block, void *stream);
+int foc_fixed_sample_nearfar(const float *rays_o, const float *rays_d, const float *aabb, float min_near, const float *noise,
+                             uint32_t N, uint32_t T, float bound, float *nears, float *fars, float *xyzs, float *enc_in,
+                             void *ray_sh, uint32_t ray_block, void *stream);
 
 int foc_fixed_head_forward(const void *h, const float *rays_d, const float *nears, const float *fars,
                            const float *noise, uint32_t N, uint32_t T, float density_scale,
@@ -303,6 +310,14 @@
                             const float *fars, const float *noise, const float *bg_ray, float bg_scalar, uint32_t N,
                             uint32_t T, float density_scale, float thresh, void *grad_c, void *grad_h0, uint32_t c_width,
                             const float *grad_sumsq, void *stream);
+uint32_t foc_fixed_tail_lean_max_steps(void);
+int foc_fixed_tail_forward_lean(const void *h0, const void *c, const float *nears, const float *fars, const float *noise,
+                                const float *bg_ray, float bg_scalar, uint32_t N, uint32_t T, float density_scale, float thresh,
+                                float *weights_sum, float *depth, float *image, uint32_t c_width, float *ray_sumsq, void *stream);
+int foc_fixed_tail_backward_lean(const float *grad_image, const float *grad_ws, const float *grad_depth, const void *c,
+                                 const void *h0, const float *nears, const float *fars, const float *noise, const float *bg_ray,
+                                 float bg_scalar, uint32_t N, uint32_t T, float density_scale, float thresh, void *grad_c,
+                                 void *grad_h0, uint32_t c_width, const float *grad_sumsq, void *stream);
 
 int foc_occ_tail_forward(const void *h, const void *c, uint32_t c_width, const float *deltas, const int32_t *rays,
                          uint32_t M, uint32_t N, float T_thresh, float density_scale, const float *bg_ray, float bg_scalar,
```

Measured after the change: 1.324 billion (median of 6 runs). About the same (+0.3%).
